# leopard-ai/betty

Hardware: AMD Instinct MI355X
Metric: hypergradient-steps/sec (CG K=20, 10M inner params) (higher is better)
Workload: dtype f32

## Files before the change

betty_amd/_native.py:

```python
from __future__ import annotations

import ctypes
import os
from ctypes import POINTER, c_char_p, c_double, c_float, c_int, c_int32, c_int64, c_size_t, c_void_p

_HERE = os.path.dirname(os.path.abspath(__file__))
LIB_PATH = os.environ.get("BHG_LIB") or os.path.join(_HERE, "csrc", "libbhg.so")
AB_LIB_PATH = os.environ.get("BHG_AB_LIB") or os.path.join(_HERE, "csrc", "libbhg_ab.so")

BHG_CHUNK_ELEMS = 4096
BHG_FLAT_ALIGN = 64
BHG_CG_AUTO, BHG_CG_STREAM, BHG_CG_RESIDENT = 0, 1, 2
BHG_CG_GLOBAL_CHAIN, BHG_CG_GLOBAL_UPDATE, BHG_CG_GLOBAL_DOTS = 0, 1, 2
BHG_CG_FX_BEGIN, BHG_CG_FX_CHAIN, BHG_CG_FX_GRAM, BHG_CG_FX_END = 0, 1, 2, 3


class NativeLibraryError(RuntimeError):
    """libbhg.so is missing or a call into it failed."""


class Chunk(ctypes.Structure):

    _fields_ = [
        ("flat_off", c_int64),
        ("src_off", c_int64),
        ("tensor", c_int32),
        ("len", c_int32),
    ]


BHG_MLP_MAX_LAYERS = 32


class Mlp(ctypes.Structure):

    _fields_ = [
        ("L", c_int32),
        ("B", c_int32),
        ("Bp", c_int32),
        ("dims", c_int32 * (BHG_MLP_MAX_LAYERS + 1)),
        ("W", c_void_p * BHG_MLP_MAX_LAYERS),
        ("h", c_void_p * BHG_MLP_MAX_LAYERS),
        ("mask", c_void_p * BHG_MLP_MAX_LAYERS),
        ("delta", c_void_p * BHG_MLP_MAX_LAYERS),
        ("prob", c_void_p),
        ("sd", c_void_p),
        ("Rh", c_void_p * BHG_MLP_MAX_LAYERS),
        ("Rd", c_void_p * BHG_MLP_MAX_LAYERS),
        ("partial", c_void_p),
        ("partial_floats", c_size_t),
        ("ridge2", c_float),
        ("prepacked", c_int32),
    ]


_PP = POINTER(c_void_p)
_CH = c_void_p

SYMBOLS = {
    "bhg_version": (c_int, []),
    "bhg_last_error": (c_char_p, []),
    "bhg_layout_flat_size": (c_int64, [POINTER(c_int64), c_int]),
    "bhg_layout_num_chunks": (c_int64, [POINTER(c_int64), c_int]),
    "bhg_layout_build": (c_int, [POINTER(c_int64), c_int, POINTER(c_int64), POINTER(Chunk)]),
    "bhg_workspace_bytes": (c_size_t, [c_int]),
    "bhg_flatten": (c_int, [_PP, c_int, _CH, c_int, c_void_p, c_float, c_void_p, c_void_p]),
    "bhg_scatter": (c_int, [c_void_p, _PP, c_int, _CH, c_int, c_float, c_void_p, c_void_p]),
    "bhg_neumann_init": (c_int, [_PP, c_int, _CH, c_int, c_void_p, c_void_p, c_void_p, c_void_p]),
    "bhg_neumann_step": (
        c_int,
        [_PP, c_int, _CH, c_int, c_void_p, c_void_p, c_float, c_float, c_float, c_void_p, c_void_p],
    ),
    "bhg_cg_init": (c_int, [_PP, c_int, _CH, c_int, c_void_p, c_void_p, c_void_p, c_void_p, c_void_p]),
    "bhg_cg_init_masked": (c_int, [_PP, c_int, _CH, c_int, c_void_p, c_void_p, c_void_p, ctypes.c_uint64, c_void_p, c_void_p]),
    "bhg_cg_step": (
        c_int,
        [_PP, c_int, _CH, c_int, c_void_p, c_void_p, c_void_p, c_float, c_int, c_float, c_float, c_int, c_void_p, c_void_p],
    ),
    "bhg_cg_phase": (
        c_int,
        [c_int, _PP, c_int, _CH, c_int, c_void_p, c_void_p, c_void_p, c_float, c_int, c_float, c_float, c_void_p, c_void_p],
    ),
    "bhg_cg_partials_dev": (c_void_p, [c_void_p, c_int, c_int]),
    "bhg_cg_partials_count": (c_int, []),
    "bhg_cg_resident_capacity_chunks": (c_int, []),
    "bhg_cg_resident_ok": (c_int, []),
    "bhg_cg_resident_usable": (c_int, [c_int]),
    "bhg_cg_scalars_dev": (c_void_p, [c_void_p]),
    "bhg_cg_timeout_flag_dev": (c_void_p, [c_void_p]),
    "bhg_scale_flat": (c_int, [c_void_p, c_int64, c_float, c_void_p]),
    "bhg_darts_eps": (c_int, [_PP, c_int, _CH, c_int, c_double, c_void_p, c_void_p, c_void_p, c_void_p]),
    "bhg_axpy_multi": (c_int, [_PP, _PP, c_int, _CH, c_int, c_void_p, c_float, c_void_p, c_void_p]),
    "bhg_fd_perturb": (c_int, [_PP, c_void_p, _PP, c_int, _CH, c_int, c_void_p, c_float, c_void_p, c_void_p]),
    "bhg_cg_step_fd": (
        c_int,
        [_PP, _PP, c_void_p, c_int, _CH, c_int, c_void_p, c_void_p, c_void_p, c_float, c_int, c_float, c_float, c_int, c_void_p, c_void_p],
    ),
    "bhg_neumann_step_fd": (
        c_int,
        [_PP, _PP, c_void_p, c_int, _CH, c_int, c_void_p, c_void_p, c_float, c_float, c_float, c_void_p, c_void_p],
    ),
    "bhg_sama_adam_precondition": (
        c_int,
        [_PP, _PP, _PP, _PP, c_int, _CH, c_int, c_void_p, c_double, c_double, c_double, c_double, c_void_p, c_void_p],
    ),
    "bhg_debug_set": (c_int, [c_char_p, c_int]),
    "bhg_debug_unset": (c_int, [c_char_p]),
    "bhg_debug_reset": (None, []),
    "bhg_debug_key_count": (c_int, []),
    "bhg_debug_key_name": (c_char_p, [c_int]),
    "bhg_is_ab_build": (c_int, []),
    "bhg_timing_enable": (c_int, [c_int]),
    "bhg_timing_read": (c_int, [c_int, POINTER(c_double), POINTER(c_int)]),
    "bhg_logreg_prepare": (c_int, [c_void_p, c_void_p, c_void_p, c_int, c_int, c_void_p]),
    "bhg_logreg_tmp_floats": (c_size_t, [c_int, c_int]),
    "bhg_logreg_hvp": (
        c_int,
        [c_void_p, c_void_p, c_void_p, c_void_p, c_void_p, c_void_p, c_int, c_int, c_void_p],
    ),
    "bhg_logreg_solve_plan": (c_int, [c_int, c_int, c_int, c_int, c_char_p, c_size_t]),
    "bhg_logreg_solve_ws_bytes": (c_size_t, [c_int, c_int]),
    "bhg_logreg_cg_solve": (
        c_int,
        [c_void_p, c_void_p, c_void_p, c_void_p, c_void_p, c_void_p, c_void_p, c_int, c_int, c_int, c_float, c_float, c_int, c_int, c_void_p],
    ),
    "bhg_logreg_neumann_solve": (
        c_int,
        [c_void_p, c_void_p, c_void_p, c_void_p, c_void_p, c_void_p, c_void_p, c_int, c_int, c_int, c_float, c_float, c_int, c_int, c_void_p],
    ),
    "bhg_mlp_partial_floats": (c_size_t, [POINTER(Mlp)]),
    "bhg_mlp_hvp": (c_int, [POINTER(Mlp), _PP, _PP, c_void_p]),
    "bhg_mlp_hvp_mode": (c_int, [POINTER(Mlp), _PP, _PP, c_int, c_void_p]),
    "bhg_mlp_supports_native_prepare": (c_int, [POINTER(Mlp)]),
    "bhg_mlp_forward": (c_int, [POINTER(Mlp), _PP, c_void_p, c_void_p, c_void_p]),
    "bhg_mlp_backward": (c_int, [POINTER(Mlp), c_void_p, c_void_p]),
    "bhg_mlp_mixed_coeff": (c_int, [POINTER(Mlp), _PP, c_void_p, c_void_p, c_void_p]),
    "bhg_mlp_supports_fused_solve": (c_int, [POINTER(Mlp)]),
    "bhg_mlp_fused_ws_bytes": (c_size_t, [POINTER(Mlp)]),
    "bhg_mlp_cg_solve": (
        c_int,
        [POINTER(Mlp), c_void_p, c_void_p, c_void_p, POINTER(c_int64), _CH, c_int, c_int, c_float, c_float, c_void_p,
         c_void_p, c_size_t, c_void_p],
    ),
    "bhg_mlp_cg_state_mask": (ctypes.c_uint64, [POINTER(Mlp), c_int]),
    "bhg_mlp_cg_solve_rhs": (
        c_int,
        [POINTER(Mlp), c_void_p, c_void_p, c_void_p, POINTER(c_int64), _CH, c_int, c_int, c_float, c_float, c_void_p,
         c_void_p, c_size_t, _PP, c_void_p],
    ),
    "bhg_mlp_cg_global_phase": (
        c_int,
        [POINTER(Mlp), c_void_p, c_void_p, c_void_p, POINTER(c_int64), _CH, c_int, c_int, c_int, c_int, c_int, c_void_p, c_float,
         c_float, c_void_p, c_void_p, c_size_t, c_void_p],
    ),
    "bhg_mlp_fx_supported": (c_int, [POINTER(Mlp), c_int]),
    "bhg_mlp_fx_ws_bytes": (c_size_t, [POINTER(Mlp), c_int]),
    "bhg_mlp_fx_const_floats": (c_size_t, [POINTER(Mlp)]),
    "bhg_mlp_fx_slab_floats": (c_size_t, [POINTER(Mlp)]),
    "bhg_mlp_fx_scal_doubles": (c_size_t, [POINTER(Mlp)]),
    "bhg_mlp_cg_fx_phase": (
        c_int,
        [POINTER(Mlp), _PP, c_int, c_int, c_int, c_int, c_int, c_void_p, c_void_p, c_void_p, c_float, c_float, c_void_p, c_size_t,
         c_void_p, c_size_t, c_void_p],
    ),
    "bhg_mlp_neumann_fx_phase": (
        c_int,
        [POINTER(Mlp), _PP, c_int, c_int, c_int, c_int, c_int, c_void_p, c_void_p, c_void_p, c_float, c_float, c_void_p, c_size_t,
         c_void_p, c_size_t, c_void_p],
    ),
    "bhg_mlp_cg_mixed_coeff": (c_int, [POINTER(Mlp), c_void_p, c_void_p, c_float, c_void_p, c_size_t, c_void_p]),
    "bhg_mlp_timeout_flag_dev": (c_void_p, [POINTER(Mlp), c_void_p]),
    "bhg_mlp_stage_batch": (c_int, [POINTER(Mlp), c_void_p, c_void_p, c_void_p, c_void_p]),
    "bhg_mlp_supports_packed_prepare": (c_int, [POINTER(Mlp)]),
    "bhg_mlp_forward_packed": (c_int, [POINTER(Mlp), _PP, c_void_p, c_void_p, c_void_p, c_size_t, c_void_p]),
    "bhg_mlp_backward_packed": (c_int, [POINTER(Mlp), c_void_p, c_void_p, c_size_t, c_void_p]),
    "bhg_mwn_max_hidden": (c_int, []),
    "bhg_mlp_fd_ws_bytes": (c_size_t, [POINTER(c_int), c_int, c_int]),
    "bhg_mlp_fd_forward": (
        c_int,
        [c_void_p, c_void_p, c_int, POINTER(c_int), c_int, _PP, _PP, c_void_p, c_int, c_void_p, c_void_p, c_void_p, c_size_t, c_void_p],
    ),
    "bhg_mwn_fd_vjp": (
        c_int,
        [c_void_p, c_void_p, c_int, c_void_p, c_void_p, c_void_p, c_void_p, c_int, c_void_p, c_int, c_void_p, c_void_p, c_void_p, c_void_p,
         c_void_p],
    ),
    "bhg_quad_fd": (c_int, [_PP, _PP, _PP, c_int, _CH, c_int, c_void_p, c_float, c_int, c_int, c_int, c_void_p]),
    "bhg_mwn_forward": (c_int, [c_void_p, c_int, c_void_p, c_void_p, c_void_p, c_void_p, c_int, c_void_p, c_void_p, c_void_p]),
    "bhg_mwn_backward": (
        c_int,
        [c_void_p, c_void_p, c_int, c_void_p, c_void_p, c_void_p, c_void_p, c_int, c_float, c_void_p, c_void_p, c_void_p, c_void_p, c_void_p],
    ),
    "bhg_mlp_neumann_solve": (
        c_int,
        [POINTER(Mlp), c_void_p, c_void_p, c_void_p, POINTER(c_int64), c_int, c_float, c_float, c_void_p, c_size_t, POINTER(c_int), c_void_p],
    ),
    "bhg_mlp_wsk_launches": (c_int64, []),
    "bhg_mlp_hoist_launches": (c_int64, []),
    "bhg_mlp_proj_iterations": (c_int64, []),
    "bhg_mlp_lin_launches": (c_int64, []),
    "bhg_mlp_neumann_mixed_coeff": (c_int, [POINTER(Mlp), _PP, c_void_p, c_void_p, c_float, c_int, c_int, c_void_p, c_size_t, c_void_p]),
    "bhg_mlp_plan_describe": (c_int, [POINTER(Mlp), c_int, c_int, ctypes.c_char_p, c_size_t]),
    "bhg_copy2d": (c_int, [c_void_p, c_int64, c_void_p, c_int64, c_int64, c_int64, c_void_p]),
    "bhg_bn_ws_bytes": (c_size_t, [c_int]),
    "bhg_bn_backward_vjp": (
        c_int,
        [c_void_p, c_void_p, c_void_p, c_void_p, c_void_p, c_void_p, c_void_p, c_void_p, c_int, c_int, c_int, c_void_p, c_void_p, c_void_p,
         c_void_p, c_size_t, c_void_p],
    ),
}

_libs = {}
_current = [None]


_PY_ENV = {"BHG_LIB", "BHG_AB_LIB", "BHG_HVP_GRAPH", "BHG_ALL_RANKS_ON_GPU0"}
_warned_env = [False]


def _warn_legacy_env() -> None:
    if _warned_env[0]:
        return
    _warned_env[0] = True
    stale = sorted(k for k in os.environ if k.startswith("BHG_") and k not in _PY_ENV)
    if stale:
        import warnings

        warnings.warn("betty_amd: environment variable(s) " + ", ".join(stale) + " are IGNORED — libbhg reads no environment variable. "
                      "Measurement arms are selected with betty_amd._native.use_ab() + debug_set(key, int) (bench.py --debug KEY=INT) "
                      "on the measurement build libbhg_ab.so.", RuntimeWarning, stacklevel=3)


def _bind(path: str) -> ctypes.CDLL:
    lib = _libs.get(path)
    if lib is not None:
        return lib
    _warn_legacy_env()
    if not os.path.exists(path):
        raise NativeLibraryError(
            f"{path} not found: the HIP extension has not been built. Run "
            "`python -c 'import __graft_entry__ as g; g.build()'` or `make -C betty_amd/csrc`. "
            "betty_amd has no CPU fallback."
        )
    lib = ctypes.CDLL(path)
    for name, (restype, argtypes) in SYMBOLS.items():
        try:
            fn = getattr(lib, name)
        except AttributeError as exc:
            raise NativeLibraryError(f"{path} does not export {name}") from exc
        fn.restype = restype
        fn.argtypes = argtypes
    _libs[path] = lib
    return lib


def load() -> ctypes.CDLL:
    return _bind(_current[0] or LIB_PATH)


def current_lib_path() -> str:
    return _current[0] or LIB_PATH


def is_ab() -> bool:
    return bool(load().bhg_is_ab_build())


def use_ab(on: bool = True) -> None:
    if on:
        _bind(AB_LIB_PATH)
        _current[0] = AB_LIB_PATH
    else:
        _current[0] = None


def check(rc: int, what: str) -> None:
    if rc != 0:
        msg = load().bhg_last_error()
        raise NativeLibraryError(f"{what} failed with code {rc}: {msg.decode() if msg else ''}")


def _debug_key(key: str) -> bytes:
    k = key.strip()
    if k.upper().startswith("BHG_"):
        k = k[4:]
    return k.lower().encode()


def debug_set(key: str, value) -> None:
    lib = load()
    if value is not None and not lib.bhg_is_ab_build():
        raise NativeLibraryError(f"bhg_debug_set({key}): the product libbhg.so carries no measurement arm — call "
                                 "betty_amd._native.use_ab() first (libbhg_ab.so; the `bhg_debug` fixture and `bench.py --debug` do)")
    if value is None:
        check(lib.bhg_debug_unset(_debug_key(key)), f"bhg_debug_unset({key})")
    else:
        check(lib.bhg_debug_set(_debug_key(key), int(value)), f"bhg_debug_set({key})")


def debug_reset() -> None:
    load().bhg_debug_reset()


def debug_keys():
    lib = load()
    return [lib.bhg_debug_key_name(i).decode() for i in range(lib.bhg_debug_key_count())]


def ptr_array(ptrs):
    arr = (c_void_p * len(ptrs))(*ptrs)
    return ctypes.cast(arr, _PP), arr


def plan_describe(dims, B: int, algo: str = "cg", keep_solution: bool = False) -> dict:
    lib = load()
    d = Mlp()
    d.L, d.B, d.Bp = len(dims) - 1, int(B), (int(B) + 127) // 128 * 128
    for i, v in enumerate(dims):
        d.dims[i] = int(v)
    buf = ctypes.create_string_buffer(2048)
    check(lib.bhg_mlp_plan_describe(ctypes.byref(d), {"cg": 0, "neumann": 1}[algo], 1 if keep_solution else 0, buf, 2048), "bhg_mlp_plan_describe")
    out, text = {}, buf.value.decode()
    import re

# ... 5 lines not shown
```

betty_amd/csrc/bhg_common.hpp:

```cpp
#pragma once
#include <hip/hip_runtime.h>
#include <stdint.h>
#include <stddef.h>
#include <stdio.h>
#include <string.h>

#include "bhg.h"

namespace bhg {

constexpr int kThreads = 256;
constexpr int kWaves = kThreads / 64;
constexpr int kChunk = BHG_CHUNK_ELEMS;
constexpr int kVecPerThread = kChunk / (kThreads * 4);
constexpr int kMaxBlocks = 1024;
constexpr int kInlineT = 32;
constexpr int kWriterT = 448;

constexpr size_t kWsScal = 0;
constexpr size_t kWsPartP = 128;
constexpr size_t kWsPartR = kWsPartP + 8 * kMaxBlocks;
constexpr size_t kWsBarrier = kWsPartR + 16 * kMaxBlocks;
constexpr size_t kWsTables = kWsBarrier + 256;
inline size_t ws_bytes(int T) {
  size_t b = kWsTables + 4 * sizeof(void*) * (size_t)(T > 0 ? T : 0);
  return (b + 255) & ~(size_t)255;
}

enum { S_RR_OLD = 0, S_PHP = 1, S_ALPHA = 2, S_RR_NEW = 3, S_BETA = 4, S_PP = 5 , S_ALPHA_RING = 10 ,
       S_NPART0 = 8  };

#define BHG_DBG_KEYS(X)                                                                                                      \
  X(mlp_wsk) X(mlp_wsk_maxk) X(mlp_wsk_depth) X(mlp_wsk_lds) X(wsl_depth) X(no_nt_slabs) X(gemm_no_xpose) X(mlp_no_fast)      \
  X(mlp_tn) X(split_target) X(split_cap) X(mlp_no_head) X(gram_ksplit) X(gram_kchunk) X(proj_graw_split) X(mlp_proj)         \
  X(mlp_hoist) X(hoist_wgs) X(proj_step_alone) X(mlp_no_side) X(mlp_no_fuse) X(mlp_no_outer_all) X(neumann_side)             \
  X(hoist_staged_mink) X(proj_alpha_alone) X(proj_small_alone) X(outer_order_by_work) X(outer_no_pre) X(outer_stagger)       \
  X(mlp_no_fused_solve) X(cg_eager_p) X(cg_x_every_iter) X(neumann_p_every_iter) X(head_no_prefetch) X(cg_spin_limit)        \
  X(packed_chain) X(packed_depth) X(packed_gram) X(proj_max_ratio) X(proj_ws_cap_mb) X(alpha_in_hoist) X(graw_v2) X(wskp_ragged) X(pstep_v2) X(pstep_unroll) X(rnew_in_graw) X(graw_cols) X(lin_first) X(lin_prio) X(lin_nub) X(lin_order) X(lin_update_next) X(lin_withhold_beta) X(neumann_vnew) X(cg_rhs_direct) X(packed_prepare) X(lin_deep) X(graw_kloop) X(lin_update_in_head) X(xcd_pairs) X(headu_head_first) X(fx_ksplit)
enum DbgKey : int {
#define BHG_DBG_ENUM(n) DBG_##n,
  BHG_DBG_KEYS(BHG_DBG_ENUM)
#undef BHG_DBG_ENUM
  DBG_COUNT
};
constexpr int kDbgUnset = INT32_MIN;
#ifdef BHG_AB
extern int g_dbg[DBG_COUNT];
inline bool dbg_is_set(DbgKey k) { return g_dbg[k] != kDbgUnset; }
inline int dbg(DbgKey k, int dflt) { return g_dbg[k] == kDbgUnset ? dflt : g_dbg[k]; }
#else
constexpr bool dbg_is_set(DbgKey) { return false; }
constexpr int dbg(DbgKey, int dflt) { return dflt; }
#endif

constexpr int kStampKernels = 4, kStampBlocks = 4096, kStampSlots = 8;
#ifdef BHG_STAMPS
#ifdef __HIPCC__
#define BHG_STAMP(kid, slot)                                                                                            \
  do {                                                                                                                  \
    if (threadIdx.x == 0 && blockIdx.x < ::bhg::kStampBlocks) {                                                         \
      unsigned long long* sp_ = ::bhg::d_stamps;                                                                        \
      if (sp_) sp_[((kid) * ::bhg::kStampBlocks + blockIdx.x) * ::bhg::kStampSlots + (slot)] = wall_clock64();          \
    }                                                                                                                   \
  } while (0)
#endif
#else
#define BHG_STAMP(kid, slot) do { } while (0)
#endif

void set_error(const char* fmt, ...);
#define BHG_HIP_CHECK(expr)                                                        \
  do {                                                                             \
    hipError_t _e = (expr);                                                        \
    if (_e != hipSuccess) {                                                        \
      ::bhg::set_error("%s failed: %s (%s:%d)", #expr, hipGetErrorString(_e), __FILE__, \
                       __LINE__);                                                  \
      return BHG_ERR_HIP;                                                          \
    }                                                                              \
  } while (0)
#define BHG_REQUIRE(cond, msg)                                                     \
  do {                                                                             \
    if (!(cond)) {                                                                 \
      ::bhg::set_error("%s: %s", __func__, msg);                                   \
      return BHG_ERR_ARG;                                                          \
    }                                                                              \
  } while (0)

struct PtrTab {
  const void* const* dev;
  const void* inl[kInlineT];
};

int make_table(PtrTab* out, const void* const* host_ptrs, int T, void* ws, int slot,
               hipStream_t stream);

bool span_begin(int kind, hipEvent_t* a, hipEvent_t* b);

#ifdef __HIPCC__
__device__ __forceinline__ float* tab_ptr(const PtrTab& t, int i) {
  const void* p = t.dev ? t.dev[i] : t.inl[i];
  return (float*)p;
}

__device__ __forceinline__ float4 ld4(const float* __restrict__ base, int e, int len) {
  if (e + 4 <= len) return *reinterpret_cast<const float4*>(base + e);
  float4 r = make_float4(0.f, 0.f, 0.f, 0.f);
  if (e < len) r.x = base[e];
  if (e + 1 < len) r.y = base[e + 1];
  if (e + 2 < len) r.z = base[e + 2];
  return r;
}
__device__ __forceinline__ void st4(float* __restrict__ base, int e, int len, float4 v) {
  if (e + 4 <= len) {
    *reinterpret_cast<float4*>(base + e) = v;
    return;
  }
  if (e < len) base[e] = v.x;
  if (e + 1 < len) base[e + 1] = v.y;
  if (e + 2 < len) base[e + 2] = v.z;
}

__device__ __forceinline__ float mul_rn(float a, float b) { return __fmul_rn(a, b); }
__device__ __forceinline__ float add_rn(float a, float b) { return __fadd_rn(a, b); }
__device__ __forceinline__ float sub_rn(float a, float b) { return __fsub_rn(a, b); }
__device__ __forceinline__ float div_rn(float a, float b) { return __fdiv_rn(a, b); }
__device__ __forceinline__ float4 scale4(float s, float4 a) {
  return make_float4(mul_rn(s, a.x), mul_rn(s, a.y), mul_rn(s, a.z), mul_rn(s, a.w));
}
__device__ __forceinline__ float4 add4(float4 a, float4 b) {
  return make_float4(add_rn(a.x, b.x), add_rn(a.y, b.y), add_rn(a.z, b.z), add_rn(a.w, b.w));
}
__device__ __forceinline__ float4 add_scaled4(float4 a, float s, float4 b) {
  return make_float4(add_rn(a.x, mul_rn(s, b.x)), add_rn(a.y, mul_rn(s, b.y)), add_rn(a.z, mul_rn(s, b.z)),
                     add_rn(a.w, mul_rn(s, b.w)));
}
__device__ __forceinline__ float4 sub_scaled4(float4 a, float s, float4 b) {
  return make_float4(sub_rn(a.x, mul_rn(s, b.x)), sub_rn(a.y, mul_rn(s, b.y)), sub_rn(a.z, mul_rn(s, b.z)),
                     sub_rn(a.w, mul_rn(s, b.w)));
}
__device__ __forceinline__ float4 diff_over4(float4 a, float4 b, float d) {
  return make_float4(div_rn(sub_rn(a.x, b.x), d), div_rn(sub_rn(a.y, b.y), d), div_rn(sub_rn(a.z, b.z), d),
                     div_rn(sub_rn(a.w, b.w), d));
}
__device__ __forceinline__ double dot4(float4 a, float4 b) {
  return (double)a.x * b.x + (double)a.y * b.y + (double)a.z * b.z + (double)a.w * b.w;
}

template <int BYTES>
__device__ __forceinline__ void kernarg_warm() {
  typedef const __attribute__((address_space(4))) unsigned* KP;
  KP kp = (KP)__builtin_amdgcn_kernarg_segment_ptr();
  unsigned acc = 0;
#pragma unroll
  for (int o = 0; o < BYTES; o += 64) acc |= kp[o / 4];
  asm volatile("" ::"s"(acc));
}
template <int U>
__device__ __forceinline__ double sum_strided(const double* __restrict__ p, const int n, const int t, const int stride) {
  double acc = 0.0;
  for (int i0 = t; i0 < n; i0 += U * stride) {
    double v[U];
#pragma unroll
    for (int u = 0; u < U; ++u) {
      const int i = i0 + u * stride;
      v[u] = p[i < n ? i : n - 1];
    }
#pragma unroll
    for (int u = 0; u < U; ++u)
      if (i0 + u * stride < n) acc += v[u];
  }
  return acc;
}

template <int U>
struct StridedRegs { double v[U]; };
template <int U>
__device__ __forceinline__ void strided_load(StridedRegs<U>& r, const double* __restrict__ p, const int n, const int t, const int stride,
                                             const double* __restrict__ dummy) {
  const double* q = (p && n > 0) ? p : dummy;
  const int last = (p && n > 0) ? n - 1 : 0;
#pragma unroll
  for (int u = 0; u < U; ++u) {
    const int i = t + u * stride;
    r.v[u] = q[i < n && i <= last ? i : last];
  }
}
template <int U>
__device__ __forceinline__ double strided_sum(const StridedRegs<U>& r, const int n, const int t, const int stride) {
  double acc = 0.0;
#pragma unroll
  for (int u = 0; u < U; ++u)
// ... 72 lines not shown
```

betty_amd/csrc/bhg_mlp.hip:

```cpp
#include <stdlib.h>
#include <vector>


#include "bhg_common.hpp"

#ifdef BHG_STAMPS
namespace bhg { __device__ unsigned long long* d_stamps = nullptr; }
#endif

namespace bhg {
namespace {
#include "mlp/gemm.inc"

#include "mlp/outer.inc"

#include "mlp/scalars.inc"

#include "mlp/head.inc"

#include "mlp/wsk.inc"

#include "mlp/wskp.inc"

inline int wsk_mode(int chain_mode, int unfused_hint) {
  if (dbg_is_set(DBG_mlp_wsk)) return dbg(DBG_mlp_wsk, 0);
  if (chain_mode == FUSE_CG) return 2;
  if (chain_mode == FUSE_NEUMANN) return 3;
  return unfused_hint;
}
inline bool wsk_wanted(int mode, int pairs, int K) {
  if (mode == 1) return true;
  if (mode != 2 && mode != 3) return false;
  return pairs * K <= dbg(DBG_mlp_wsk_maxk, 1024);
}
inline int wsk_depth() {
  const int d = dbg(DBG_mlp_wsk_depth, 3);
  return d == 2 ? 2 : 3;
}
inline bool wsk_eligible(const WskArgs& a) {
  if (a.pairs < 1 || a.pairs > 2) return false;
  bool ok = a.M % 32 == 0 && a.N % 32 == 0 && a.K % 32 == 0 && a.K >= 32;
  for (int i = 0; i < a.pairs; ++i) ok = ok && (a.pr[i].lda & 3) == 0 && (a.pr[i].ldb & 3) == 0;
  return ok;
}
int64_t g_wsk_launches = 0;
int64_t g_hoist_launches = 0;
int64_t g_proj_iterations = 0;
int64_t g_lin_launches = 0;
template <int LB>
void launch_gemm_wsk(const WskArgs& a_in, hipStream_t st, bool staged = false) {
  WskArgs a = a_in;
  ++g_wsk_launches;
  a.ntm = a.M / 32;
  a.ntn = a.N / 32;
  bool bf = false;
  for (int i = 0; i < a.pairs; ++i) bf = bf || a.pr[i].mix != 0;
  const dim3 grid(a.ntm * a.ntn), block(64 * kWskWaves);
  const int d = wsk_depth();
  const bool force_staged = dbg(DBG_mlp_wsk_lds, 0) != 0;
  if ((staged || force_staged) && !bf) {
    const int lds = (int)(sizeof(float) * kWslWaveFloats * kWskWaves);
    static bool attr_done = false;
    if (!attr_done) {
      (void)hipFuncSetAttribute(reinterpret_cast<const void*>(k_gemm_wsk<LB, false, 2, true>), hipFuncAttributeMaxDynamicSharedMemorySize, lds);
      attr_done = true;
    }
#ifdef BHG_AB
    const int wsl_depth = dbg(DBG_wsl_depth, 2);
    if (wsl_depth == 3) {
      static bool attr3 = false;
      if (!attr3) {
        (void)hipFuncSetAttribute(reinterpret_cast<const void*>(k_gemm_wsk<LB, false, 3, true>), hipFuncAttributeMaxDynamicSharedMemorySize, lds);
        attr3 = true;
      }
      hipLaunchKernelGGL((k_gemm_wsk<LB, false, 3, true>), grid, block, lds, st, a);
      return;
    }
#endif
    hipLaunchKernelGGL((k_gemm_wsk<LB, false, 2, true>), grid, block, lds, st, a);
    return;
  }
#define BHG_WSK(BFV, DV) hipLaunchKernelGGL((k_gemm_wsk<LB, BFV, DV>), grid, block, 0, st, a)
  if (bf) {
    if (d == 2 || LB == LAYOUT_RC) BHG_WSK(true, 2); else BHG_WSK(true, LB == LAYOUT_RC ? 2 : 3);
  } else {
#ifdef BHG_AB
    if (d == 2) BHG_WSK(false, 2); else
#endif
    BHG_WSK(false, 3);
  }
#undef BHG_WSK
}

#ifdef BHG_AB
void launch_wsk_group(const WskGroupArgs& g, int blocks, hipStream_t st) {
  const int lds = (int)(sizeof(float) * kWslWaveFloats * kWskWaves);
  static bool attr_done = false;
  if (!attr_done) {
    (void)hipFuncSetAttribute(reinterpret_cast<const void*>(k_wsk_group<2>), hipFuncAttributeMaxDynamicSharedMemorySize, lds);
#ifdef BHG_AB
    (void)hipFuncSetAttribute(reinterpret_cast<const void*>(k_wsk_group<3>), hipFuncAttributeMaxDynamicSharedMemorySize, lds);
#endif
    attr_done = true;
  }
#ifdef BHG_AB
  const int wsl_depth = dbg(DBG_wsl_depth, 2);
  if (wsl_depth == 3) { hipLaunchKernelGGL(k_wsk_group<3>, dim3(blocks), dim3(64 * kWskWaves), lds, st, g); return; }
#endif
  hipLaunchKernelGGL(k_wsk_group<2>, dim3(blocks), dim3(64 * kWskWaves), lds, st, g);
}
#endif

int chip_cus() {
  static int cus[64];
  int dev = 0;
  if (hipGetDevice(&dev) != hipSuccess || dev < 0 || dev >= 64) { (void)hipGetLastError(); return 256; }
  if (cus[dev] > 0) return cus[dev];
  int n = 0;
  if (hipDeviceGetAttribute(&n, hipDeviceAttributeMultiprocessorCount, dev) != hipSuccess || n <= 0) { (void)hipGetLastError(); n = 256; }
  return cus[dev] = n;
}
inline void wskp_tiling(WskpProb* q, bool ragged) {
  q->nfull = q->RA / 32;
  q->nstrip = 0;
  q->pairs = dbg(DBG_xcd_pairs, 1);
  if (!ragged || q->raw || q->nsplit != 1 || q->RB % 64 != 0) return;
  int nf = q->B / 32, rem = q->B % 32;
  if (rem > 16) { ++nf; rem = 0; }
  if (nf == 0) return;
  q->nfull = nf;
  q->nstrip = rem > 0 ? q->RB / 64 : 0;
}
struct WskpBuilder {
  WskpArgs g{};
  int blk = 0;
  bool add(const WskpProb& q_in) {
    if (g.n >= kWskpMax) return false;
    g.p[g.n++] = q_in;
    return true;
  }
  void tile(bool ragged) {
    blk = 0;
    for (int i = 0; i < g.n; ++i) {
      WskpProb& q = g.p[i];
      wskp_tiling(&q, ragged);
      g.blk0[i] = blk;
      blk += (((q.nfull * (q.RB / 32) + q.nstrip) * q.nsplit) + 7) & ~7;
    }
  }
  void launch(hipStream_t st) {
    if (!g.n) return;
    const int mode = dbg(DBG_wskp_ragged, 1);
    tile(mode == 2);
    if (mode == 1 && blk > chip_cus()) tile(true);
    g.blk0[g.n] = blk;
    const int d = dbg(DBG_packed_depth, 2);
    bool riders = g.n <= 3;
// ... 197 lines not shown
  size_t rh0alt_off;
  size_t gp2alt_off;
  bool proj_ok;
  size_t floats;
  int gf[BHG_MLP_MAX_LAYERS], gb[BHG_MLP_MAX_LAYERS];
};
inline bool graw_batch_ok(int Bp) { return Bp == 128 || (Bp % 128 == 0 && dbg(DBG_graw_kloop, 1) != 0); }
inline bool graw_split() {
  return dbg(DBG_proj_graw_split, 1) != 0;
}
inline int proj_mode() {
  return dbg(DBG_mlp_proj, 1);
}
inline int hoist_mode() {
  return dbg(DBG_mlp_hoist, 1);
}
void hoist_plan(const bhg_mlp* m, HoistPlan* hp) {
  memset(hp, 0, sizeof(*hp));
  const int L = m->L, Bp = m->Bp;
  for (int l = 0; l < BHG_MLP_MAX_LAYERS; ++l) hp->gf[l] = hp->gb[l] = -1;
  if (!use_head(m) || L < 3 || L - 1 > kHoistMax / 2 || Bp % kTM != 0) return;
  for (int l = 0; l <= L - 1; ++l) if (m->dims[l] % 32 != 0) return;
  const int Nh = m->dims[L - 1];
  if ((size_t)Nh * sizeof(float) > 64 * 1024) return;
  for (int l = 1; l + 1 < L; ++l)
    if ((Bp / 32) * (m->dims[l] / 32) != reduce_blocks(Bp * m->dims[l], m->dims[l])) return;
  int n = 0;
  for (int l = 0; l + 1 < L; ++l) { hp->layer[n] = l; hp->bwd[n] = 0; hp->K[n] = m->dims[l]; hp->N[n] = m->dims[l + 1]; hp->gf[l] = n; ++n; }
  for (int l = 1; l + 1 < L; ++l) { hp->layer[n] = l; hp->bwd[n] = 1; hp->K[n] = m->dims[l + 1]; hp->N[n] = m->dims[l]; hp->gb[l] = n; ++n; }
  hp->n = n;
  const int slots = dbg(DBG_hoist_wgs, 768);
  const int ntm = Bp / kTM;
  int tgt = 8;
  for (; tgt < 4096; ++tgt) {
    int wgs = 0;
    for (int i = 0; i < n; ++i) {
      const int ks = hp->K[i] / kTK;
      const int per = ks < tgt ? ks : tgt;
      wgs += (hp->N[i] / 32) * ntm * ((ks + per - 1) / per);
    }
    if (wgs <= slots) break;
  }
  size_t off = 0;
  int blk = 0;
  for (int i = 0; i < n; ++i) {
    const int ks = hp->K[i] / kTK;
    int sp = (ks + tgt - 1) / tgt;
    const int per = (ks + sp - 1) / sp;
    sp = (ks + per - 1) / per;
    hp->splits[i] = sp;
    hp->blk0[i] = blk;
    blk += (hp->N[i] / 32) * ntm * sp;
    hp->slab_off[i] = off; off += (size_t)sp * Bp * hp->N[i];
    hp->g_off[i] = off;    off += (size_t)Bp * hp->N[i];
    hp->gr_off[i] = off;   off += (size_t)Bp * hp->N[i];
    hp->graw_off[i] = off; off += (size_t)2 * Bp * hp->N[i];
  }
  {
    double fh = 0.0, fp = 0.0;
    for (int l = 0; l + 1 < L; ++l) fh += (double)m->dims[l] * m->dims[l + 1] * (l >= 1 ? 2.0 : 1.0);
    fh *= 2.0 * Bp;
    for (int l = 0; l + 1 < L; ++l) {
      fp += (double)m->dims[l + 1] * (l == 0 ? 1.0 : 2.0);
      if (l >= 1) fp += 2.0 * m->dims[l] + (double)m->dims[l] + (double)m->dims[l + 1];
    }
    fp *= 2.0 * Bp * (double)Bp;
    size_t gram = 0;
    for (int l = 0; l + 1 < L; ++l) gram += (size_t)Bp * Bp * (l >= 1 ? (2 + 2 * kGramSplitMax + 6) : 2);
    size_t widest = 0;
    for (int i = 0; i < n; ++i) widest = (size_t)hp->N[i] > widest ? (size_t)hp->N[i] : widest;
    hp->proj_ok = fp * 100.0 <= fh * (double)dbg(DBG_proj_max_ratio, 400) &&
                  gram * sizeof(float) <= (size_t)dbg(DBG_proj_ws_cap_mb, 1024) * 1024 * 1024 &&
                  (size_t)Bp * (widest / 4) <= ((size_t)1 << 20);
  }
  hp->dot_blocks = 0;
  for (int i = 0; i < n; ++i) hp->dot_blocks += dot_blocks_of(Bp * (hp->N[i] / 4));
  hp->raw_blocks = 0;
  for (int i = 0; i < n; ++i) hp->raw_blocks += (hp->N[i] / 32) * ntm * 2;
  for (int l = 0; hp->proj_ok && l + 1 < L; ++l) {
    hp->s_off[l] = off; off += (size_t)Bp * Bp;
    if (l >= 1) {
      hp->d_off[l] = off; off += (size_t)Bp * Bp;
      hp->tslab_off[l] = off; off += (size_t)kGramSplitMax * Bp * Bp;
      hp->eslab_off[l] = off; off += (size_t)kGramSplitMax * Bp * Bp;
    }
  }
  for (int l = 0; hp->proj_ok && l + 1 < L; ++l) {
    hp->sp_off[l] = off; off += (size_t)Bp * Bp;
    if (l >= 1) {
      hp->dp_off[l] = off; off += (size_t)Bp * Bp;
      hp->tslabp_off[l] = off; off += (size_t)2 * Bp * Bp;
      hp->eslabp_off[l] = off; off += (size_t)2 * Bp * Bp;
    }
  }
  hp->lin_ok = hp->proj_ok && L >= 4 && (L == 4 || dbg(DBG_lin_deep, 1) != 0);
  if (hp->lin_ok) {
    for (int i = 0; i < 2; ++i) { hp->z1_off[i] = off; off += (size_t)Bp * m->dims[2]; }
    hp->rh0rp_off = off; off += (size_t)Bp * m->dims[1];
    hp->gp1alt_off = off; off += (size_t)Bp * m->dims[2];
    hp->rb0c_off = off; off += (size_t)((m->dims[1] + 63) & ~63);
  }
  if (hp->proj_ok) { hp->rh0alt_off = off; off += (size_t)Bp * m->dims[1]; }
  if (hp->lin_ok) { hp->gp2alt_off = off; off += (size_t)Bp * m->dims[L - 1]; }
  hp->graw_tiles = 0;
  for (int i = 0; i < n; ++i) hp->graw_tiles += (Bp / 64) * (hp->N[i] / 32);
  hp->blk0[n] = blk;
  hp->floats = off;
  hp->ok = true;
}

int graw_cols(const HoistPlan* hp, int Bp = 128) {
  if (dbg(DBG_graw_cols, 32) != 64 || Bp != 128) return 32;
  for (int i = 0; i < hp->n; ++i)
    if (hp->N[i] % 64) return 32;
  return 64;
}
int graw_tile_count(const HoistPlan* hp, int Bp) {
  const int ct = graw_cols(hp, Bp);
  int t = 0;
  for (int i = 0; i < hp->n; ++i) t += (Bp / 64) * (hp->N[i] / ct);
  return t;
}
int graw_blocks(const HoistPlan* hp, int Bp) {
  int n = 0;
  for (int i = 0; i < hp->n; ++i) {
    const bool two = !(hp->bwd[i] == 0 && hp->layer[i] == 0);
    n += (hp->N[i] / 32) * (Bp / kTM) * ((two && graw_split()) ? 2 : 1);
  }
  return n;
}

bool proj_step_merged() {
  return dbg(DBG_proj_step_alone, 0) == 0;
}

struct FusedWs {
  double* partT1; double* partT2h; double* partT2; double* partPP; double* partRR[2];
  float* rz; double* rzx;
  int t2_off[BHG_MLP_MAX_LAYERS];
  int nRR, nT2;
  float* hoist;
  double* part_dot; double* pscal;
  double* part_raw;
  double* part_graw;
  float* pb0[2];
  float* pb1[2];
  unsigned long long* gran;
  float* Wf[BHG_MLP_MAX_LAYERS];
  float* Wb[BHG_MLP_MAX_LAYERS];
  float* hpk[BHG_MLP_MAX_LAYERS];
  float* dpk[BHG_MLP_MAX_LAYERS];
  float* Rhp[BHG_MLP_MAX_LAYERS];
  float* Rdp[BHG_MLP_MAX_LAYERS];
  size_t bytes;
};
void carve_fused_ws(const bhg_mlp* m, void* base, FusedWs* w) {
  memset(w, 0, sizeof(*w));
  const bool head = use_head(m);
  int nrr = bias_blocks(m);
  for (int l = 0; l < m->L; ++l) nrr += outer_blocks(m, l, head);
  w->nRR = nrr;
  size_t off = 0;
  auto take = [&](size_t bytes) { void* p = base ? static_cast<char*>(base) + off : nullptr; off += (bytes + 255) & ~(size_t)255; return p; };
  w->partT1 = static_cast<double*>(take(sizeof(double) * m->Bp));
  w->partT2h = static_cast<double*>(take(sizeof(double) * m->Bp));
  w->partPP = static_cast<double*>(take(sizeof(double) * kMaxBlocks));
  w->partRR[0] = static_cast<double*>(take(sizeof(double) * 3 * nrr));
  w->partRR[1] = static_cast<double*>(take(sizeof(double) * 3 * nrr));
  int nt2 = 0;
  for (int l = 1; l + 1 < m->L; ++l) { w->t2_off[l] = nt2; nt2 += reduce_blocks(m->Bp * m->dims[l], m->dims[l]); }
  w->nT2 = nt2;
  w->partT2 = static_cast<double*>(take(sizeof(double) * (nt2 > 0 ? nt2 : 1)));
  w->rz = static_cast<float*>(take(sizeof(float) * (size_t)m->Bp * m->dims[m->L]));
  w->rzx = static_cast<double*>(take(sizeof(double) * (size_t)m->Bp * m->dims[m->L]));
  HoistPlan hp;
  hoist_plan(m, &hp);
  w->hoist = static_cast<float*>(take(sizeof(float) * (hp.ok ? hp.floats : 1)));
  w->part_dot = static_cast<double*>(take(sizeof(double) * 2 * (hp.ok ? hp.dot_blocks : 1)));
  w->part_raw = static_cast<double*>(take(sizeof(double) * (hp.ok ? hp.raw_blocks : 1)));
  w->part_graw = static_cast<double*>(take(sizeof(double) * 3 * (hp.ok ? hp.graw_tiles : 1)));
  w->pscal = static_cast<double*>(take(sizeof(double) * 8));
  for (int i = 0; i < 2; ++i) w->pb0[i] = static_cast<float*>(take(sizeof(float) * (size_t)m->dims[1]));
  for (int i = 0; i < 2; ++i) w->pb1[i] = static_cast<float*>(take(sizeof(float) * (size_t)(m->L >= 2 ? m->dims[2] : 1)));
  w->gran = static_cast<unsigned long long*>(take(64 * 64));
  if (hp.ok) {
    const int L = m->L;
    const size_t Bp = (size_t)m->Bp;
    for (int l = 0; l + 1 < L; ++l) {
      w->hpk[l] = static_cast<float*>(take(sizeof(float) * Bp * m->dims[l]));
      if (l + 2 < L) w->Rhp[l] = static_cast<float*>(take(sizeof(float) * Bp * m->dims[l + 1]));
      if (l >= 1) {
        w->Wf[l] = static_cast<float*>(take(sizeof(float) * (size_t)m->dims[l + 1] * m->dims[l]));
        w->Wb[l] = static_cast<float*>(take(sizeof(float) * (size_t)m->dims[l + 1] * m->dims[l]));
        w->dpk[l] = static_cast<float*>(take(sizeof(float) * Bp * m->dims[l + 1]));
        w->Rdp[l] = static_cast<float*>(take(sizeof(float) * Bp * m->dims[l + 1]));
      }
    }
  }
  w->bytes = off;
}

bool graw_single_on(bool packed, int Bp) { return packed && dbg(DBG_packed_gram, 1) != 0 && dbg(DBG_graw_v2, 1) != 0 && graw_batch_ok(Bp); }
bool rnew_keys_on() { return dbg(DBG_proj_small_alone, 0) == 0 && dbg(DBG_alpha_in_hoist, 1) != 0 && dbg(DBG_rnew_in_graw, 1) != 0; }

bool packed_chain_on(const FusedWs& w) { return w.Wf[1] != nullptr && dbg(DBG_packed_chain, 1) != 0; }
int pack_operands(const bhg_mlp* m, const FusedWs& w, hipStream_t st, bool weights_only = false) {
  PackArgs g{};
  int blk = 0;
  auto add = [&](const float* X, float* Xp, int R, int K, int kind) {
    if (g.n >= kPackMax) return false;
    g.p[g.n] = {X, Xp, R, K, kind};
    g.blk0[g.n] = blk;
    blk += pack_blocks(g.p[g.n]);
    ++g.n;
    return true;
  };
  const int L = m->L, Bp = m->Bp;
  bool ok = true;
  for (int l = 0; l + 1 < L && ok; ++l) {
    if (!weights_only || l == 0) ok = ok && add(m->h[l], w.hpk[l], Bp, m->dims[l], 0);
    if (l >= 1) {
      if (!weights_only) ok = ok && add(m->delta[l], w.dpk[l], Bp, m->dims[l + 1], 0);
      ok = ok && add(m->W[l], w.Wf[l], m->dims[l + 1], m->dims[l], 0);
      ok = ok && add(m->W[l], w.Wb[l], m->dims[l], m->dims[l + 1], 1);
    }
  }
  BHG_REQUIRE(ok, "too many layers for one packing launch");
  g.blk0[g.n] = blk;
  hipLaunchKernelGGL(k_pack, dim3(blk), dim3(256), 0, st, g);
  BHG_HIP_CHECK(hipGetLastError());
  return BHG_OK;
}

#include "mlp/chain_plan.inc"

int hoist_products(const bhg_mlp* m, const void* const* dir, const ChainMode& cm, const ChainPlan& pl, hipStream_t st, ChainState* cs) {
  const int L = m->L, Bp = m->Bp, B = m->B;
  const HoistPlan* hp = pl.hp;
  float* hbase = pl.hoist;
  HoistArgs ha{};
  HoistRedArgs ra{};
  for (int i = 0; i < hp->n; ++i) {
    const int l = hp->layer[i];
    HoistProb& q = ha.p[i];
    q.A = hp->bwd[i] ? m->delta[l] : m->h[l];
    q.Bm = pl.cg ? ((cm.first && cm.rhs) ? static_cast<const float*>(cm.rhs[2 * l]) : cm.fa + cm.starts[2 * l]) : static_cast<const float*>(dir[2 * l]);
    q.slabs = hbase + hp->slab_off[i];
    q.K = hp->K[i]; q.N = hp->N[i]; q.splits = hp->splits[i]; q.rc = hp->bwd[i];
    q.lda = hp->K[i]; q.ldb = hp->bwd[i] ? hp->N[i] : hp->K[i];
    ha.blk0[i] = hp->blk0[i];
    HoistRedProb& rq = ra.p[i];
    rq.slabs = q.slabs; rq.G = hbase + hp->g_off[i]; rq.N = hp->N[i]; rq.splits = hp->splits[i];
    if (!hp->bwd[i] && l == 0) {
      rq.bias = static_cast<const float*>(dir[1]); rq.mask = m->mask[0]; rq.out = m->Rh[0];
      rq.outp = pl.packed ? cm.ws->Rhp[0] : nullptr;
    }
  }
  ha.blk0[hp->n] = hp->blk0[hp->n];
  ha.n = hp->n; ha.Bp = Bp; ha.gemm_blocks = hp->blk0[hp->n];
  const bool proj = cm.proj != 0;
  int rblk = 0;
  for (int i = 0; i < hp->n; ++i) { ra.blk0[i] = rblk; rblk += (Bp * (hp->N[i] / 4) + 255) / 256; }
  ra.blk0[hp->n] = rblk;
  if (!proj || cm.first) {
    ha.do_beta = (pl.cg && !cm.first && cm.beta && !proj) ? 1 : 0;
    ha.beta_blocks = ha.do_beta ? cm.beta_blocks : 0;
    if (ha.do_beta) ha.beta = *cm.beta;
    hipLaunchKernelGGL(k_hoist<FUSE_CG>, dim3(ha.gemm_blocks + (ha.do_beta ? cm.beta_blocks : 0)), dim3(256), 0, st, ha);
    ++g_hoist_launches;
    if (proj && pl.cg) for (int i = 0; i < hp->n; ++i) ra.p[i].G2 = hbase + hp->gr_off[i];
    ra.n = hp->n; ra.Bp = Bp; ra.B = B; ra.first = pl.cg ? cm.first : 1; ra.scal = cm.scal;
    hipLaunchKernelGGL(k_hoist_reduce, dim3(rblk), dim3(256), 0, st, ra);
  } else if (pl.vnew) {
    ++g_proj_iterations;
  } else {
    ProjArgs pa{};
    for (int i = 0; i < hp->n; ++i) {
      ProjProb& q = pa.p[i];
      q.Gr = hbase + (pl.cg ? hp->gr_off[i] : hp->g_off[i]); q.Gp = hbase + hp->g_off[i]; q.Graw = hbase + hp->graw_off[i]; q.N = hp->N[i];
      if (!pl.graw_single && graw_split() && !(hp->bwd[i] == 0 && hp->layer[i] == 0)) q.Graw2 = q.Graw + (size_t)Bp * hp->N[i];
      if (pl.rnew) q.Graw = nullptr;
      if (!hp->bwd[i] && hp->layer[i] == 0) {
        q.bias = static_cast<const float*>(dir[1]); q.mask = m->mask[0]; q.out = m->Rh[0];
        q.outp = pl.packed ? cm.ws->Rhp[0] : nullptr;
      }
      pa.blk0[i] = ra.blk0[i];
    }
    pa.blk0[hp->n] = rblk;
    pa.n = hp->n; pa.Bp = Bp; pa.B = B; pa.kpar_prev = cm.kpar ^ 1; pa.shift = cm.shift; pa.scal = pl.cg ? cm.scal : nullptr; pa.alpha = cm.alpha;
    if (pl.cg && cm.proj >= 2 && proj_step_merged()) {
      ProjStepArgs g{};
      g.pa = pa;
      ProjScalArgs& sa = g.sa;
      sa.part_dot = cm.ws->part_dot; sa.dot_blocks = hp->dot_blocks;
      sa.part_raw = cm.ws->part_raw; sa.raw_blocks = graw_blocks(hp, Bp);
      if (pl.graw_single) {
        const int gt = graw_tile_count(hp, Bp);
        sa.part_dot = cm.ws->part_graw; sa.dot_blocks = gt;
        sa.part_raw = cm.ws->part_graw + 2 * (size_t)gt; sa.raw_blocks = gt;
      }
      sa.part = cm.beta->part; sa.part_stride = cm.ws->nRR;
      sa.off0 = pl.part_base_w[L - 1]; sa.n0 = outer_blocks(m, L - 1, pl.head); sa.off1 = pl.part_base_bias; sa.n1 = bias_blocks(m);
      sa.r_small = cm.beta->r; sa.p_small = cm.beta->p; sa.snt = cm.beta->nt;
      int small_total = 0;
      for (int t = 0; t < cm.beta->nt; ++t) { sa.soff[t] = cm.beta->off[t]; sa.slen[t] = cm.beta->len[t]; small_total += cm.beta->len[t]; }
      sa.scal = cm.scal; sa.pscal = cm.ws->pscal; sa.shift = cm.shift; sa.first = cm.second; sa.kpar = cm.kpar ^ 1;
      const int sgrid = small_total > 0 ? (small_total + kThreads - 1) / kThreads : 1;
      g.update_blocks = rblk;
      g.r_b0 = cm.fa + cm.starts[1];
      g.p0_rd = cm.second ? cm.fd + cm.starts[1] : cm.ws->pb0[cm.kpar ^ 1];
      g.p0_wr = cm.ws->pb0[cm.kpar];
      if (pl.graw_single && cm.beta->nt <= 16 && dbg(DBG_pstep_v2, 1) != 0) {
        PstepArgs ps{};
        PstepHdr& h = ps.h;
        const int pu = pl.lin ? 4 : dbg(DBG_pstep_unroll, 4);
        const int U = pu >= 4 ? 4 : (pu >= 2 ? 2 : 1);
        int ublk = 0;
        for (int i = 0; i < hp->n; ++i) { h.blk0[i] = ublk; ublk += (Bp * (hp->N[i] / 4) + 256 * U - 1) / (256 * U); }
        h.blk0[hp->n] = ublk;
        const int rblk = ublk;
        h.n = pa.n; h.Bp = pa.Bp; h.B = pa.B; h.kpar_prev = pa.kpar_prev; h.shift = pa.shift; h.update_blocks = rblk;
        h.scal = sa.scal; h.r_b0 = g.r_b0; h.p0_rd = g.p0_rd; h.p0_wr = g.p0_wr; h.r_small = sa.r_small; h.p_small = sa.p_small;
        h.part_dot = sa.part_dot; h.part_raw = sa.part_raw; h.part = sa.part; h.pscal = sa.pscal;
        h.dot_blocks = sa.dot_blocks; h.raw_blocks = sa.raw_blocks; h.part_stride = sa.part_stride;
        h.off0 = sa.off0; h.n0 = sa.n0; h.off1 = sa.off1; h.n1 = sa.n1; h.first = sa.first; h.kpar = sa.kpar; h.snt = sa.snt;
        for (int i = 0; i < hp->n; ++i) {
          const ProjProb& q = pa.p[i];
          ps.p[i] = {q.Gr, q.Gp, q.Graw, q.bias, q.mask, q.out, q.outp, q.N, q.Graw ? 1 : 0};
          if (pl.lin && i == hp->gf[1]) { ps.p[i].Gp = pl.gp1(cm.kpar ^ 1); ps.p[i].X = pl.gp1(cm.kpar); ps.p[i].xkind = 2; }
          if (pl.lin_head && i == hp->gf[L - 2]) { ps.p[i].Gp = pl.gp2(cm.kpar ^ 1); ps.p[i].X = pl.gp2(cm.kpar); ps.p[i].xkind = 2; }
          if (pl.lin) ps.p[i].outp = nullptr;
        }
        if (pl.lin) {
          h.p1_rd = cm.second ? cm.fd + cm.starts[3] : cm.ws->pb1[cm.kpar ^ 1];
          h.p1_wr = cm.ws->pb1[cm.kpar];
          h.gran = cm.ws->gran;
          h.rb0_copy = hbase + hp->rb0c_off;
          h.prio = dbg(DBG_lin_prio, 0);
          h.withhold = dbg(DBG_lin_withhold_beta, 0);
          int nub = dbg(DBG_lin_nub, 0);
          if (nub > 0) {
            WskpProb tq{};
            tq.RA = Bp; tq.RB = m->dims[2]; tq.B = B; tq.nsplit = 1;
            wskp_tiling(&tq, true);
            const int tiles = ((tq.nfull * (tq.RB / 32) + tq.nstrip + 7) & ~7) + (Bp / 32) * (Bp / 32);
            const int room = chip_cus() - tiles - sgrid;
            if (nub == 1 || nub > room) nub = room;
          }
          h.nub = (nub > 0 && nub < rblk) ? nub : 0;
        }
        for (int t = 0; t < sa.snt; ++t) { ps.t.slen[t] = sa.slen[t]; ps.t.soff[t] = sa.soff[t]; }
        if (pl.lin) { cs->lin_ps = ps; cs->lin_nu = (h.nub > 0 ? h.nub : rblk) + sgrid; cs->lin_U = U; }
#ifdef BHG_AB
        else if (U == 2) hipLaunchKernelGGL(k_pstep<2>, dim3(rblk + sgrid), dim3(256), 0, st, ps);
        else if (U == 1) hipLaunchKernelGGL(k_pstep<1>, dim3(rblk + sgrid), dim3(256), 0, st, ps);
#endif
        else hipLaunchKernelGGL(k_pstep<4>, dim3(rblk + sgrid), dim3(256), 0, st, ps);
      } else {
#ifdef BHG_AB
        hipLaunchKernelGGL(k_proj_step, dim3(rblk + sgrid), dim3(256), 0, st, g);
#else
        BHG_REQUIRE(false, "internal: every plan of the product takes k_pstep (<= 16 small tensors, the packed closing launch)");
#endif
      }
    } else {
      hipLaunchKernelGGL(k_proj_update, dim3(rblk), dim3(256), 0, st, pa);
    }
    ++g_proj_iterations;
  }
  return BHG_OK;
}

int lin_first_product(const bhg_mlp* m, const void* const* dir, const ChainMode& cm, const ChainPlan& pl, hipStream_t st, ChainState* cs) {
  const int L = m->L, Bp = m->Bp, B = m->B, K = m->dims[1], N = m->dims[2];
  const HoistPlan* hp = pl.hp;
  float* hbase = pl.hoist;
  const float* c = static_cast<const float*>(dir[3]);
  const float* Gf = hbase + hp->g_off[hp->gf[1]];
  BHG_REQUIRE(cm.first || cs->lin_nu > 0, "no update blocks for the linear first product");
  WskplArgs la{};
  WskpProb& q = la.a;
  q.Ap = cm.first ? cm.ws->Rhp[0] : hbase + hp->rh0rp_off;
  q.Bq = cm.ws->Wf[1]; q.RA = Bp; q.RB = N; q.K = K; q.B = B; q.nsplit = 1;
  q.mask = m->mask[1]; q.out = m->Rh[1]; q.outp = cm.ws->Rhp[1];
  q.znew = hbase + hp->z1_off[cm.kpar];
  if (cm.first) { q.addend = Gf; q.bias = c; }
  else {
    q.addend = hbase + hp->gr_off[hp->gf[1]]; q.addend2 = pl.gp1(cm.kpar ^ 1);
    q.bias = cm.fa + cm.starts[3]; q.bias2 = cs->lin_ps.h.p1_rd;
    q.zold = hbase + hp->z1_off[cm.kpar ^ 1];
    q.gran = cm.ws->gran;
  }
  const int rider_blocks = pl.gram_in_chain ? (Bp / 32) * (Bp / 32) : 0;
  wskp_tiling(&q, false);
  int na = (q.nfull * (q.RB / 32) + q.nstrip + 7) & ~7;
  if (dbg(DBG_wskp_ragged, 1) == 2 || (dbg(DBG_wskp_ragged, 1) == 1 && na + rider_blocks > chip_cus()) ||
      (!cm.first && cs->lin_ps.h.nub > 0)) {
    wskp_tiling(&q, true);
    na = (q.nfull * (q.RB / 32) + q.nstrip + 7) & ~7;
  }
  la.na = na;
  if (pl.gram_in_chain) {
    float* tnew = hbase + hp->tslab_off[1] + (size_t)cm.kpar * Bp * Bp;
    float* tnewp = pl.graw2 ? hbase + hp->tslabp_off[1] + (size_t)cm.kpar * Bp * Bp : nullptr;
    la.r0 = {cm.ws->hpk[1], q.Ap, tnew, tnewp, K, 0};
    la.r0_old = cm.first ? nullptr : hbase + hp->tslab_off[1] + (size_t)(cm.kpar ^ 1) * Bp * Bp;
  }
  la.nu = cm.first ? 0 : cs->lin_nu;
  const bool upd_next = !cm.first && L == 4 && dbg(DBG_lin_update_next, 1) != 0 && cs->lin_ps.h.nub == 0;
  if (upd_next) {
    la.ns = cs->lin_nu - cs->lin_ps.h.update_blocks;
    la.nt = na + rider_blocks;
  } else if (!cm.first && L > 4 && cs->lin_ps.h.nub == 0) {
    la.ns = cs->lin_nu - cs->lin_ps.h.update_blocks;
    la.nt = na + rider_blocks;
    la.upd_first = 1;
  } else
  if (!cm.first && dbg(DBG_lin_order, 0) != 0) {
    la.ns = cs->lin_nu - (cs->lin_ps.h.nub > 0 ? cs->lin_ps.h.nub : cs->lin_ps.h.update_blocks);
    la.nt = na + rider_blocks;
  }
  la.ps = cs->lin_ps;
  BHG_REQUIRE(cm.first || la.ns > 0 || cs->lin_ps.h.update_blocks <= 2 * chip_cus(),
              "update blocks ahead of the publisher would not all be resident: use the default order");
  const int grid = (upd_next ? la.ns : la.nu) + na + rider_blocks;
  cs->lin_update_pending = upd_next;
  BHG_REQUIRE(cm.first || cs->lin_U == 4, "the update blocks inside k_wskpl are built for four float4 per thread");
#ifdef BHG_AB
  if (la.ps.h.nub > 0) hipLaunchKernelGGL((k_wskpl<2, 4, true>), dim3(grid), dim3(64 * kWskpWaves), 0, st, la); else
#endif
  hipLaunchKernelGGL((k_wskpl<2, 4, false>), dim3(grid), dim3(64 * kWskpWaves), 0, st, la);
  ++g_lin_launches;
  if (cm.first)
    BHG_HIP_CHECK(hipMemcpyAsync(hbase + hp->rb0c_off, cm.fa + cm.starts[1], sizeof(float) * (size_t)m->dims[1],
                                 hipMemcpyDeviceToDevice, st));
  return BHG_OK;
}

int hoist_forward(const bhg_mlp* m, const void* const* dir, const ChainMode& cm, const ChainPlan& pl, hipStream_t st, int staged_mink,
                  ChainState* cs) {
  const int L = m->L, Bp = m->Bp, B = m->B;
  const HoistPlan* hp = pl.hp;
  float* hbase = pl.hoist;
  for (int l = 1; l + 1 < L; ++l) {
    const int K = m->dims[l], N = m->dims[l + 1];
    const float* c = static_cast<const float*>(dir[2 * l + 1]);
    const float* Gf = hbase + hp->g_off[hp->gf[l]];
    if (pl.packed) {
    if (pl.lin && l == 1) {
      if (int rc = lin_first_product(m, dir, cm, pl, st, cs)) return rc;
    } else {
      WskpBuilder wb;
      WskpProb q{};
      q.Ap = cm.ws->Rhp[l - 1]; q.Bq = cm.ws->Wf[l]; q.RA = Bp; q.RB = N; q.K = K; q.B = B; q.nsplit = 1;
      if (l == L - 2) {
        const int riders = (pl.gram_in_chain && l == 1) ? (Bp / 32) * (Bp / 32) : 0;
        const int tiles_l = (Bp / 32) * (N / 32);
        int sp = (chip_cus() - riders) / tiles_l;
        const int cap = pick_splits((N + pl.tn - 1) / pl.tn, K, 1);
        if (sp > cap) sp = cap;
        if (sp > K / 64) sp = K / 64;
        if (sp < 1) sp = 1;
        q.nsplit = sp; q.raw = 1; q.out = m->partial;
        cs->head_fuse = {m->partial, sp, Bp * N, c, m->mask[l], m->Rh[l], (pl.lin_head && !cm.first) ? hbase + hp->gr_off[hp->gf[l]] : Gf};
        cs->fuse_head = true;
      } else {
        q.bias = c; q.mask = m->mask[l]; q.addend = Gf; q.out = m->Rh[l]; q.outp = cm.ws->Rhp[l];
      }
      wb.add(q);
      if (pl.gram_in_chain && l == 1) {
        WskpProb t{};
        t.Ap = cm.ws->hpk[l]; t.Bq = cm.ws->Rhp[l - 1]; t.RA = Bp; t.RB = Bp; t.K = K; t.B = B;
        t.nsplit = 1; t.raw = 1; t.out = hbase + hp->tslab_off[l]; t.outp = pl.graw2 ? hbase + hp->tslabp_off[l] : nullptr;
        wb.add(t);
      }
      if (cs->lin_update_pending && wb.g.n == 1 && !pl.lin_head) {
        launch_wskpu(wb.g.p[0], cs->lin_ps, cs->lin_ps.h.update_blocks, st);
        cs->lin_update_pending = false;
      } else wb.launch(st);
    }
      if (pl.gram_in_chain && cm.first && l == 1) {
        WskpBuilder sb;
        for (int j = 0; j + 1 < L; ++j) {
          WskpProb u{};
          u.Ap = cm.ws->hpk[j]; u.Bq = cm.ws->hpk[j]; u.RA = Bp; u.RB = Bp; u.K = m->dims[j]; u.B = B; u.raw = 1;
          u.nsplit = 1;
          u.out = hbase + hp->s_off[j]; u.outp = hbase + hp->sp_off[j];
          if (!sb.add(u)) { sb.launch(st); sb.add(u); }
          if (j >= 1) {
            u.Ap = cm.ws->dpk[j]; u.Bq = cm.ws->dpk[j]; u.K = m->dims[j + 1]; u.out = hbase + hp->d_off[j]; u.outp = hbase + hp->dp_off[j];
            if (!sb.add(u)) { sb.launch(st); sb.add(u); }
          }
        }
        sb.launch(st);
        cs->sd_in_chain = true;
      }
      continue;
    }
    if (l == L - 2) {
      GemmArgs a{};
      a.pr[0] = {m->Rh[l - 1], m->W[l], K, K};
      a.pairs = 1; a.M = Bp; a.N = N; a.K = K;
      a.splits = pick_splits((N + pl.tn - 1) / pl.tn, K, 1);
      a.out = m->partial; a.ldo = N; a.out_rows = Bp;
      launch_gemm<LAYOUT_KC, LAYOUT_KC>(a, pl.tn, st);
      cs->head_fuse = {m->partial, a.splits, Bp * N, c, m->mask[l], m->Rh[l], Gf};
      cs->fuse_head = true;
    } else {
      WskArgs w{};
      w.pr[0] = {m->Rh[l - 1], m->W[l], K, K}; w.pairs = 1; w.M = Bp; w.N = N; w.K = K; w.B = B;
      w.bias = c; w.mask = m->mask[l]; w.out = m->Rh[l]; w.addend = Gf;
      launch_gemm_wsk<LAYOUT_KC>(w, st, K >= staged_mink);
    }
  }
  BHG_REQUIRE(!cs->lin_update_pending || pl.lin_head, "the update blocks found no launch to ride in");
  return BHG_OK;
}

int hoist_head(const bhg_mlp* m, const void* const* dir, const ChainMode& cm, const ChainPlan& pl, hipStream_t st, ChainState* cs) {
  const int L = m->L, Bp = m->Bp, B = m->B;
  if (cs->lin_update_pending) {
    const int l = L - 1, K = m->dims[l], N = m->dims[l + 1];
    BHG_REQUIRE(cs->fuse_head && pl.cg && pl.packed && N <= 12 && K <= 512, "k_headu was planned for a head it cannot run");
    HeaduArgs ha{};
    ha.Rh = (const float*)m->Rh[l - 1]; ha.h = m->h[l]; ha.W = m->W[l]; ha.V = static_cast<const float*>(dir[2 * l]);
    ha.cb = static_cast<const float*>(dir[2 * l + 1]); ha.prob = m->prob; ha.sd = m->sd; ha.rd = m->Rd[l];
    ha.K = K; ha.C = N; ha.B = B; ha.mode = HEAD_JVP;
    ha.delta_top = (const float*)m->delta[l]; ha.mask_prev = (const float*)m->mask[l - 1]; ha.rd_prev = m->Rd[l - 1];
    ha.fz = cs->head_fuse;
    ha.partT1 = cm.ws->partT1; ha.partT2h = cm.ws->partT2h; ha.rz_out = cm.ws->rz; ha.rzx_acc = cm.rzx_acc; ha.rzx_first = cm.first;
    ha.rows = Bp; ha.rd_prev_p = cm.ws->Rdp[l - 1];
    ha.addend2 = pl.gp2(cm.kpar ^ 1); ha.gran = cm.ws->gran;
    ha.nu = cs->lin_ps.h.update_blocks; ha.ps = cs->lin_ps; ha.head_first = dbg(DBG_headu_head_first, 1);
    hipLaunchKernelGGL(k_headu<4>, dim3(ha.nu + Bp), dim3(256), (size_t)K * sizeof(float), st, ha);
    cs->lin_update_pending = false;
  } else {
    const int l = L - 1, K = m->dims[l], N = m->dims[l + 1];
    launch_head_forward(st, Bp, (const float*)m->Rh[l - 1], m->h[l], m->W[l], static_cast<const float*>(dir[2 * l]),
                        static_cast<const float*>(dir[2 * l + 1]), m->prob, m->sd, m->Rd[l], K, N, B, HEAD_JVP, nullptr, nullptr,
                        (const float*)m->delta[l], (const float*)m->mask[l - 1], m->Rd[l - 1], &cs->head_fuse,
                        pl.cg ? cm.ws->partT1 : nullptr, pl.cg ? cm.ws->partT2h : nullptr, pl.cg ? cm.ws->rz : nullptr, cm.rzx_acc, cm.first,
                        pl.packed ? cm.ws->Rdp[l - 1] : nullptr);
  }
  return BHG_OK;
}

void hoist_backward(const bhg_mlp* m, const ChainMode& cm, const ChainPlan& pl, hipStream_t st, int staged_mink) {
  const int L = m->L, Bp = m->Bp, B = m->B;
  const HoistPlan* hp = pl.hp;
  float* hbase = pl.hoist;
  for (int l = L - 2; l >= 1; --l) {
    const int K = m->dims[l + 1], N = m->dims[l];
    if (pl.packed) {
      WskpBuilder wb;
      WskpProb q{};
      q.Ap = cm.ws->Rdp[l]; q.Bq = cm.ws->Wb[l]; q.RA = Bp; q.RB = N; q.K = K; q.B = B; q.nsplit = 1;
      q.mask = m->mask[l - 1]; q.addend = hbase + hp->g_off[hp->gb[l]]; q.out = m->Rd[l - 1];
      q.outp = l >= 2 ? cm.ws->Rdp[l - 1] : nullptr;
      if (pl.cg) { q.rh = m->Rh[l - 1]; q.partT2 = cm.ws->partT2 + cm.ws->t2_off[l]; }
      wb.add(q);
      if (pl.gram_in_chain) {
        WskpProb t{};
        t.Ap = cm.ws->dpk[l]; t.Bq = cm.ws->Rdp[l]; t.RA = Bp; t.RB = Bp; t.K = K; t.B = B;
        t.nsplit = 1; t.raw = 1; t.out = hbase + hp->eslab_off[l]; t.outp = pl.graw2 ? hbase + hp->eslabp_off[l] : nullptr;
        wb.add(t);
        if (l + 1 <= L - 2) {
          t.Ap = cm.ws->hpk[l + 1]; t.Bq = cm.ws->Rhp[l];
          t.out = hbase + hp->tslab_off[l + 1]; t.outp = pl.graw2 ? hbase + hp->tslabp_off[l + 1] : nullptr;
          wb.add(t);
        }
      }
      wb.launch(st);
      continue;
    }
    WskArgs w{};
    w.pr[0] = {m->Rd[l], m->W[l], K, N}; w.pairs = 1; w.M = Bp; w.N = N; w.K = K; w.B = B;
    w.mask = m->mask[l - 1]; w.out = m->Rd[l - 1]; w.addend = hbase + hp->g_off[hp->gb[l]];
    if (pl.cg) { w.rh = m->Rh[l - 1]; w.partT2 = cm.ws->partT2 + cm.ws->t2_off[l]; }
    launch_gemm_wsk<LAYOUT_RC>(w, st, K >= staged_mink);
  }
}

int chain_hoisted(const bhg_mlp* m, const void* const* dir, const ChainMode& cm, const ChainPlan& pl, hipStream_t st, ChainState* cs) {
  if (int rc = hoist_products(m, dir, cm, pl, st, cs)) return rc;
  const int staged_mink = dbg(DBG_hoist_staged_mink, 256);
  if (int rc = hoist_forward(m, dir, cm, pl, st, staged_mink, cs)) return rc;
  if (int rc = hoist_head(m, dir, cm, pl, st, cs)) return rc;
  if (!cm.stop_after_head) hoist_backward(m, cm, pl, st, staged_mink);
  return BHG_OK;
}

void chain_forward(const bhg_mlp* m, const void* const* dir, const ChainMode& cm, const ChainPlan& pl, hipStream_t st, ChainState* cs) {
  const int L = m->L, Bp = m->Bp, B = m->B;
  for (int l = 0; l < L; ++l) {
    const int K = m->dims[l], N = m->dims[l + 1];
    const float* V = static_cast<const float*>(dir[2 * l]);
    const float* c = static_cast<const float*>(dir[2 * l + 1]);
    if (pl.head && l == L - 1) {
      launch_head_forward(st, Bp, l > 0 ? (const float*)m->Rh[l - 1] : nullptr, m->h[l], m->W[l], V, c, m->prob, m->sd,
                          m->Rd[l], K, N, B, HEAD_JVP, nullptr, nullptr, l > 0 ? (const float*)m->delta[l] : nullptr,
                          l > 0 ? (const float*)m->mask[l - 1] : nullptr, l > 0 ? m->Rd[l - 1] : nullptr,
                          cs->fuse_head ? &cs->head_fuse : nullptr, pl.cg ? cm.ws->partT1 : nullptr, pl.cg ? cm.ws->partT2h : nullptr,
                          pl.cg ? cm.ws->rz : nullptr, cm.rzx_acc, cm.first);
      continue;
    }
    GemmArgs a{};
    a.pr[0] = {m->h[l], V, K, K};
    if (cm.lazy) a.pr[0] = {m->h[l], cm.fa + cm.starts[2 * l], K, K, cm.fd + cm.starts[2 * l], 1};
    a.scal = cm.scal;
    a.pairs = 1;
    if (l > 0) { a.pr[1] = {m->Rh[l - 1], m->W[l], K, K}; a.pairs = 2; }
    a.M = Bp; a.N = N; a.K = K;
    const bool to_head = pl.head && l == L - 2 && !pl.no_fuse && (N & 3) == 0 && (size_t)N * sizeof(float) <= 64 * 1024;
    if (wsk_wanted(pl.wsk, a.pairs, K) && !to_head && l + 1 < L) {
      WskArgs w{};
      w.pr[0] = a.pr[0]; w.pr[1] = a.pr[1]; w.pairs = a.pairs; w.M = Bp; w.N = N; w.K = K; w.B = B;
      w.bias = c; w.mask = m->mask[l]; w.out = m->Rh[l]; w.scal = cm.scal;
      if (wsk_eligible(w)) { launch_gemm_wsk<LAYOUT_KC>(w, st); continue; }
    }
    a.splits = pick_splits((N + pl.tn - 1) / pl.tn, K, a.pairs);
    a.out = m->partial; a.ldo = N; a.out_rows = Bp;
    launch_gemm<LAYOUT_KC, LAYOUT_KC>(a, pl.tn, st);
    const int slab = Bp * N;
    if (to_head) {
      cs->head_fuse = {m->partial, a.splits, slab, c, m->mask[l], m->Rh[l]};
      cs->fuse_head = true;
    } else if (l + 1 < L) {
      launch_reduce_mask(st, m->partial, a.splits, slab, c, m->mask[l], m->Rh[l], Bp, N, B);
    } else {
      hipLaunchKernelGGL(k_reduce_softmax_jvp, dim3((Bp + 15) / 16), dim3(256), 0, st, (const float*)m->partial,
                         a.splits, slab, c, m->prob, m->sd, m->Rd[l], Bp, N, B);
    }
  }
}

void outer_args(const bhg_mlp* m, const void* const* dir, const ChainMode& cm, const ChainPlan& pl, int l, GemmArgs* ga, size_t* lds,
                bool* fast) {
  const int B = m->B, Mo = m->dims[l + 1], No = m->dims[l];
  const float* V = static_cast<const float*>(dir[2 * l]);
  GemmArgs a{};
  a.pr[0] = {m->Rd[l], m->h[l], Mo, No};
  a.pairs = 1;
  if (l > 0) { a.pr[1] = {m->delta[l], m->Rh[l - 1], Mo, No}; a.pairs = 2; }
  a.M = Mo; a.N = No; a.K = B;
  a.splits = 1;
  a.out = cm.mode == FUSE_NONE ? static_cast<float*>(cm.out[2 * l]) : nullptr; a.ldo = No; a.out_rows = 0;
  a.addend = pl.rho2 != 0.f ? V : nullptr; a.addend_scale = pl.rho2;
  a.kstages = (B + kOH - 1) / kOH < 2 ? 2 : (B + kOH - 1) / kOH;
  const int Kh = (((B + a.kstages - 1) / a.kstages) + 1) & ~1;
  *lds = (size_t)Kh * (kTM + kTN) * sizeof(float);
  const size_t lds_c = (size_t)kTM * kCPad * sizeof(float);
  if (*lds < lds_c) *lds = lds_c;
  bool f = Mo % kTM == 0 && No % kTN == 0 && (a.ldo & 3) == 0;
  for (int i = 0; i < a.pairs; ++i) f = f && (a.pr[i].lda & 3) == 0 && (a.pr[i].ldb & 3) == 0;
  if (cm.mode != FUSE_NONE) f = f && (cm.starts[2 * l] & 3) == 0;
  const bool no_fast = dbg(DBG_mlp_no_fast, 0) != 0;
  *fast = f && !no_fast;
  *ga = a;
}
HeadOuterArgs head_outer_args(const bhg_mlp* m, const void* const* dir, const ChainMode& cm, const ChainPlan& pl, int l) {
  HeadOuterArgs ha{};
  ha.rd = m->Rd[l]; ha.h = m->h[l]; ha.delta = m->delta[l]; ha.Rh = l > 0 ? m->Rh[l - 1] : nullptr;
  ha.V = static_cast<const float*>(dir[2 * l]); ha.rho2 = pl.rho2;
  ha.out = cm.mode == FUSE_NONE ? static_cast<float*>(cm.out[2 * l]) : nullptr;
  ha.N = m->dims[l]; ha.C = m->dims[l + 1]; ha.B = m->B;
  return ha;
}
void launch_outer(const bhg_mlp* m, const void* const* dir, const ChainMode& cm, const ChainPlan& pl, int l, hipStream_t s) {
  const FuseArgs fz = fuse_at(cm, pl, 2 * l, pl.part_base_w[l]);
  if (pl.head && l == pl.L - 1) {
    const HeadOuterArgs ha = head_outer_args(m, dir, cm, pl, l);
    const dim3 grid((ha.N + 63) / 64, ha.C);
#define BHG_HEAD_OUTER(RH, MODE) hipLaunchKernelGGL((k_head_outer<RH, MODE>), grid, dim3(256), 0, s, ha, fz)
    if (l > 0) {
// ... 237 lines not shown
  for (int i = 0; i < hp->n && !pl.graw2; ++i) {
    const int l = hp->layer[i];
    HoistProb& q = ga.p[i];
    if (!hp->bwd[i]) {
      q.A = hbase + hp->s_off[l]; q.Bm = m->Rd[l];
      if (l >= 1) { q.A2 = hbase + hp->tslab_off[l]; q.B2m = m->delta[l]; q.a2_slabs = pl.gram_slabs(m->dims[l]); }
    } else {
      q.A = hbase + hp->eslab_off[l]; q.Bm = m->h[l]; q.a_slabs = pl.gram_slabs(m->dims[l + 1]);
      q.A2 = hbase + hp->d_off[l]; q.B2m = m->Rh[l - 1];
    }
    q.slabs = hbase + hp->graw_off[i];
    q.a_slab_stride = Bp * Bp;
    if (full) q.X = hp->bwd[i] ? (const float*)m->Rh[l - 1] : (const float*)m->Rd[l];
    q.K = Bp; q.N = hp->N[i]; q.splits = (q.A2 && graw_split()) ? 2 : 1; q.rc = 1; q.lda = Bp; q.ldb = hp->N[i];
    ga.blk0[i] = gblk; gblk += (hp->N[i] / 32) * ntm * q.splits;
  }
  ga.blk0[hp->n] = gblk;
  ga.n = hp->n; ga.Bp = Bp; ga.gemm_blocks = gblk; ga.do_beta = 0;
  if (full && !pl.graw2) {
    int dblk = 0, nd = 0;
    for (int i = 0; i < hp->n; ++i) {
      const int l = hp->layer[i];
      ga.dp[nd] = {hbase + hp->gr_off[i], hbase + hp->g_off[i], hp->bwd[i] ? (const float*)m->Rh[l - 1] : (const float*)m->Rd[l], hp->N[i]};
      ga.dblk0[nd++] = dblk; dblk += dot_blocks_of(Bp * (hp->N[i] / 4));
    }
    ga.dblk0[nd] = dblk;
    ga.nd = nd; ga.dot_blocks = dblk; ga.B = B; ga.part_dot = cm.ws->part_dot; ga.part_raw = cm.ws->part_raw;
    BHG_REQUIRE(gblk == graw_blocks(hp, Bp), "tile count of the G(raw) launch and of its raw.raw partials disagree");
    BHG_REQUIRE(dblk == hp->dot_blocks, "dot block count of the plan and of the launch disagree");
  }
  if (small_in_graw) {
    ga.so = so;
    ga.small_blocks = small_blocks;
    if (alpha_in_hoist) { ga.do_alpha = 1; ga.alpha = od.aa; }
  }
  if (pl.graw2) {
  } else if (pl.cg) hipLaunchKernelGGL(k_hoist<FUSE_CG>, dim3(gblk + ga.dot_blocks + ga.small_blocks), dim3(256), 0, st, ga);
  else hipLaunchKernelGGL(k_hoist<FUSE_NEUMANN>, dim3(gblk + ga.dot_blocks + ga.small_blocks), dim3(256), 0, st, ga);
#endif
  return BHG_OK;
}

int close_outputs(const bhg_mlp* m, const void* const* dir, const ChainMode& cm, const ChainPlan& pl, const ChainOutputs& od, hipStream_t st,
                  bool small_in_graw) {
  const int L = m->L;
  const HoistPlan* hp = pl.hp;
  const bool proj_full = hp && ((pl.cg && cm.proj >= 2) || (!pl.cg && cm.proj));
  const int n_mfma = proj_full ? 0 : (pl.head ? L - 1 : L);
  OuterAllArgs oa{};
  bool all_fast = !pl.no_outer_all && n_mfma <= kOuterAllMax && pl.head;
  size_t lds_max = 0;
  int order[BHG_MLP_MAX_LAYERS];
  const bool work_first = dbg(DBG_outer_order_by_work, 0) != 0;
  auto weight = [&](int l) { return !work_first ? (double)outer_blocks(m, l, pl.head) : (l > 0 ? 2.0 : 1.0) * 1e9 + outer_blocks(m, l, pl.head); };
  for (int i = 0; i < n_mfma; ++i) order[i] = i;
  for (int i = 1; i < n_mfma; ++i)
    for (int j = i; j > 0 && weight(order[j]) > weight(order[j - 1]); --j) { int t = order[j]; order[j] = order[j - 1]; order[j - 1] = t; }
  int blk = 0;
  for (int i = 0; i < n_mfma && all_fast; ++i) {
    const int l = order[i];
    size_t lds; bool fast;
    outer_args(m, dir, cm, pl, l, &oa.g[i], &lds, &fast);
    all_fast = all_fast && fast;
    if (lds > lds_max) lds_max = lds;
    oa.f[i] = fuse_at(cm, pl, 2 * l, pl.part_base_w[l]);
    oa.gx[i] = (oa.g[i].N + kTN - 1) / kTN;
    oa.blk0[i] = blk;
    blk += outer_blocks(m, l, pl.head);
  }
  if (small_in_graw) {
  } else if (all_fast) {
    oa.n = n_mfma;
    oa.blk0[n_mfma] = blk;
    oa.head = head_outer_args(m, dir, cm, pl, L - 1);
    oa.hf = fuse_at(cm, pl, 2 * (L - 1), pl.part_base_w[L - 1]);
    oa.head_gx = (oa.head.N + 63) / 64;
    oa.head_blocks = oa.head_gx * oa.head.C;
    oa.head_has_rh = L > 1;
    oa.bf = od.bias_fz;
    const int total = blk + oa.head_blocks + od.bias_blk;
    if (lds_max < (size_t)kTM * kCPad * sizeof(float)) lds_max = (size_t)kTM * kCPad * sizeof(float);
    const bool no_pre = dbg(DBG_outer_no_pre, 0) != 0;
    (void)no_pre;
    const int stagger = dbg(DBG_outer_stagger, 1);
    oa.stagger = stagger;
#ifdef BHG_AB
    if (no_pre) {
      if (pl.cg) hipLaunchKernelGGL((k_outer_all<FUSE_CG, false>), dim3(total), dim3(256), lds_max, st, oa, od.ba);
      else hipLaunchKernelGGL((k_outer_all<FUSE_NEUMANN, false>), dim3(total), dim3(256), lds_max, st, oa, od.ba);
    } else
#endif
    {
      if (pl.cg) hipLaunchKernelGGL((k_outer_all<FUSE_CG, true>), dim3(total), dim3(256), lds_max, st, oa, od.ba);
      else hipLaunchKernelGGL((k_outer_all<FUSE_NEUMANN, true>), dim3(total), dim3(256), lds_max, st, oa, od.ba);
    }
  } else {
    for (int l = L - 1; l >= 0; --l) launch_outer(m, dir, cm, pl, l, st);
    launch_bias(cm, od, st);
  }
#ifdef BHG_AB
  if (proj_full && pl.cg && !proj_step_merged()) {
    BHG_REQUIRE(all_fast || small_in_graw, "the fully projected CG solver needs the single-launch output path");
    ProjScalArgs sa{};
    sa.part_dot = cm.ws->part_dot; sa.dot_blocks = hp->dot_blocks;
    sa.part_raw = cm.ws->part_raw; sa.raw_blocks = graw_blocks(hp, m->Bp);
    if (pl.graw_single) {
      const int gt = graw_tile_count(hp, m->Bp);
      sa.part_dot = cm.ws->part_graw; sa.dot_blocks = gt;
      sa.part_raw = cm.ws->part_graw + 2 * (size_t)gt; sa.raw_blocks = gt;
    }
    sa.part = cm.partRR_new; sa.part_stride = cm.ws->nRR;
    sa.off0 = pl.part_base_w[L - 1]; sa.n0 = outer_blocks(m, L - 1, pl.head); sa.off1 = pl.part_base_bias; sa.n1 = od.bias_blk;
    sa.r_small = cm.beta->r; sa.p_small = cm.beta->p; sa.snt = cm.beta->nt;
    for (int t = 0; t < cm.beta->nt; ++t) { sa.soff[t] = cm.beta->off[t]; sa.slen[t] = cm.beta->len[t]; }
    sa.scal = cm.scal; sa.pscal = cm.ws->pscal; sa.shift = cm.shift; sa.first = cm.first; sa.kpar = cm.kpar;
    int small_total = 0;
    for (int t = 0; t < cm.beta->nt; ++t) small_total += cm.beta->len[t];
    const int sgrid = small_total > 0 ? (small_total + kThreads - 1) / kThreads : 1;
    hipLaunchKernelGGL(k_proj_scalars, dim3(sgrid), dim3(kThreads), 0, st, sa);
  }
#endif
  return BHG_OK;
}

int chain_close(const bhg_mlp* m, const void* const* dir, const ChainMode& cm, const ChainPlan& pl, const ChainOutputs& od, hipStream_t st,
                const ChainState& cs) {
  const bool alpha_alone = dbg(DBG_proj_alpha_alone, 0) != 0 || pl.gram_in_chain;
  const bool small_alone = dbg(DBG_proj_small_alone, 0) != 0;
  const bool small_in_graw = pl.proj_iter && (cm.proj >= 2 || !pl.cg) && !small_alone;
  const bool alpha_in_hoist = pl.cg && pl.proj_iter && cm.proj >= 2 && small_in_graw && pl.gram_in_chain && cm.gphase == 0 &&
                              dbg(DBG_alpha_in_hoist, 1) != 0;
  const bool alpha_in_gram = pl.cg && pl.proj_iter && !alpha_alone;
  if (pl.cg && !alpha_in_gram && !alpha_in_hoist) hipLaunchKernelGGL(k_cg_alpha, dim3(1), dim3(kThreads), 0, st, od.aa);
  if (pl.cg && cm.skip_outputs) return BHG_OK;
  if (pl.proj_iter)
    if (int rc = close_graw(m, dir, cm, pl, od, st, cs, small_in_graw, alpha_in_gram, alpha_in_hoist)) return rc;
  return close_outputs(m, dir, cm, pl, od, st, small_in_graw);
}

int run_chain(const bhg_mlp* m, const void* const* dir, const ChainMode& cm, hipStream_t st) {
  ChainPlan pl;
  if (int rc = plan_chain(m, cm, &pl)) return rc;
  ChainState cs;
  if (pl.do_chain && pl.hp) {
    if (int rc = chain_hoisted(m, dir, cm, pl, st, &cs)) return rc;
    if (cm.stop_after_head) {
      BHG_HIP_CHECK(hipGetLastError());
      return BHG_OK;
    }
  }
  if (pl.do_chain && !pl.hp) chain_forward(m, dir, cm, pl, st, &cs);
  ChainOutputs od;
  describe_outputs(m, dir, cm, pl, &od);
  if (pl.do_chain && !pl.hp)
    if (int rc = chain_backward(m, dir, cm, pl, st)) return rc;

  if (pl.cg && cm.gphase == 1) {
    hipLaunchKernelGGL(k_php_local, dim3(1), dim3(kThreads), 0, st, od.aa, cm.php);
    BHG_HIP_CHECK(hipGetLastError());
    return BHG_OK;
  }
  if (pl.single) {
    if (int rc = chain_close(m, dir, cm, pl, od, st, cs)) return rc;
    BHG_HIP_CHECK(hipGetLastError());
    return BHG_OK;
  }

  const bool fork = m->L > 1 && !pl.no_side;
  if (fork) {
    BHG_HIP_CHECK(hipEventRecord(pl.ss->ev_rd[0], st));
    BHG_HIP_CHECK(hipStreamWaitEvent(pl.ss->side, pl.ss->ev_rd[0], 0));
    launch_bias(cm, od, pl.ss->side);
  } else {
    launch_bias(cm, od, st);
  }
  launch_outer(m, dir, cm, pl, 0, st);
  if (fork) {
    BHG_HIP_CHECK(hipEventRecord(pl.ss->ev_join, pl.ss->side));
    BHG_HIP_CHECK(hipStreamWaitEvent(st, pl.ss->ev_join, 0));
  }
  BHG_HIP_CHECK(hipGetLastError());
  return BHG_OK;
}

int check_mlp(const bhg_mlp* m) {
  BHG_REQUIRE(m, "NULL descriptor");
  BHG_REQUIRE(m->L >= 1 && m->L <= BHG_MLP_MAX_LAYERS, "unsupported layer count");
  BHG_REQUIRE(m->Bp > 0 && m->Bp % kTM == 0 && m->B >= 1 && m->B <= m->Bp, "Bp must be a multiple of 128 rows >= B");
  return BHG_OK;
}

#include "mlp/fx.inc"

}
}

using namespace bhg;

extern "C" {

size_t bhg_mlp_partial_floats(const bhg_mlp* m) {
  if (!m || m->L < 1 || m->L > BHG_MLP_MAX_LAYERS) return 0;
  size_t mx = 0;
  for (int l = 0; l < m->L; ++l) {
    const int Nf = m->dims[l + 1], Kf = m->dims[l];
    const int sf = pick_splits((Nf + skinny_tile_n() - 1) / skinny_tile_n(), Kf, 2);
    mx = mx > (size_t)sf * m->Bp * Nf ? mx : (size_t)sf * m->Bp * Nf;
    int sb = pick_splits((Kf + skinny_tile_n() - 1) / skinny_tile_n(), Nf, 2);
    if (sb < 2) sb = 2;
    mx = mx > (size_t)sb * m->Bp * Kf ? mx : (size_t)sb * m->Bp * Kf;
  }
  return mx;
}

int bhg_mlp_hvp(const bhg_mlp* m, const void* const* dir, void* const* out, void* stream) {
  return bhg_mlp_hvp_mode(m, dir, out, 0, stream);
}

int bhg_mlp_hvp_mode(const bhg_mlp* m, const void* const* dir, void* const* out, int gemm_mode, void* stream) {
  if (int rc = check_mlp(m)) return rc;
  BHG_REQUIRE(gemm_mode >= 0 && gemm_mode <= 3, "gemm_mode is 0 .. 3");
  BHG_REQUIRE(dir && out, "NULL argument");
  BHG_REQUIRE(m->partial && m->partial_floats >= bhg_mlp_partial_floats(m), "split-K scratch too small");
  hipStream_t st = static_cast<hipStream_t>(stream);
  hipEvent_t t_a, t_b;
  const bool timed = span_begin(BHG_TIMING_MLP_HVP, &t_a, &t_b);
  if (timed) BHG_HIP_CHECK(hipEventRecord(t_a, st));
  ChainMode cm{};
  cm.mode = FUSE_NONE;
  cm.out = out;
  cm.gemm_mode = gemm_mode;
  if (int rc = run_chain(m, dir, cm, st)) return rc;
  if (timed) BHG_HIP_CHECK(hipEventRecord(t_b, st));
  return BHG_OK;
}

int64_t bhg_mlp_wsk_launches(void) { return bhg::g_wsk_launches; }
int64_t bhg_mlp_hoist_launches(void) { return bhg::g_hoist_launches; }
int64_t bhg_mlp_proj_iterations(void) { return bhg::g_proj_iterations; }
int64_t bhg_mlp_lin_launches(void) { return bhg::g_lin_launches; }

int bhg_mlp_neumann_mixed_coeff(const bhg_mlp* m, const void* const* v_last, const int64_t* labels, float* coeff, float alpha,
                                int K, int projected, void* fws, size_t fws_bytes, void* stream) {
  BHG_REQUIRE(fws && fws_bytes >= bhg_mlp_fused_ws_bytes(m), "fused workspace too small");
  if (!projected)
    if (int rc = bhg_mlp_mixed_coeff(m, v_last, labels, coeff, stream)) return rc;
  FusedWs w;
  carve_fused_ws(m, fws, &w);
  hipLaunchKernelGGL(k_coeff_from_rzx, dim3((m->Bp + kThreads - 1) / kThreads), dim3(kThreads), 0, static_cast<hipStream_t>(stream),
                     K > 0 ? (const double*)w.rzx : (const double*)nullptr, m->prob, labels, coeff, m->Bp, m->dims[m->L], m->B, -alpha,
                     projected ? 0.f : -alpha);
  BHG_HIP_CHECK(hipGetLastError());
  return BHG_OK;
}

int bhg_mlp_supports_fused_solve(const bhg_mlp* m) {
  const bool off = dbg(DBG_mlp_no_fused_solve, 0) != 0;
  return !off && m && m->L >= 1 && m->L <= BHG_MLP_MAX_LAYERS && m->Bp > 0 && m->Bp % kTM == 0 && use_head(m);
}

void* bhg_mlp_timeout_flag_dev(const bhg_mlp* m, void* fws) {
  if (!m || !fws || m->L < 1 || m->L > BHG_MLP_MAX_LAYERS || m->Bp <= 0) return nullptr;
  FusedWs w;
  carve_fused_ws(m, fws, &w);
  return w.gran + 1;
}

size_t bhg_mlp_fused_ws_bytes(const bhg_mlp* m) {
  if (!m || m->L < 1 || m->L > BHG_MLP_MAX_LAYERS || m->Bp <= 0) return 0;
  FusedWs w;
  carve_fused_ws(m, nullptr, &w);
  return w.bytes;
}

static int solve_common_checks(const bhg_mlp* m, const int64_t* starts, const void* fws, size_t fws_bytes) {
  if (int rc = check_mlp(m)) return rc;
  BHG_REQUIRE(bhg_mlp_supports_fused_solve(m), "fused solve needs a narrow classifier head (<= 256 classes, feature width % 4 == 0)");
  BHG_REQUIRE(starts && fws, "NULL argument");
  BHG_REQUIRE(m->partial && m->partial_floats >= bhg_mlp_partial_floats(m), "split-K scratch too small");
  BHG_REQUIRE(fws_bytes >= bhg_mlp_fused_ws_bytes(m), "fused workspace too small");
  for (int l = 0; l < m->L; ++l) BHG_REQUIRE((starts[2 * l] & 3) == 0, "weight slices of the flat vectors must be 16-byte aligned");
  return BHG_OK;
}

struct CgCtx {
  const bhg_mlp* m; float* x; float* r; float* p; const int64_t* starts; const bhg_chunk* chunks_dev; int n_chunks, K;
  float cg_alpha, shift;
  FusedWs w; double* scal; const double* partR0; int n_init, pgrid, bgrid;
  bool lazy, hoist, lin, lin_head; int proj_level;
  const void* const* rhs;
  BetaArgs ba; HoistPlan hplan;
  const void* dir[2 * BHG_MLP_MAX_LAYERS];
};
static void cg_ctx_init(CgCtx* c, const bhg_mlp* m, float* x, float* r, float* p, const int64_t* starts, const bhg_chunk* chunks_dev,
                        int n_chunks, int K, float cg_alpha, float hvp_shift, void* ws, void* fws, bool global) {
  c->m = m; c->x = x; c->r = r; c->p = p; c->starts = starts; c->chunks_dev = chunks_dev; c->n_chunks = n_chunks; c->K = K;
  c->cg_alpha = cg_alpha; c->shift = hvp_shift; c->rhs = nullptr;
  carve_fused_ws(m, fws, &c->w);
  char* wsb = static_cast<char*>(ws);
  c->scal = reinterpret_cast<double*>(wsb + kWsScal);
  c->partR0 = reinterpret_cast<const double*>(wsb + kWsPartR);
  c->n_init = n_chunks < kMaxBlocks ? n_chunks : kMaxBlocks;
  for (int i = 0; i < 2 * m->L; ++i) c->dir[i] = p + starts[i];
  c->pgrid = n_chunks < kMaxBlocks ? n_chunks : kMaxBlocks;
  const bool eager = dbg(DBG_cg_eager_p, 0) != 0;
  c->lazy = global || !eager;
  BetaArgs& ba = c->ba;
  ba = BetaArgs{};
  int small_total = 0;
  {
    const bool head = use_head(m);
    ba.stride = c->w.nRR; ba.n = c->w.nRR; ba.scal = c->scal; ba.r = r; ba.p = p;
    for (int l = 0; l < m->L; ++l) {
      ba.off[ba.nt] = starts[2 * l + 1]; ba.len[ba.nt] = m->dims[l + 1]; small_total += ba.len[ba.nt]; ++ba.nt;
    }
    if (head) {
      ba.off[ba.nt] = starts[2 * (m->L - 1)]; ba.len[ba.nt] = m->dims[m->L] * m->dims[m->L - 1]; small_total += ba.len[ba.nt]; ++ba.nt;
    }
  }
  c->bgrid = small_total > 0 ? (small_total + kThreads - 1) / kThreads : 1;
  c->hplan.ok = false;
  if (c->lazy && hoist_mode() != 0) hoist_plan(m, &c->hplan);
  c->hoist = c->lazy && c->hplan.ok;
  c->proj_level = (!c->hoist || !c->hplan.proj_ok || proj_mode() == 0 || global) ? 0 : ((proj_mode() == 9 || x) ? 1 : 2);
  c->lin = c->proj_level == 2 && c->hplan.lin_ok && graw_single_on(packed_chain_on(c->w), m->Bp) && rnew_keys_on() &&
           c->ba.nt <= 16 && proj_step_merged() && dbg(DBG_pstep_v2, 1) != 0 && dbg(DBG_lin_first, 1) != 0;
  c->lin_head = c->lin && m->L == 4 && dbg(DBG_lin_update_next, 1) != 0 && dbg(DBG_lin_update_in_head, 1) != 0 && dbg(DBG_lin_nub, 0) == 0 &&
                m->dims[m->L] <= 12 && m->dims[m->L - 1] <= 512 && dbg(DBG_head_no_prefetch, 0) == 0;
}
static int cg_iteration(CgCtx* c, int k, int gphase, double* php, double inv_world, hipStream_t st) {
  const bhg_mlp* m = c->m;
  FusedWs& w = c->w;
  const int K = c->K;
  const bool lazy = c->lazy, hoist = c->hoist;
  hipEvent_t ta, tb, tc, td;
  const bool timed = gphase == 0 && span_begin(BHG_TIMING_MLP_HVP, &ta, &tb);
  const bool timed_it = gphase == 0 && span_begin(BHG_TIMING_MLP_CG_ITER, &tc, &td);
  if (timed_it) BHG_HIP_CHECK(hipEventRecord(tc, st));
  if (lazy && k > 0 && gphase != 2) {
    c->ba.part = w.partRR[k & 1];
    if (!hoist || c->proj_level == 1) hipLaunchKernelGGL(k_cg_beta, dim3(c->bgrid), dim3(kThreads), 0, st, c->ba);
  }
  if (timed) BHG_HIP_CHECK(hipEventRecord(ta, st));
  ChainMode cm{};
  cm.mode = FUSE_CG;
  cm.fa = c->r; cm.fb = c->x; cm.fd = c->p; cm.starts = c->starts;
  cm.shift = c->shift; cm.cg_alpha = c->cg_alpha;
  cm.apply_out = k == K - 1; cm.out_scale = -c->cg_alpha;
  cm.ws = &w; cm.scal = c->scal;
  cm.partRR_old = c->partR0;
  cm.nRR_old = k == 0 ? c->n_init : 0;
  cm.partPP = k == 0 ? c->partR0 : w.partPP;
  cm.nPP = k == 0 ? c->n_init : (lazy ? 0 : c->pgrid);
  cm.partRR_new = w.partRR[(k + 1) & 1];
  cm.lazy = lazy;
  const bool x_every = dbg(DBG_cg_x_every_iter, 0) != 0;
  cm.x_mode = (lazy && !x_every) ? ((k & 1) ? 2 : (k + 1 < K ? 1 : 0)) : 0;
  if (!c->x) cm.x_mode = 1;
  cm.skip_outputs = (!c->x && k == K - 1) ? 1 : 0;
  cm.first = k == 0;
  cm.kpar = k & 1;
  cm.hoist = hoist ? &c->hplan : nullptr;
  cm.beta = &c->ba; cm.beta_blocks = c->bgrid;
  cm.proj = c->proj_level;
  cm.gphase = gphase; cm.php = php; cm.inv_world = inv_world;
  cm.second = k == 1;
  if (c->proj_level == 2 && proj_step_merged())
    c->dir[1] = k == 0 ? static_cast<const void*>(c->p + c->starts[1]) : static_cast<const void*>(w.pb0[k & 1]);
  if (c->lin) c->dir[3] = k == 0 ? static_cast<const void*>(c->p + c->starts[3]) : static_cast<const void*>(w.pb1[k & 1]);
  cm.lin = c->lin ? 1 : 0;
  cm.lin_head = c->lin_head ? 1 : 0;
  cm.rhs = c->rhs;
  if (int rc = run_chain(m, c->dir, cm, st)) return rc;
  if (timed) BHG_HIP_CHECK(hipEventRecord(tb, st));
#ifdef BHG_AB
  if (!lazy && k + 1 < K)
    hipLaunchKernelGGL(k_cg_pdir, dim3(c->pgrid), dim3(kThreads), 0, st, c->chunks_dev, c->n_chunks, (const float*)c->r, c->p,
                       (const double*)w.partRR[(k + 1) & 1], w.nRR, w.partPP, c->scal);
#endif
  if (timed_it) BHG_HIP_CHECK(hipEventRecord(td, st));
  return BHG_OK;
}

int bhg_mlp_cg_solve(const bhg_mlp* m, float* x, float* r, float* p, const int64_t* starts,
                     const bhg_chunk* chunks_dev, int n_chunks, int K, float cg_alpha, float hvp_shift, void* ws,
                     void* fws, size_t fws_bytes, void* stream) {
  return bhg_mlp_cg_solve_rhs(m, x, r, p, starts, chunks_dev, n_chunks, K, cg_alpha, hvp_shift, ws, fws, fws_bytes, nullptr, stream);
}

unsigned long long bhg_mlp_cg_state_mask(const bhg_mlp* m, int has_x) {
  if (!m || m->L < 1 || m->L > BHG_MLP_MAX_LAYERS || 2 * m->L > 64 || has_x || !bhg_mlp_supports_fused_solve(m)) return ~0ull;
  HoistPlan hp;
  hp.ok = false;
  if (dbg(DBG_cg_eager_p, 0) == 0 && hoist_mode() != 0) hoist_plan(m, &hp);
  const bool level2 = hp.ok && hp.proj_ok && proj_mode() != 0 && proj_mode() != 9;
  if (!level2 || dbg(DBG_cg_rhs_direct, 1) == 0) return ~0ull;
  unsigned long long mask = 0ull;
  for (int l = 0; l < m->L; ++l) mask |= 1ull << (2 * l + 1);
  mask |= 1ull << (2 * (m->L - 1));
  return mask;
}

int bhg_mlp_cg_solve_rhs(const bhg_mlp* m, float* x, float* r, float* p, const int64_t* starts,
                         const bhg_chunk* chunks_dev, int n_chunks, int K, float cg_alpha, float hvp_shift, void* ws,
                         void* fws, size_t fws_bytes, const void* const* rhs, void* stream) {
  if (int rc = solve_common_checks(m, starts, fws, fws_bytes)) return rc;
  BHG_REQUIRE(r && p && ws && chunks_dev, "NULL argument");
  BHG_REQUIRE(K >= 0 && n_chunks > 0, "bad size");
  if (K == 0) return BHG_OK;
  hipStream_t st = static_cast<hipStream_t>(stream);
  CgCtx c;
  cg_ctx_init(&c, m, x, r, p, starts, chunks_dev, n_chunks, K, cg_alpha, hvp_shift, ws, fws, false);
  BHG_REQUIRE(!rhs || c.proj_level == 2, "rhs names the right-hand side for the FULLY PROJECTED solver only (see bhg_mlp_cg_state_mask)");
  if (rhs)
    for (int l = 0; l + 1 < m->L; ++l) BHG_REQUIRE(rhs[2 * l] && ((uintptr_t)rhs[2 * l] & 15) == 0, "rhs tensors must be 16-byte aligned device pointers");
  c.rhs = rhs;
  if (c.hoist && packed_chain_on(c.w) && !m->prepacked)
    if (int rc = pack_operands(m, c.w, st)) return rc;
  for (int k = 0; k < K; ++k)
    if (int rc = cg_iteration(&c, k, 0, nullptr, 1.0, st)) return rc;
  BHG_HIP_CHECK(hipGetLastError());
  return BHG_OK;
}

int bhg_mlp_cg_global_phase(const bhg_mlp* m, float* x, float* r, float* p, const int64_t* starts, const bhg_chunk* chunks_dev,
                            int n_chunks, int k, int K, int phase, int world, double* php, float cg_alpha, float hvp_shift,
                            void* ws, void* fws, size_t fws_bytes, void* stream) {
  if (int rc = solve_common_checks(m, starts, fws, fws_bytes)) return rc;
  BHG_REQUIRE(r && p && ws && chunks_dev && php, "NULL argument");
  BHG_REQUIRE(K > 0 && k >= 0 && k < K && n_chunks > 0 && world >= 1, "bad size");
  BHG_REQUIRE(phase == BHG_CG_GLOBAL_CHAIN || phase == BHG_CG_GLOBAL_UPDATE || phase == BHG_CG_GLOBAL_DOTS, "unknown phase");
  hipStream_t st = static_cast<hipStream_t>(stream);
  CgCtx c;
  cg_ctx_init(&c, m, x, r, p, starts, chunks_dev, n_chunks, K, cg_alpha, hvp_shift, ws, fws, true);
  if (phase == BHG_CG_GLOBAL_DOTS) {
    BHG_REQUIRE(k + 1 < K, "the last iteration has no direction update");
    int grid = n_chunks < c.w.nRR ? n_chunks : c.w.nRR;
    if (grid > kMaxBlocks) grid = kMaxBlocks;
    hipLaunchKernelGGL(k_cg_global_dots, dim3(grid), dim3(kThreads), 0, st, chunks_dev, n_chunks, (const float*)r, (const float*)p,
                       c.w.partRR[(k + 1) & 1], c.w.nRR, c.w.nRR);
    BHG_HIP_CHECK(hipGetLastError());
    return BHG_OK;
  }
  if (k == 0 && phase == BHG_CG_GLOBAL_CHAIN && c.hoist && packed_chain_on(c.w) && !m->prepacked)
    if (int rc = pack_operands(m, c.w, st)) return rc;
  if (int rc = cg_iteration(&c, k, phase == BHG_CG_GLOBAL_CHAIN ? 1 : 2, php, 1.0 / (double)world, st)) return rc;
  BHG_HIP_CHECK(hipGetLastError());
  return BHG_OK;
}

int bhg_mlp_fx_supported(const bhg_mlp* m, int world) {
  if (!m || m->L < 1 || m->L > BHG_MLP_MAX_LAYERS || m->Bp <= 0 || m->Bp % kTM != 0 || !bhg_mlp_supports_fused_solve(m)) return 0;
  FxPlan fp;
  fx_plan(m, world, &fp);
  return fp.ok && dbg(DBG_packed_chain, 1) != 0 ? 1 : 0;
}
size_t bhg_mlp_fx_ws_bytes(const bhg_mlp* m, int world) {
  if (!bhg_mlp_fx_supported(m, world)) return 0;
  FxPlan fp; fx_plan(m, world, &fp);
  FxWs x; fx_carve(m, fp, nullptr, &x);
  return x.bytes;
}
size_t bhg_mlp_fx_const_floats(const bhg_mlp* m) {
  if (!bhg_mlp_fx_supported(m, 1)) return 0;
  FxPlan fp; fx_plan(m, 1, &fp);
  return fp.const_floats;
}
size_t bhg_mlp_fx_slab_floats(const bhg_mlp* m) {
  if (!bhg_mlp_fx_supported(m, 1)) return 0;
  FxPlan fp; fx_plan(m, 1, &fp);
  return fp.slab_floats;
}
size_t bhg_mlp_fx_scal_doubles(const bhg_mlp* m) {
  if (!bhg_mlp_fx_supported(m, 1)) return 0;
  FxPlan fp; fx_plan(m, 1, &fp);
  return fp.scal_doubles;
}
static int fx_phase(int algo, const bhg_mlp* m, const void* const* rhs, int k, int K, int phase, int world, int rank, float* const_all,
                    float* slab_all, double* scal_all, float alpha, float hvp_shift, void* fws, size_t fws_bytes, void* xws, size_t xws_bytes,
                    void* stream) {
  if (int rc = check_mlp(m)) return rc;
  const bool neumann = algo == 1;
  BHG_REQUIRE(world >= 1 && rank >= 0 && rank < world, "bad world size / rank");
  BHG_REQUIRE(bhg_mlp_fx_supported(m, world), "this network does not take the factor-exchange form (bhg_mlp_fx_supported)");
  BHG_REQUIRE(phase == BHG_CG_FX_BEGIN || phase == BHG_CG_FX_CHAIN || phase == BHG_CG_FX_GRAM || phase == BHG_CG_FX_END, "unknown phase");
  BHG_REQUIRE(K > 0 && k >= 0 && (k < K || (neumann && k == K && (phase == BHG_CG_FX_CHAIN || phase == BHG_CG_FX_END))), "bad iteration index");
  BHG_REQUIRE(const_all && slab_all && scal_all && fws && xws, "NULL argument");
  BHG_REQUIRE(m->partial && m->partial_floats >= bhg_mlp_partial_floats(m), "split-K scratch too small");
  BHG_REQUIRE(fws_bytes >= bhg_mlp_fused_ws_bytes(m), "fused workspace too small");
  BHG_REQUIRE(xws_bytes >= bhg_mlp_fx_ws_bytes(m, world), "factor-exchange workspace too small");
  hipStream_t st = static_cast<hipStream_t>(stream);
  FxPlan fp;
  fx_plan(m, world, &fp);
  FusedWs w;
  carve_fused_ws(m, fws, &w);
  FxWs x;
  fx_carve(m, fp, xws, &x);
  const bhg_mlp ml = fx_local(m, fp, slab_all, rank);
  double* scal_mine = scal_all + (size_t)rank * fp.scal_doubles;
  if (phase == BHG_CG_FX_BEGIN) {
    BHG_REQUIRE(k == 0, "BEGIN belongs to iteration 0");
    return fx_begin(m, fp, const_all, rank, st);
  }
  if (phase == BHG_CG_FX_CHAIN) {
    if (k == 0) {
      BHG_REQUIRE(rhs, "iteration 0 reads the right-hand side");
      for (int l = 0; l + 1 < m->L; ++l) BHG_REQUIRE(rhs[2 * l] && ((uintptr_t)rhs[2 * l] & 15) == 0, "rhs tensors must be 16-byte aligned device pointers");
      for (int i = 0; i < 2 * m->L; ++i) BHG_REQUIRE(rhs[i], "rhs holds 2 L device pointers");
      if (int rc = fx_first(m, &ml, fp, w, x, rhs, const_all, rank, st, neumann)) return rc;
    } else {
      if (int rc = fx_step(&ml, fp, w, x, scal_all, k - 1, false, alpha, hvp_shift, st, neumann)) return rc;
    }
    return fx_chain(&ml, fp, w, x, k & 1, st, neumann && k == K);
  }
  if (phase == BHG_CG_FX_GRAM) {
    BHG_REQUIRE(k < K, "GRAM belongs to iterations 0 .. K-1");
    return fx_gram(&ml, fp, w, x, slab_all, const_all, scal_mine, k & 1, hvp_shift, st);
  }
  BHG_REQUIRE(k == (neumann ? K : K - 1), "END belongs to the last iteration");
  return fx_step(&ml, fp, w, x, scal_all, k, true, alpha, hvp_shift, st, neumann);
}
int bhg_mlp_cg_fx_phase(const bhg_mlp* m, const void* const* rhs, int k, int K, int phase, int world, int rank, float* const_all,
                        float* slab_all, double* scal_all, float cg_alpha, float hvp_shift, void* fws, size_t fws_bytes, void* xws,
                        size_t xws_bytes, void* stream) {
  return fx_phase(0, m, rhs, k, K, phase, world, rank, const_all, slab_all, scal_all, cg_alpha, hvp_shift, fws, fws_bytes, xws, xws_bytes, stream);
}
int bhg_mlp_neumann_fx_phase(const bhg_mlp* m, const void* const* rhs, int k, int K, int phase, int world, int rank, float* const_all,
                             float* slab_all, double* scal_all, float alpha, float hvp_shift, void* fws, size_t fws_bytes, void* xws,
                             size_t xws_bytes, void* stream) {
  return fx_phase(1, m, rhs, k, K, phase, world, rank, const_all, slab_all, scal_all, alpha, hvp_shift, fws, fws_bytes, xws, xws_bytes, stream);
}

int bhg_mlp_neumann_solve(const bhg_mlp* m, float* v0, float* v1, float* p, const int64_t* starts, int K, float alpha,
                          float hvp_shift, void* fws, size_t fws_bytes, int* projected_out, void* stream) {
  if (int rc = solve_common_checks(m, starts, fws, fws_bytes)) return rc;
  BHG_REQUIRE(v0 && v1, "NULL argument");
  BHG_REQUIRE(K >= 0, "bad size");
  BHG_REQUIRE(p || use_head(m), "the accumulator-free Neumann solver needs the narrow-head kernels");
  hipStream_t st = static_cast<hipStream_t>(stream);
  FusedWs w;
  carve_fused_ws(m, fws, &w);
  HoistPlan hplan;
  hplan.ok = false;
  const bool want_proj = !p && K > 0 && proj_mode() != 0 && hoist_mode() != 0;
  if (hoist_mode() == 2 || want_proj) hoist_plan(m, &hplan);
  const bool proj = want_proj && hplan.ok && hplan.proj_ok && use_head(m);
  if (projected_out) *projected_out = proj ? 1 : 0;
  if (hplan.ok && K > 0 && packed_chain_on(w) && !m->prepacked)
    if (int rc = pack_operands(m, w, st)) return rc;
  for (int k = 0; k < K; ++k) {
    float* vin = (k & 1) ? v1 : v0;
    float* vout = (k & 1) ? v0 : v1;
    const void* dir[2 * BHG_MLP_MAX_LAYERS];
    for (int i = 0; i < 2 * m->L; ++i) dir[i] = vin + starts[i];
    hipEvent_t ta, tb;
    const bool timed = span_begin(BHG_TIMING_MLP_HVP, &ta, &tb);
    if (timed) BHG_HIP_CHECK(hipEventRecord(ta, st));
    ChainMode cm{};
    cm.mode = FUSE_NEUMANN;
    cm.fa = vout; cm.fb = p; cm.fd = vin; cm.starts = starts;
    cm.alpha = alpha; cm.shift = hvp_shift;
    cm.apply_out = k == K - 1; cm.out_scale = -alpha;
    const bool p_every = dbg(DBG_neumann_p_every_iter, 0) != 0;
    cm.x_mode = p_every ? 0 : ((k & 1) ? 2 : (k + 1 < K ? 1 : 0));
    cm.first = k == 0;
    if (!p) { cm.x_mode = 1; cm.rzx_acc = w.rzx; }
    cm.ws = &w;
    cm.hoist = hplan.ok ? &hplan : nullptr;
    cm.proj = proj ? 1 : 0;
    cm.nk = k;
    if (int rc = run_chain(m, dir, cm, st)) return rc;
// ... 146 lines not shown
    launch_reduce_mask(st, m->partial, a.splits, Bp * N, nullptr, m->mask[l - 1], const_cast<float*>(m->delta[l - 1]), Bp,
                       N, B);
  }
  BHG_HIP_CHECK(hipGetLastError());
  return BHG_OK;
}

int bhg_mlp_supports_packed_prepare(const bhg_mlp* m) {
  if (!bhg_mlp_supports_native_prepare(m) || !bhg_mlp_supports_fused_solve(m) || dbg(DBG_packed_prepare, 1) == 0) return 0;
  HoistPlan hp;
  hoist_plan(m, &hp);
  return hp.ok && dbg(DBG_packed_chain, 1) != 0 ? 1 : 0;
}

int bhg_mlp_forward_packed(const bhg_mlp* m, const void* const* bias, const int64_t* labels, float* ce, void* fws, size_t fws_bytes,
                           void* stream) {
  if (int rc = check_head_problem(m)) return rc;
  BHG_REQUIRE(narrow_head(m), "the packed once-per-step passes need a narrow classifier head (<= 256 classes, feature width % 4 == 0)");
  BHG_REQUIRE(bias && labels && ce && fws, "NULL argument");
  BHG_REQUIRE(bhg_mlp_supports_packed_prepare(m), "this network does not take the packed form (bhg_mlp_supports_packed_prepare)");
  BHG_REQUIRE(fws_bytes >= bhg_mlp_fused_ws_bytes(m), "fused workspace too small");
  hipStream_t st = static_cast<hipStream_t>(stream);
  const int L = m->L, Bp = m->Bp, B = m->B;
  FusedWs w;
  carve_fused_ws(m, fws, &w);
  if (int rc = pack_operands(m, w, st, true)) return rc;
  {
    const int K = m->dims[0], N = m->dims[1];
    GemmArgs a{};
    a.pr[0] = {m->h[0], m->W[0], K, K};
    a.pairs = 1;
    a.M = Bp; a.N = N; a.K = K;
    const int tn = skinny_tile_n();
    a.splits = pick_splits((N + tn - 1) / tn, K, 1);
    a.out = m->partial; a.ldo = N; a.out_rows = Bp;
    launch_gemm<LAYOUT_KC, LAYOUT_KC>(a, tn, st);
    launch_reduce_mask(st, m->partial, a.splits, Bp * N, static_cast<const float*>(bias[0]), nullptr, const_cast<float*>(m->h[1]), Bp, N, B,
                       const_cast<float*>(m->mask[0]), w.hpk[1]);
  }
  for (int l = 1; l + 1 < L; ++l) {
    WskpfArgs f{};
    WskpProb& q = f.a;
    q.Ap = w.hpk[l]; q.Bq = w.Wf[l]; q.RA = Bp; q.RB = m->dims[l + 1]; q.K = m->dims[l]; q.B = B; q.nsplit = 1;
    q.bias = static_cast<const float*>(bias[l]);
    q.out = const_cast<float*>(m->h[l + 1]);
    q.outp = l + 2 < L ? w.hpk[l + 1] : nullptr;
    f.relu_mask = const_cast<float*>(m->mask[l]);
    wskp_tiling(&q, false);
    const int blk = q.nfull * (q.RB / 32) + q.nstrip;
    hipLaunchKernelGGL(k_wskpf<2>, dim3(blk), dim3(64 * kWskpWaves), 0, st, f);
  }
  launch_head_forward(st, Bp, nullptr, m->h[L - 1], m->W[L - 1] , m->W[L - 1], static_cast<const float*>(bias[L - 1]),
                      nullptr, nullptr, const_cast<float*>(m->prob), m->dims[L - 1], m->dims[L], B, HEAD_LOGITS, labels, ce, nullptr,
                      nullptr, nullptr);
  BHG_HIP_CHECK(hipGetLastError());
  return BHG_OK;
}

int bhg_mlp_backward_packed(const bhg_mlp* m, const int64_t* labels, void* fws, size_t fws_bytes, void* stream) {
  if (int rc = check_head_problem(m)) return rc;
  BHG_REQUIRE(narrow_head(m), "the packed once-per-step passes need a narrow classifier head (<= 256 classes, feature width % 4 == 0)");
  BHG_REQUIRE(labels && fws, "NULL argument");
  BHG_REQUIRE(bhg_mlp_supports_packed_prepare(m), "this network does not take the packed form (bhg_mlp_supports_packed_prepare)");
  BHG_REQUIRE(fws_bytes >= bhg_mlp_fused_ws_bytes(m), "fused workspace too small");
  hipStream_t st = static_cast<hipStream_t>(stream);
  const int L = m->L, Bp = m->Bp, B = m->B;
  const int C = m->dims[L];
  FusedWs w;
  carve_fused_ws(m, fws, &w);
  hipLaunchKernelGGL(k_delta_top, dim3((Bp * C + 255) / 256), dim3(256), 0, st, m->prob, m->sd, labels,
                     const_cast<float*>(m->delta[L - 1]), Bp, C, B);
  {
    const int l = L - 1, K = m->dims[l + 1], N = m->dims[l];
    const int blocks = (Bp * (N / 4) + 255) / 256;
    hipLaunchKernelGGL(k_head_backward, dim3(blocks), dim3(256), 0, st, (const float*)nullptr, m->delta[l], m->W[l],
                       (const float*)nullptr, m->mask[l - 1], const_cast<float*>(m->delta[l - 1]), N, K, B, Bp, w.dpk[l - 1]);
  }
  for (int l = L - 2; l >= 1; --l) {
    WskpBuilder wb;
    WskpProb q{};
    q.Ap = w.dpk[l]; q.Bq = w.Wb[l]; q.RA = Bp; q.RB = m->dims[l]; q.K = m->dims[l + 1]; q.B = B; q.nsplit = 1;
    q.mask = m->mask[l - 1]; q.out = const_cast<float*>(m->delta[l - 1]);
    q.outp = l >= 2 ? w.dpk[l - 1] : nullptr;
    wb.add(q);
    wb.launch(st);
  }
  BHG_HIP_CHECK(hipGetLastError());
  return BHG_OK;
}

__global__ __launch_bounds__(256) void k_stage_batch(const float* __restrict__ x, const int64_t* __restrict__ y, float* __restrict__ h0,
                                                     int64_t* __restrict__ labels, int64_t n4, int B) {
  for (int64_t i = (int64_t)blockIdx.x * 256 + threadIdx.x; i < n4; i += (int64_t)gridDim.x * 256)
    reinterpret_cast<float4*>(h0)[i] = reinterpret_cast<const float4*>(x)[i];
  if (blockIdx.x == 0)
    for (int b = threadIdx.x; b < B; b += 256) labels[b] = y[b];
}
int bhg_mlp_stage_batch(const bhg_mlp* m, const float* x, const int64_t* y, int64_t* labels, void* stream) {
  if (int rc = check_mlp(m)) return rc;
  BHG_REQUIRE(x && y && labels && m->h[0], "NULL argument");
  BHG_REQUIRE((m->dims[0] & 3) == 0 && ((uintptr_t)x & 15) == 0, "the input batch must be 16-byte aligned with a width that is a multiple of 4");
  const int64_t n4 = (int64_t)m->B * m->dims[0] / 4;
  int blocks = (int)((n4 + 255) / 256);
  if (blocks > 2048) blocks = 2048;
  if (blocks < 1) blocks = 1;
  hipLaunchKernelGGL(k_stage_batch, dim3(blocks), dim3(256), 0, static_cast<hipStream_t>(stream), x, y, const_cast<float*>(m->h[0]), labels, n4, m->B);
  BHG_HIP_CHECK(hipGetLastError());
  return BHG_OK;
}

int bhg_mlp_mixed_coeff(const bhg_mlp* m, const void* const* dir, const int64_t* labels, float* coeff, void* stream) {
  if (int rc = check_head_problem(m)) return rc;
  BHG_REQUIRE(dir && labels && coeff, "NULL argument");
  hipStream_t st = static_cast<hipStream_t>(stream);
  const int L = m->L, Bp = m->Bp, B = m->B;
  for (int l = 0; l < L; ++l) {
    const int K = m->dims[l], N = m->dims[l + 1];
    const float* V = static_cast<const float*>(dir[2 * l]);
    const float* c = static_cast<const float*>(dir[2 * l + 1]);
    if (l == L - 1 && narrow_head(m)) {
      launch_head_forward(st, Bp, l > 0 ? (const float*)m->Rh[l - 1] : nullptr, m->h[l], m->W[l], V, c, m->prob, nullptr,
                          nullptr, K, N, B, HEAD_COEFF, labels, coeff, nullptr, nullptr, nullptr);
      break;
    }
    GemmArgs a{};
    a.pr[0] = {m->h[l], V, K, K};
    a.pairs = 1;
    if (l > 0) { a.pr[1] = {m->Rh[l - 1], m->W[l], K, K}; a.pairs = 2; }
    a.M = Bp; a.N = N; a.K = K;
    const int tn = skinny_tile_n();
    a.splits = pick_splits((N + tn - 1) / tn, K, a.pairs);
    a.out = m->partial; a.ldo = N; a.out_rows = Bp;
    launch_gemm<LAYOUT_KC, LAYOUT_KC>(a, tn, st);
    if (l == L - 1) {
      launch_reduce_mask(st, m->partial, a.splits, Bp * N, c, nullptr, m->Rd[l], Bp, N, B);
      hipLaunchKernelGGL(k_coeff_rows, dim3(Bp), dim3(kThreads), 0, st, m->prob, (const float*)m->Rd[l], labels, coeff, N, B);
      break;
    }
    launch_reduce_mask(st, m->partial, a.splits, Bp * N, c, m->mask[l], m->Rh[l], Bp, N, B);
  }
  BHG_HIP_CHECK(hipGetLastError());
  return BHG_OK;
}

int bhg_mlp_plan_describe(const bhg_mlp* m, int algo, int keep_solution, char* buf, size_t buf_bytes) {
  if (int rc = check_mlp(m)) return rc;
  BHG_REQUIRE(buf && buf_bytes >= 64, "output buffer too small");
  BHG_REQUIRE(algo == 0 || algo == 1, "algo: 0 = cg, 1 = neumann");
  const int L = m->L;
  const bool fused = bhg_mlp_supports_fused_solve(m) != 0;
  HoistPlan hp;
  hoist_plan(m, &hp);
  const char* form = "unfused";
  int hoist = 0, proj_level = 0, lin = 0, lin_head = 0, upd_first = 0;
  const char* closing = "k_outer_all";
  if (fused) {
    int64_t numel[2 * BHG_MLP_MAX_LAYERS], starts[2 * BHG_MLP_MAX_LAYERS];
    for (int l = 0; l < L; ++l) { numel[2 * l] = (int64_t)m->dims[l] * m->dims[l + 1]; numel[2 * l + 1] = m->dims[l + 1]; }
    const int64_t nch = bhg_layout_num_chunks(numel, 2 * L);
    std::vector<bhg_chunk> chunks((size_t)(nch > 0 ? nch : 1));
    if (int rc = bhg_layout_build(numel, 2 * L, starts, chunks.data())) return rc;
    float* const fake = reinterpret_cast<float*>((uintptr_t)1 << 30);
    if (algo == 0) {
      static CgCtx c;
      cg_ctx_init(&c, m, keep_solution ? fake : nullptr, fake, fake, starts, nullptr, (int)nch, 2, 1.f, 0.f, fake, fake, false);
      hoist = c.hoist ? 1 : 0; proj_level = c.proj_level; lin = c.lin ? 1 : 0; lin_head = c.lin_head ? 1 : 0;
      upd_first = (c.lin && L > 4) ? 1 : 0;
      form = !c.lazy ? "classic-eager" : (!c.hoist ? "classic" : (c.proj_level == 0 ? "hoisted" : (c.proj_level == 1 ? "projected-keep-state" :
             (c.lin ? (c.lin_head ? "six-launch (k_wskpl .. k_headu .. k_graw)" : "six-launch-class (k_wskpl first, recurrences beside the chain)") :
              "fully-projected (k_pstep launch)"))));
      if (c.proj_level >= 1) closing = graw_batch_ok(m->Bp) ? (m->Bp == 128 ? "k_graw" : "k_grawk") : "k_hoist+k_proj_update";
    } else {
      const bool want_proj = !keep_solution && proj_mode() != 0 && hoist_mode() != 0;
      const bool proj = want_proj && hp.ok && hp.proj_ok && use_head(m);
      hoist = (hp.ok && (hoist_mode() == 2 || want_proj)) ? 1 : 0;
      proj_level = proj ? 1 : 0;
      form = proj ? "projected-neumann (update inside k_graw)" : (hoist ? "hoisted" : "classic");
      if (proj) closing = graw_batch_ok(m->Bp) ? (m->Bp == 128 ? "k_graw" : "k_grawk") : "k_hoist+k_proj_update";
    }
  }
  size_t gram = 0;
  if (hp.ok && hp.proj_ok)
    for (int l = 0; l + 1 < L; ++l) gram += (size_t)m->Bp * m->Bp * (l >= 1 ? (2 + 2 * kGramSplitMax + 6) : 2);
  const int n = snprintf(buf, buf_bytes,
                         "algo=%s keep_solution=%d fused=%d form=\"%s\" hoist=%d proj_level=%d lin=%d lin_head=%d upd_first=%d closing=%s "
                         "plan_ok=%d proj_ok=%d lin_ok=%d hoist_products=%d hoist_wgs=%d gram_floats=%zu fused_ws_bytes=%zu narrow_head=%d packed_prepare=%d "
                         "global_form=%s fx_slab_bytes=%zu fx_ws_bytes_world8=%zu",
                         algo == 0 ? "cg" : "neumann", keep_solution ? 1 : 0, fused ? 1 : 0, form, hoist, proj_level, lin, lin_head, upd_first, closing,
                         hp.ok ? 1 : 0, hp.proj_ok ? 1 : 0, hp.lin_ok ? 1 : 0, hp.n, hp.ok ? hp.blk0[hp.n] : 0, gram,
                         fused ? bhg_mlp_fused_ws_bytes(m) : (size_t)0, narrow_head(m) ? 1 : 0, bhg_mlp_supports_packed_prepare(m),
                         (algo == 0 && !keep_solution && bhg_mlp_fx_supported(m, 1)) ? "factor-exchange" : (fused ? "one-pass" : "sharded"),
                         sizeof(float) * bhg_mlp_fx_slab_floats(m), bhg_mlp_fx_ws_bytes(m, 8));
  BHG_REQUIRE(n > 0 && (size_t)n < buf_bytes, "output buffer too small");
  return BHG_OK;
}

#ifdef BHG_STAMPS
static unsigned long long* g_stamps_dev = nullptr;
int bhg_debug_stamps_enable(int on) {
  const size_t bytes = sizeof(unsigned long long) * bhg::kStampKernels * bhg::kStampBlocks * bhg::kStampSlots;
  if (on && !g_stamps_dev) {
    BHG_HIP_CHECK(hipMalloc(&g_stamps_dev, bytes));
  }
  if (g_stamps_dev) BHG_HIP_CHECK(hipMemset(g_stamps_dev, 0, bytes));
  unsigned long long* p = on ? g_stamps_dev : nullptr;
  BHG_HIP_CHECK(hipMemcpyToSymbol(HIP_SYMBOL(bhg::d_stamps), &p, sizeof(p)));
  return BHG_OK;
}
int bhg_debug_stamps_read(unsigned long long* host, size_t count) {
  BHG_REQUIRE(g_stamps_dev && host, "stamps are not enabled");
  const size_t total = (size_t)bhg::kStampKernels * bhg::kStampBlocks * bhg::kStampSlots;
  BHG_HIP_CHECK(hipDeviceSynchronize());
  BHG_HIP_CHECK(hipMemcpy(host, g_stamps_dev, sizeof(unsigned long long) * (count < total ? count : total), hipMemcpyDeviceToHost));
  return BHG_OK;
}
#endif

}

#ifndef BHG_LAYOUT_PAD
#define BHG_LAYOUT_PAD 8
#endif
namespace bhg {
namespace {
#define BHG_STR2(x) #x
#define BHG_STR(x) BHG_STR2(x)
__global__ __attribute__((aligned(16384))) void k_layout_anchor() {
#if BHG_LAYOUT_PAD > 0
  asm volatile(".rept " BHG_STR(BHG_LAYOUT_PAD) " * 64 - 8\n s_nop 0\n .endr");
#endif
}
}
}
```

betty_amd/csrc/mlp/chain_plan.inc:

```

struct ChainMode {
  int mode;
  void* const* out;
  float* fa; float* fb; float* fd;
  const int64_t* starts;
  float alpha, shift, out_scale;
  int apply_out;
  FusedWs* ws;
  const double* partRR_old; int nRR_old;
  const double* partPP; int nPP;
  double* partRR_new;
  double* scal;
  float cg_alpha;
  int kpar;
  int x_mode;
  int first;
  int lazy;
  double* rzx_acc;
  int skip_outputs;
  int gemm_mode;
  const HoistPlan* hoist;
  const BetaArgs* beta; int beta_blocks;
  int proj;
  int stop_after_head;
  int gphase; double* php; double inv_world;
  int second;
  int lin;
  int nk;
  const void* const* rhs;
  int lin_head;
};

struct ChainPlan {
  int L;
  float rho2;
  bool cg;
  bool no_fuse, no_outer_all;
  bool single;
  bool no_side;
  bool head;
  SideState* ss;
  int tn, wsk;
  FuseArgs fbase;
  int part_base_w[BHG_MLP_MAX_LAYERS], part_base_bias;
  const HoistPlan* hp;
  float* hoist;
  float* rh0;
  bool do_chain;
  bool proj_iter;
  bool packed, gram_in_chain;
  bool graw_single, graw2;
  bool rnew;
  bool vnew;
  bool lin, lin_head;

  float* rh0_slot(int k) const { return (k & 1) ? hoist + hp->rh0alt_off : rh0; }
  float* gp1(int par) const { return hoist + (par ? hp->gp1alt_off : hp->g_off[hp->gf[1]]); }
  float* gp2(int par) const { return hoist + (par ? hp->gp2alt_off : hp->g_off[hp->gf[L - 2]]); }
  int gram_slabs(int K) const { return gram_in_chain ? 1 : gram_ksplit(K); }
};

struct ChainState {
  HeadFuse head_fuse{};
  bool fuse_head = false;
  PstepArgs lin_ps{};
  int lin_nu = 0, lin_U = 4;
  bool lin_update_pending = false;
  bool sd_in_chain = false;
};

int plan_chain(const bhg_mlp* m, const ChainMode& cm, ChainPlan* p) {
  const int L = m->L;
  *p = ChainPlan{};
  p->L = L;
  p->rho2 = cm.mode == FUSE_NONE ? m->ridge2 : 0.f;
  const bool cg = p->cg = cm.mode == FUSE_CG;
  const bool no_side_env = dbg(DBG_mlp_no_side, 0) != 0;
  p->no_fuse = dbg(DBG_mlp_no_fuse, 0) != 0;
  p->no_outer_all = dbg(DBG_mlp_no_outer_all, 0) != 0;
  const bool neumann_side = dbg(DBG_neumann_side, 0) != 0;
  p->single = cg || (cm.mode == FUSE_NEUMANN && !neumann_side && !p->no_outer_all);
  p->no_side = no_side_env || p->single;
  p->head = use_head(m);
  BHG_REQUIRE(!cg || p->head, "the fused CG solver needs the narrow-head kernels");
  if (int rc = side_state(&p->ss)) return rc;
  p->tn = skinny_tile_n();
  p->wsk = wsk_mode(cm.mode, cm.gemm_mode);

  FuseArgs& fbase = p->fbase;
  fbase.scal = cm.scal; fbase.part = cm.partRR_new; fbase.alpha = cm.alpha; fbase.shift = cm.shift;
  fbase.out_scale = cm.out_scale; fbase.apply_out = cm.apply_out;
  fbase.part_stride = cg ? cm.ws->nRR : 0;
  fbase.kpar = cm.kpar;
  int base = 0;
  for (int l = 0; l < L; ++l) { p->part_base_w[l] = base; base += outer_blocks(m, l, p->head); }
  p->part_base_bias = base;

  const HoistPlan* hp = p->hp = ((cg && cm.lazy) || (cm.mode == FUSE_NEUMANN && p->single)) ? cm.hoist : nullptr;
  p->hoist = hp ? cm.ws->hoist : nullptr;
  p->rh0 = m->Rh[0];
  p->do_chain = cm.gphase != 2;
  p->proj_iter = hp && cm.proj && (cg ? (!cm.apply_out && !cm.skip_outputs) : true);
  p->packed = hp && packed_chain_on(*cm.ws);
  p->gram_in_chain = p->packed && p->proj_iter && !cm.stop_after_head && dbg(DBG_packed_gram, 1) != 0;
  p->graw_single = graw_single_on(p->packed, m->Bp);
  p->graw2 = p->gram_in_chain && p->graw_single;
  p->rnew = p->graw_single && cg && cm.proj >= 2 && cm.gphase == 0 && rnew_keys_on();
  p->vnew = cm.mode == FUSE_NEUMANN && hp && cm.proj && p->graw_single && L >= 3 && dbg(DBG_neumann_vnew, 1) != 0;
  p->lin = cm.lin != 0;
  BHG_REQUIRE(!p->lin || (p->rnew && hp && hp->lin_ok && cm.beta && cm.beta->nt <= 16 && proj_step_merged() && L >= 4),
              "the linear first product was planned for a solve that cannot run it");
  p->lin_head = p->lin && cm.lin_head != 0;
  return BHG_OK;
}

FuseArgs fuse_at(const ChainMode& cm, const ChainPlan& pl, int tensor, int part_base) {
  FuseArgs f = pl.fbase;
  if (cm.mode != FUSE_NONE) {
    const int64_t o = cm.starts[tensor];
    f.a = cm.fa + o; f.b = cm.fb ? cm.fb + o : nullptr; f.d = cm.fd + o;
    f.lazy = cm.lazy && (tensor & 1) == 0 && !(pl.head && tensor == 2 * (pl.L - 1));
    f.x_mode = (f.lazy || cm.mode == FUSE_NEUMANN) ? cm.x_mode : 0;
    if (!cm.fb) f.x_mode = 1;
  }
  f.part_base = part_base;
  return f;
}
```

betty_amd/csrc/mlp/head_body.inc:

```
#if !BHG_HEAD_LAZY
  kernarg_warm<256>();
#endif
  extern __shared__ __attribute__((aligned(16))) float srow[];
  __shared__ float t1s[kSmallC];
  __shared__ double red_t[kWaves];
  __shared__ float rz[kSmallC], rdl[kSmallC], dtl[kSmallC], pz[kSmallC];
  const int b = BHG_HEAD_B;
  const int t = threadIdx.x;
  const int lane = t & 63, wave = t >> 6;
  if (b >= B) {
    if (mode != HEAD_COEFF && t < C) rd[(int64_t)b * C + t] = 0.f;
    if (mode != HEAD_JVP && t == 0) aux[b] = 0.f;
    if (mode == HEAD_JVP && rd_prev)
      for (int k = 4 * t; k < K; k += 1024) {
        *reinterpret_cast<float4*>(rd_prev + (int64_t)b * K + k) = make_float4(0.f, 0.f, 0.f, 0.f);
        if (rd_prev_p) *reinterpret_cast<float4*>(rd_prev_p + ((int64_t)(k >> 4) * BHG_HEAD_ROWS + b) * 16 + (k & 15)) = make_float4(0.f, 0.f, 0.f, 0.f);
      }
    if (FUSED)
      for (int k = 4 * t; k < K; k += 1024) *reinterpret_cast<float4*>(fz.rh_out + (int64_t)b * K + k) = make_float4(0.f, 0.f, 0.f, 0.f);
    return;
  }
  const float* hb = h + (int64_t)b * K;
  float acc[JMAX], cbv[JMAX];
  const float* vrow[JMAX];
  const float* wrow[JMAX];
#pragma unroll
  for (int j = 0; j < JMAX; ++j) {
    const int cc = min(wave + 4 * j, C - 1);
    acc[j] = 0.f;
    vrow[j] = V + (int64_t)cc * K;
    wrow[j] = W + (int64_t)cc * K;
    cbv[j] = cb[cc];
  }
  float4 pf_h[2], pf_v[2][JMAX], pf_w[2][JMAX];
  float pf_p = 0.f, pf_sd = 0.f, pf_dt = 0.f;
  if (PF) {
#pragma unroll
    for (int tr = 0; tr < 2; ++tr) {
      const int k = 4 * lane + 256 * tr;
      const int kc = k < K ? k : 0;
      pf_h[tr] = ld16(hb + kc);
#pragma unroll
      for (int j = 0; j < JMAX; ++j) {
        pf_v[tr][j] = ld16(vrow[j] + kc);
        pf_w[tr][j] = ld16(wrow[j] + kc);
      }
    }
    const int tc = t < C ? t : C - 1;
    pf_p = prob[(int64_t)b * C + tc];
    pf_sd = sd[b];
    pf_dt = delta_top[(int64_t)b * C + tc];
  }
  if (FUSED) {
    for (int k = 4 * t; k < K; k += 1024) {
      const float* p0 = fz.part + (int64_t)b * K + k;
      const float4 bv = ld16(fz.bias + k);
      const float4 mv = ld16(fz.mask + (int64_t)b * K + k);
      float4 v = make_float4(0.f, 0.f, 0.f, 0.f);
      constexpr int NB = PF ? 16 : 8;
      for (int s0 = 0; s0 < fz.splits; s0 += NB) {
        float4 tt[NB];
#pragma unroll
        for (int u = 0; u < NB; ++u) tt[u] = ld16(p0 + (int64_t)(s0 + u < fz.splits ? s0 + u : fz.splits - 1) * fz.slab);
#pragma unroll
        for (int u = 0; u < NB; ++u)
          if (s0 + u < fz.splits) { v.x += tt[u].x; v.y += tt[u].y; v.z += tt[u].z; v.w += tt[u].w; }
      }
      if (fz.addend) {
        float4 ad = ld16(fz.addend + (int64_t)b * K + k);
#if BHG_HEAD_LAZY
        if (lazy_addend2) {
          const float4 a2 = ld16(lazy_addend2 + (int64_t)b * K + k);
          ad.x = add_rn(ad.x, mul_rn(lazy_beta, a2.x)); ad.y = add_rn(ad.y, mul_rn(lazy_beta, a2.y));
          ad.z = add_rn(ad.z, mul_rn(lazy_beta, a2.z)); ad.w = add_rn(ad.w, mul_rn(lazy_beta, a2.w));
        }
#endif
        v.x += ad.x; v.y += ad.y; v.z += ad.z; v.w += ad.w;
      }
      v.x = (v.x + bv.x) * mv.x; v.y = (v.y + bv.y) * mv.y; v.z = (v.z + bv.z) * mv.z; v.w = (v.w + bv.w) * mv.w;
      *reinterpret_cast<float4*>(srow + k) = v;
      *reinterpret_cast<float4*>(fz.rh_out + (int64_t)b * K + k) = v;
    }
    __syncthreads();
  }
  const float* rhb = HAS_RH ? (FUSED ? srow : Rh + (int64_t)b * K) : nullptr;
  float4 pf_mk, pf_W[12], pf_V[12];
  if (PF) {
    const int kd = 4 * t < K ? 4 * t : 0;
    pf_mk = ld16(mask_prev + (int64_t)b * K + kd);
#pragma unroll
    for (int c = 0; c < 12; ++c) {
      const int cc = min(c, C - 1);
      pf_W[c] = ld16(W + (int64_t)cc * K + kd);
      pf_V[c] = ld16(V + (int64_t)cc * K + kd);
    }
#pragma unroll
    for (int tr = 0; tr < 2; ++tr) {
      const int k = 4 * lane + 256 * tr;
      if (k < K) {
        const float4 hv = pf_h[tr];
        float4 rv = make_float4(0.f, 0.f, 0.f, 0.f);
        if (HAS_RH) rv = *reinterpret_cast<const float4*>(rhb + k);
#pragma unroll
        for (int j = 0; j < JMAX; ++j) {
          float a = acc[j];
          const float4 vv = pf_v[tr][j], ww = pf_w[tr][j];
          a = fmaf(hv.x, vv.x, a); a = fmaf(hv.y, vv.y, a); a = fmaf(hv.z, vv.z, a); a = fmaf(hv.w, vv.w, a);
          if (HAS_RH) {
            a = fmaf(rv.x, ww.x, a); a = fmaf(rv.y, ww.y, a); a = fmaf(rv.z, ww.z, a); a = fmaf(rv.w, ww.w, a);
          }
          acc[j] = a;
        }
      }
    }
  }
  for (int k = 4 * lane; k < (PF ? 0 : K); k += 256) {
    const float4 hv = *reinterpret_cast<const float4*>(hb + k);
    float4 rv = make_float4(0.f, 0.f, 0.f, 0.f);
    if (HAS_RH) rv = *reinterpret_cast<const float4*>(rhb + k);
    float4 vv[JMAX], ww[JMAX];
#pragma unroll
    for (int j = 0; j < JMAX; ++j) {
      vv[j] = *reinterpret_cast<const float4*>(vrow[j] + k);
      if (HAS_RH) ww[j] = *reinterpret_cast<const float4*>(wrow[j] + k);
    }
#pragma unroll
    for (int j = 0; j < JMAX; ++j) {
      float a = acc[j];
      a = fmaf(hv.x, vv[j].x, a); a = fmaf(hv.y, vv[j].y, a); a = fmaf(hv.z, vv[j].z, a); a = fmaf(hv.w, vv[j].w, a);
      if (HAS_RH) {
        a = fmaf(rv.x, ww[j].x, a); a = fmaf(rv.y, ww[j].y, a); a = fmaf(rv.z, ww[j].z, a); a = fmaf(rv.w, ww[j].w, a);
      }
      acc[j] = a;
    }
  }
#pragma unroll
  for (int j = 0; j < JMAX; ++j) {
    const int c = wave + 4 * j;
    const float a = wave_sum_f32(acc[j]);
    if (lane == 0 && c < C) rz[c] = a + cbv[j];
  }
  for (int cbase = 4 * JMAX; cbase < C; cbase += 4 * JMAX) {
    float acc2[JMAX], cb2[JMAX];
    const float* v2[JMAX];
    const float* w2[JMAX];
#pragma unroll
    for (int j = 0; j < JMAX; ++j) {
      const int cc = min(cbase + wave + 4 * j, C - 1);
      acc2[j] = 0.f;
      v2[j] = V + (int64_t)cc * K;
      w2[j] = W + (int64_t)cc * K;
      cb2[j] = cb[cc];
    }
    for (int k = 4 * lane; k < K; k += 256) {
      const float4 hv = *reinterpret_cast<const float4*>(hb + k);
      float4 rv = make_float4(0.f, 0.f, 0.f, 0.f);
      if (HAS_RH) rv = *reinterpret_cast<const float4*>(rhb + k);
      float4 vv[JMAX], ww[JMAX];
#pragma unroll
      for (int j = 0; j < JMAX; ++j) {
        vv[j] = *reinterpret_cast<const float4*>(v2[j] + k);
        if (HAS_RH) ww[j] = *reinterpret_cast<const float4*>(w2[j] + k);
      }
#pragma unroll
      for (int j = 0; j < JMAX; ++j) {
        float a = acc2[j];
        a = fmaf(hv.x, vv[j].x, a); a = fmaf(hv.y, vv[j].y, a); a = fmaf(hv.z, vv[j].z, a); a = fmaf(hv.w, vv[j].w, a);
        if (HAS_RH) {
          a = fmaf(rv.x, ww[j].x, a); a = fmaf(rv.y, ww[j].y, a); a = fmaf(rv.z, ww[j].z, a); a = fmaf(rv.w, ww[j].w, a);
        }
        acc2[j] = a;
      }
    }
#pragma unroll
    for (int j = 0; j < JMAX; ++j) {
      const int c = cbase + wave + 4 * j;
      const float a = wave_sum_f32(acc2[j]);
      if (lane == 0 && c < C) rz[c] = a + cb2[j];
    }
  }
  __syncthreads();
  if (mode == HEAD_JVP) {
    float p = 0.f, sdv = 0.f, dt = 0.f;
    if (rz_out && t < C) rz_out[(int64_t)b * C + t] = rz[t];
    if (rzx_acc && t < C) rzx_acc[(int64_t)b * C + t] = (rzx_first ? 0.0 : rzx_acc[(int64_t)b * C + t]) + (double)rz[t];
    if (t < C) {
      if (PF) { p = pf_p; sdv = pf_sd; dt = pf_dt; }
      else {
        p = prob[(int64_t)b * C + t];
        sdv = sd[b];
        if (rd_prev) dt = delta_top[(int64_t)b * C + t];
      }
      pz[t] = p * rz[t];
    }
    __syncthreads();
    if (t < C) {
      float dot = 0.f;
      for (int c = 0; c < C; ++c) dot += pz[c];
      const float v = sdv * (p * rz[t] - p * dot);
      rd[(int64_t)b * C + t] = v;
      rdl[t] = v;
      dtl[t] = dt;
      t1s[t] = rz[t] * v;
    }
    if (rd_prev || partT1) __syncthreads();
    if (partT1 && t == 0) {
      double s1 = 0.0;
      for (int c = 0; c < C; ++c) s1 += (double)t1s[c];
      partT1[b] = s1;
    }
    double dacc = 0.0;
    if (PF) {
      const int k = 4 * t;
      if (k < K) {
        float4 acc2 = make_float4(0.f, 0.f, 0.f, 0.f);
        float4 accd = make_float4(0.f, 0.f, 0.f, 0.f);
#pragma unroll
        for (int c = 0; c < 12; ++c) {
          if (c < C) {
            const float r = rdl[c], d = dtl[c];
            const float4 v = pf_V[c], w = pf_W[c];
            acc2.x += d * v.x + r * w.x; acc2.y += d * v.y + r * w.y;
            acc2.z += d * v.z + r * w.z; acc2.w += d * v.w + r * w.w;
            accd.x += d * v.x; accd.y += d * v.y; accd.z += d * v.z; accd.w += d * v.w;
          }
        }
        acc2.x *= pf_mk.x; acc2.y *= pf_mk.y; acc2.z *= pf_mk.z; acc2.w *= pf_mk.w;
        *reinterpret_cast<float4*>(rd_prev + (int64_t)b * K + k) = acc2;
        if (rd_prev_p) *reinterpret_cast<float4*>(rd_prev_p + ((int64_t)(k >> 4) * BHG_HEAD_ROWS + b) * 16 + (k & 15)) = acc2;
        if (HAS_RH && partT2h) {
          const float4 rh4 = *reinterpret_cast<const float4*>(rhb + k);
          dacc += (double)accd.x * rh4.x + (double)accd.y * rh4.y + (double)accd.z * rh4.z + (double)accd.w * rh4.w;
        }
      }
    } else if (rd_prev) {
      for (int k = 4 * t; k < K; k += 1024) {
        const float4 mk = *reinterpret_cast<const float4*>(mask_prev + (int64_t)b * K + k);
// ... 72 lines not shown
```

include/bhg.h:

```cpp
#ifndef BHG_H_
#define BHG_H_

#include <stddef.h>
#include <stdint.h>

#ifdef __cplusplus
extern "C" {
#endif

#define BHG_VERSION 1
#define BHG_CHUNK_ELEMS 4096
#define BHG_FLAT_ALIGN 64

#define BHG_OK 0
#define BHG_ERR_ARG (-1)
#define BHG_ERR_HIP (-2)
#define BHG_ERR_WS (-3)
#define BHG_ERR_CAPACITY (-4)

typedef struct bhg_chunk {
  int64_t flat_off;
  int64_t src_off;
  int32_t tensor;
  int32_t len;
// ... 12 lines not shown
int bhg_scatter(const float* flat, void* const* dst, int T, const bhg_chunk* chunks_dev,
                int n_chunks, float scale, void* ws, void* stream);

int bhg_neumann_init(const void* const* vec, int T, const bhg_chunk* chunks_dev, int n_chunks,
                     float* v, float* p, void* ws, void* stream);
int bhg_neumann_step(const void* const* hvp, int T, const bhg_chunk* chunks_dev, int n_chunks,
                     float* v, float* p, float alpha, float out_scale, float hvp_shift, void* ws,
                     void* stream);

#define BHG_CG_AUTO 0
#define BHG_CG_STREAM 1
#define BHG_CG_RESIDENT 2
int bhg_cg_init(const void* const* vec, int T, const bhg_chunk* chunks_dev, int n_chunks,
                float* x, float* r, float* p, void* ws, void* stream);
int bhg_cg_init_masked(const void* const* vec, int T, const bhg_chunk* chunks_dev, int n_chunks,
                       float* x, float* r, float* p, unsigned long long keep_mask, void* ws, void* stream);
int bhg_cg_step(const void* const* hvp, int T, const bhg_chunk* chunks_dev, int n_chunks,
                float* x, float* r, float* p, float cg_alpha, int iter, float out_scale,
                float hvp_shift , int variant,
                void* ws, void* stream);
int bhg_cg_resident_capacity_chunks(void);
int bhg_cg_resident_ok(void);
int bhg_cg_resident_usable(int n_chunks);
const double* bhg_cg_scalars_dev(const void* ws);
const unsigned* bhg_cg_timeout_flag_dev(const void* ws);

int bhg_cg_phase(int phase, const void* const* hvp, int T, const bhg_chunk* chunks_dev, int n_chunks, float* x,
                 float* r, float* p, float cg_alpha, int iter, float out_scale, float hvp_shift, void* ws, void* stream);
double* bhg_cg_partials_dev(void* ws, int which, int iter);
int bhg_cg_partials_count(void);

int bhg_scale_flat(float* flat, int64_t n, float scale, void* stream);

int bhg_darts_eps(const void* const* vec, int T, const bhg_chunk* chunks_dev, int n_chunks,
                  double R, double* out_dev, float* eps_f32_dev, void* ws, void* stream);
int bhg_axpy_multi(void* const* dst, const void* const* src, int T, const bhg_chunk* chunks_dev,
                   int n_chunks, const float* coef_dev, float mul, void* ws, void* stream);

int bhg_fd_perturb(void* const* w, const float* w0_flat, const void* const* dir, int T, const bhg_chunk* chunks_dev,
                   int n_chunks, const float* eps_dev, float sign, void* ws, void* stream);
int bhg_cg_step_fd(const void* const* grad_plus, const void* const* grad_minus, const float* two_eps_dev, int T,
                   const bhg_chunk* chunks_dev, int n_chunks, float* x, float* r, float* p, float cg_alpha, int iter,
                   float out_scale, float hvp_shift, int variant, void* ws, void* stream);
int bhg_neumann_step_fd(const void* const* grad_plus, const void* const* grad_minus, const float* two_eps_dev, int T,
                        const bhg_chunk* chunks_dev, int n_chunks, float* v, float* p, float alpha, float out_scale,
                        float hvp_shift, void* ws, void* stream);

int bhg_sama_adam_precondition(const void* const* vec, const void* const* last_grad,
                               const void* const* exp_avg, const void* const* exp_avg_sq, int T,
                               const bhg_chunk* chunks_dev, int n_chunks, float* out_flat,
                               double beta1, double beta2, double eps, double lr, void* ws, void* stream);

int bhg_debug_set(const char* key, int value);
int bhg_debug_unset(const char* key);
void bhg_debug_reset(void);
int bhg_debug_key_count(void);
const char* bhg_debug_key_name(int i);
int bhg_is_ab_build(void);

#define BHG_TIMING_CG_STEP 0
#define BHG_TIMING_NEUMANN_STEP 1
#define BHG_TIMING_MLP_HVP 2
#define BHG_TIMING_MLP_CG_ITER 3
int bhg_timing_enable(int on);
int bhg_timing_read(int kind, double* total_ms, int* launches);

int bhg_logreg_prepare(const float* X, const float* w, float* s, int n, int d, void* stream);
size_t bhg_logreg_tmp_floats(int n, int d);
int bhg_logreg_hvp(const float* X, const float* s, const float* lam, const float* p, float* out,
                   float* tmp, int n, int d, void* stream);

int bhg_logreg_solve_plan(int n, int d, int form, int strips, char* buf, size_t buf_bytes);
size_t bhg_logreg_solve_ws_bytes(int n, int d);
int bhg_logreg_cg_solve(const float* X, const float* w, const float* lam, const float* rhs, float* out, float* coeff, void* ws,
                        int n, int d, int K, float cg_alpha, float out_scale, int form, int strips, void* stream);
int bhg_logreg_neumann_solve(const float* X, const float* w, const float* lam, const float* rhs, float* out, float* coeff, void* ws,
                             int n, int d, int K, float alpha, float out_scale, int form, int strips, void* stream);

#define BHG_MLP_MAX_LAYERS 32
typedef struct bhg_mlp {
  int32_t L, B, Bp;
  int32_t dims[BHG_MLP_MAX_LAYERS + 1];
  const float* W[BHG_MLP_MAX_LAYERS];
  const float* h[BHG_MLP_MAX_LAYERS];
  const float* mask[BHG_MLP_MAX_LAYERS];
  const float* delta[BHG_MLP_MAX_LAYERS];
  const float* prob;
  const float* sd;
  float* Rh[BHG_MLP_MAX_LAYERS];
  float* Rd[BHG_MLP_MAX_LAYERS];
  float* partial;
  size_t partial_floats;
  float ridge2;
  int32_t prepacked;
} bhg_mlp;
size_t bhg_mlp_partial_floats(const bhg_mlp* m);
int bhg_mlp_hvp(const bhg_mlp* m, const void* const* dir, void* const* out, void* stream);
int bhg_mlp_hvp_mode(const bhg_mlp* m, const void* const* dir, void* const* out, int gemm_mode, void* stream);

int bhg_mlp_supports_native_prepare(const bhg_mlp* m);
int bhg_mlp_forward(const bhg_mlp* m, const void* const* bias, const int64_t* labels, float* ce, void* stream);
int bhg_mlp_backward(const bhg_mlp* m, const int64_t* labels, void* stream);
int bhg_mlp_mixed_coeff(const bhg_mlp* m, const void* const* dir, const int64_t* labels, float* coeff, void* stream);

int bhg_mlp_supports_fused_solve(const bhg_mlp* m);
size_t bhg_mlp_fused_ws_bytes(const bhg_mlp* m);
int bhg_mlp_cg_solve(const bhg_mlp* m, float* x, float* r, float* p, const int64_t* starts,
                     const bhg_chunk* chunks_dev, int n_chunks, int K, float cg_alpha, float hvp_shift, void* ws,
                     void* fws, size_t fws_bytes, void* stream);
int bhg_mlp_neumann_solve(const bhg_mlp* m, float* v0, float* v1, float* p, const int64_t* starts, int K,
                          float alpha, float hvp_shift, void* fws, size_t fws_bytes, int* projected_out, void* stream);
#define BHG_CG_GLOBAL_CHAIN 0
#define BHG_CG_GLOBAL_UPDATE 1
#define BHG_CG_GLOBAL_DOTS 2
int bhg_mlp_cg_global_phase(const bhg_mlp* m, float* x, float* r, float* p, const int64_t* starts, const bhg_chunk* chunks_dev,
                            int n_chunks, int k, int K, int phase, int world, double* php, float cg_alpha, float hvp_shift,
                            void* ws, void* fws, size_t fws_bytes, void* stream);
#define BHG_CG_FX_BEGIN 0
#define BHG_CG_FX_CHAIN 1
#define BHG_CG_FX_GRAM 2
#define BHG_CG_FX_END 3
int bhg_mlp_fx_supported(const bhg_mlp* m, int world);
size_t bhg_mlp_fx_ws_bytes(const bhg_mlp* m, int world);
size_t bhg_mlp_fx_const_floats(const bhg_mlp* m);
size_t bhg_mlp_fx_slab_floats(const bhg_mlp* m);
size_t bhg_mlp_fx_scal_doubles(const bhg_mlp* m);
int bhg_mlp_cg_fx_phase(const bhg_mlp* m, const void* const* rhs, int k, int K, int phase, int world, int rank, float* const_all,
                        float* slab_all, double* scal_all, float cg_alpha, float hvp_shift, void* fws, size_t fws_bytes, void* xws,
                        size_t xws_bytes, void* stream);
int bhg_mlp_neumann_fx_phase(const bhg_mlp* m, const void* const* rhs, int k, int K, int phase, int world, int rank, float* const_all,
                             float* slab_all, double* scal_all, float alpha, float hvp_shift, void* fws, size_t fws_bytes, void* xws,
                             size_t xws_bytes, void* stream);
unsigned long long bhg_mlp_cg_state_mask(const bhg_mlp* m, int has_x);
int bhg_mlp_cg_solve_rhs(const bhg_mlp* m, float* x, float* r, float* p, const int64_t* starts, const bhg_chunk* chunks_dev,
                         int n_chunks, int K, float cg_alpha, float hvp_shift, void* ws, void* fws, size_t fws_bytes,
                         const void* const* rhs, void* stream);
int bhg_mlp_cg_mixed_coeff(const bhg_mlp* m, const int64_t* labels, float* coeff, float cg_alpha, void* fws,
                           size_t fws_bytes, void* stream);
int64_t bhg_mlp_wsk_launches(void);
int64_t bhg_mlp_hoist_launches(void);
int64_t bhg_mlp_proj_iterations(void);
int64_t bhg_mlp_lin_launches(void);
int bhg_mlp_neumann_mixed_coeff(const bhg_mlp* m, const void* const* v_last, const int64_t* labels, float* coeff,
                                float alpha, int K, int projected, void* fws, size_t fws_bytes, void* stream);

int bhg_mlp_stage_batch(const bhg_mlp* m, const float* x, const int64_t* y, int64_t* labels, void* stream);
int bhg_mlp_supports_packed_prepare(const bhg_mlp* m);
int bhg_mlp_forward_packed(const bhg_mlp* m, const void* const* bias, const int64_t* labels, float* ce, void* fws, size_t fws_bytes,
                           void* stream);
int bhg_mlp_backward_packed(const bhg_mlp* m, const int64_t* labels, void* fws, size_t fws_bytes, void* stream);

void* bhg_mlp_timeout_flag_dev(const bhg_mlp* m, void* fws);

int bhg_mwn_max_hidden(void);
int bhg_mwn_forward(const float* ce, int B, const float* w1, const float* b1, const float* w2, const float* b2, int H, float* s,
                    float* sd, void* stream);
int bhg_mwn_backward(const float* ce, const float* coeff, int B, const float* w1, const float* b1, const float* w2, const float* b2,
                     int H, float scale, float* gw1, float* gb1, float* gw2, float* gb2, void* stream);

int bhg_mlp_plan_describe(const bhg_mlp* m, int algo, int keep_solution, char* buf, size_t buf_bytes);

int bhg_copy2d(float* dst, int64_t ldd, const float* src, int64_t lds, int64_t rows, int64_t cols, void* stream);

size_t bhg_bn_ws_bytes(int C);
int bhg_bn_backward_vjp(const float* x, const float* gy, const float* a, const float* gamma, const float* mean, const float* invstd,
                        const float* b, const float* c, int N, int C, int HW, float* dx, float* dgy, float* dgamma, void* ws,
                        size_t ws_bytes, void* stream);

size_t bhg_mlp_fd_ws_bytes(const int* dims, int L, int B);
int bhg_mlp_fd_forward(const float* x, const int64_t* labels, int B, const int* dims, int L, void* const* params, const void* const* dir,
                       const float* eps_dev, int restore, float* ce_plus, float* ce_minus, void* ws, size_t ws_bytes, void* stream);
int bhg_mwn_fd_vjp(const float* ce_plus, const float* ce_minus, int B, const float* w1, const float* b1, const float* w2, const float* b2,
                   int H, const float* two_eps_dev, int accumulate, float* gw1, float* gb1, float* gw2, float* gb2, void* stream);

int bhg_quad_fd(void* const* w, const void* const* dir, void* const* out, int T, const bhg_chunk* chunks_dev, int n_chunks,
                const float* eps_dev, float scale, int mode, int restore, int accumulate, void* stream);

#ifdef __cplusplus
}
#endif
#endif
```

Before: 767.9.

## Precompute head Jacobian J once per solve and fuse it into a new k_headj kernel

Before the CG iterations, a product J = (W3 masked) × W2 is built once per solve from weights that stay fixed. A new k_headj kernel then computes the head's contribution directly as Rh1·J and fuses the layer-3 tile GEMM, its reduction and the update blocks into one launch. This replaces the split-K partial GEMM and the separate reduction in the head path. The cost is extra workspace, a packing pass and a GEMM at setup, and a new, large and complex code path that only applies to L=4 nets with a narrow head.

```diff
diff --git a/betty_amd/_native.py b/betty_amd/_native.py
--- a/betty_amd/_native.py
+++ b/betty_amd/_native.py
@@ -170,6 +170,7 @@
     ),
     "bhg_mlp_cg_mixed_coeff": (c_int, [POINTER(Mlp), c_void_p, c_void_p, c_float, c_void_p, c_size_t, c_void_p]),
     "bhg_mlp_timeout_flag_dev": (c_void_p, [POINTER(Mlp), c_void_p]),
+    "bhg_mlp_head_j_dev": (c_void_p, [POINTER(Mlp), c_void_p, POINTER(c_int), POINTER(c_int)]),
     "bhg_mlp_stage_batch": (c_int, [POINTER(Mlp), c_void_p, c_void_p, c_void_p, c_void_p]),
     "bhg_mlp_supports_packed_prepare": (c_int, [POINTER(Mlp)]),
     "bhg_mlp_forward_packed": (c_int, [POINTER(Mlp), _PP, c_void_p, c_void_p, c_void_p, c_size_t, c_void_p]),
diff --git a/betty_amd/csrc/bhg_common.hpp b/betty_amd/csrc/bhg_common.hpp
--- a/betty_amd/csrc/bhg_common.hpp
+++ b/betty_amd/csrc/bhg_common.hpp
@@ -36,7 +36,7 @@
   X(mlp_hoist) X(hoist_wgs) X(proj_step_alone) X(mlp_no_side) X(mlp_no_fuse) X(mlp_no_outer_all) X(neumann_side)             \
   X(hoist_staged_mink) X(proj_alpha_alone) X(proj_small_alone) X(outer_order_by_work) X(outer_no_pre) X(outer_stagger)       \
   X(mlp_no_fused_solve) X(cg_eager_p) X(cg_x_every_iter) X(neumann_p_every_iter) X(head_no_prefetch) X(cg_spin_limit)        \
-  X(packed_chain) X(packed_depth) X(packed_gram) X(proj_max_ratio) X(proj_ws_cap_mb) X(alpha_in_hoist) X(graw_v2) X(wskp_ragged) X(pstep_v2) X(pstep_unroll) X(rnew_in_graw) X(graw_cols) X(lin_first) X(lin_prio) X(lin_nub) X(lin_order) X(lin_update_next) X(lin_withhold_beta) X(neumann_vnew) X(cg_rhs_direct) X(packed_prepare) X(lin_deep) X(graw_kloop) X(lin_update_in_head) X(xcd_pairs) X(headu_head_first) X(fx_ksplit)
+  X(packed_chain) X(packed_depth) X(packed_gram) X(proj_max_ratio) X(proj_ws_cap_mb) X(alpha_in_hoist) X(graw_v2) X(wskp_ragged) X(pstep_v2) X(pstep_unroll) X(rnew_in_graw) X(graw_cols) X(lin_first) X(lin_prio) X(lin_nub) X(lin_order) X(lin_update_next) X(lin_withhold_beta) X(neumann_vnew) X(cg_rhs_direct) X(packed_prepare) X(lin_deep) X(graw_kloop) X(lin_update_in_head) X(xcd_pairs) X(headu_head_first) X(fx_ksplit) X(head_j) X(head_j_tile)
 enum DbgKey : int {
 #define BHG_DBG_ENUM(n) DBG_##n,
   BHG_DBG_KEYS(BHG_DBG_ENUM)
diff --git a/betty_amd/csrc/bhg_mlp.hip b/betty_amd/csrc/bhg_mlp.hip
--- a/betty_amd/csrc/bhg_mlp.hip
+++ b/betty_amd/csrc/bhg_mlp.hip
@@ -3,6 +3,7 @@
 
 
 #include "bhg_common.hpp"
+#include "bhg_mlp_headj.hpp"
 
 #ifdef BHG_STAMPS
 namespace bhg { __device__ unsigned long long* d_stamps = nullptr; }
@@ -506,8 +507,13 @@
   float* dpk[BHG_MLP_MAX_LAYERS];
   float* Rhp[BHG_MLP_MAX_LAYERS];
   float* Rdp[BHG_MLP_MAX_LAYERS];
+  float* hj_J; float* hj_Ap; int nT2j;
   size_t bytes;
 };
+inline bool headj_shape_ok(const bhg_mlp* m, const HoistPlan& hp) {
+  return hp.ok && hp.lin_ok && m->L == 4 && m->dims[m->L] <= 12 && m->dims[m->L - 1] <= 512 && m->Bp == 128;
+}
+inline int headj_rows(int rows_valid, int C) { return (rows_valid * C + 31) & ~31; }
 void carve_fused_ws(const bhg_mlp* m, void* base, FusedWs* w) {
   memset(w, 0, sizeof(*w));
   const bool head = use_head(m);
@@ -524,11 +530,13 @@
   int nt2 = 0;
   for (int l = 1; l + 1 < m->L; ++l) { w->t2_off[l] = nt2; nt2 += reduce_blocks(m->Bp * m->dims[l], m->dims[l]); }
   w->nT2 = nt2;
-  w->partT2 = static_cast<double*>(take(sizeof(double) * (nt2 > 0 ? nt2 : 1)));
+  HoistPlan hp;
+  hoist_plan(m, &hp);
+  const bool hj = headj_shape_ok(m, hp);
+  w->nT2j = hj ? headj_tiles(m->Bp, m->dims[m->L - 1], 1) : 0;
+  w->partT2 = static_cast<double*>(take(sizeof(double) * (nt2 + w->nT2j > 0 ? nt2 + w->nT2j : 1)));
   w->rz = static_cast<float*>(take(sizeof(float) * (size_t)m->Bp * m->dims[m->L]));
   w->rzx = static_cast<double*>(take(sizeof(double) * (size_t)m->Bp * m->dims[m->L]));
-  HoistPlan hp;
-  hoist_plan(m, &hp);
   w->hoist = static_cast<float*>(take(sizeof(float) * (hp.ok ? hp.floats : 1)));
   w->part_dot = static_cast<double*>(take(sizeof(double) * 2 * (hp.ok ? hp.dot_blocks : 1)));
   w->part_raw = static_cast<double*>(take(sizeof(double) * (hp.ok ? hp.raw_blocks : 1)));
@@ -551,6 +559,11 @@
       }
     }
   }
+  if (hj) {
+    const size_t rj = (size_t)headj_rows(m->Bp, m->dims[m->L]);
+    w->hj_J = static_cast<float*>(take(sizeof(float) * rj * m->dims[m->L - 2]));
+    w->hj_Ap = static_cast<float*>(take(sizeof(float) * rj * m->dims[m->L - 1]));
+  }
   w->bytes = off;
 }
 
@@ -582,6 +595,20 @@
   BHG_REQUIRE(ok, "too many layers for one packing launch");
   g.blk0[g.n] = blk;
   hipLaunchKernelGGL(k_pack, dim3(blk), dim3(256), 0, st, g);
+  BHG_HIP_CHECK(hipGetLastError());
+  return BHG_OK;
+}
+
+int build_head_j(const bhg_mlp* m, const FusedWs& w, hipStream_t st) {
+  const int L = m->L, C = m->dims[L], K = m->dims[L - 1], N = m->dims[L - 2], RA = headj_rows(m->B, C);
+  BHG_REQUIRE(w.nT2j > 0 && w.hj_J && w.hj_Ap && w.Wb[L - 2], "the head_j form was planned for a net it cannot take");
+  if (int rc = launch_headj_pack(m->W[L - 1], m->mask[L - 2], w.hj_Ap, m->B, C, K, RA, st)) return rc;
+  WskpBuilder wb;
+  WskpProb q{};
+  q.Ap = w.hj_Ap; q.Bq = w.Wb[L - 2]; q.RA = RA; q.RB = N; q.K = K; q.B = m->B * C; q.nsplit = 1;
+  q.out = w.hj_J;
+  wb.add(q);
+  wb.launch(st);
   BHG_HIP_CHECK(hipGetLastError());
   return BHG_OK;
 }
@@ -815,6 +842,12 @@
         if (sp > cap) sp = cap;
         if (sp > K / 64) sp = K / 64;
         if (sp < 1) sp = 1;
+        if (pl.head_j && cs->lin_update_pending) {
+          cs->head_fuse = {nullptr, 0, Bp * N, c, m->mask[l], m->Rh[l], hbase + hp->gr_off[hp->gf[l]]};
+          cs->fuse_head = true;
+          cs->head_j = true;
+          continue;
+        }
         q.nsplit = sp; q.raw = 1; q.out = m->partial;
         cs->head_fuse = {m->partial, sp, Bp * N, c, m->mask[l], m->Rh[l], (pl.lin_head && !cm.first) ? hbase + hp->gr_off[hp->gf[l]] : Gf};
         cs->fuse_head = true;
@@ -873,7 +906,27 @@
 
 int hoist_head(const bhg_mlp* m, const void* const* dir, const ChainMode& cm, const ChainPlan& pl, hipStream_t st, ChainState* cs) {
   const int L = m->L, Bp = m->Bp, B = m->B;
-  if (cs->lin_update_pending) {
+  if (cs->lin_update_pending && cs->head_j) {
+    const int l = L - 1, K = m->dims[l], N = m->dims[l + 1];
+    BHG_REQUIRE(cs->fuse_head && pl.cg && pl.packed && cm.ws->nT2j > 0 && !cm.rzx_acc, "k_headj was planned for a head it cannot run");
+    HeadjLaunch a{};
+    a.h = m->h[l]; a.W = m->W[l]; a.V = static_cast<const float*>(dir[2 * l]); a.cb = static_cast<const float*>(dir[2 * l + 1]);
+    a.prob = m->prob; a.sd = m->sd; a.rd = m->Rd[l];
+    a.K = K; a.C = N; a.B = B; a.rows = Bp;
+    a.delta_top = (const float*)m->delta[l]; a.mask_prev = (const float*)m->mask[l - 1]; a.rd_prev = m->Rd[l - 1]; a.rd_prev_p = cm.ws->Rdp[l - 1];
+    a.partT1 = cm.ws->partT1; a.rz_out = cm.ws->rz;
+    a.bias2 = cs->head_fuse.bias; a.mask2 = cs->head_fuse.mask; a.addend = cs->head_fuse.addend;
+    a.addend2 = pl.gp2(cm.kpar ^ 1); a.gran = cm.ws->gran;
+    a.J = cm.ws->hj_J; a.Rh1 = m->Rh[l - 2]; a.K1 = m->dims[l - 1];
+    a.Rh1p = cm.ws->Rhp[l - 2]; a.W2p = cm.ws->Wf[l - 1]; a.rh_out = m->Rh[l - 1];
+    a.tile_shape = dbg(DBG_head_j_tile, kHeadjTile);
+    const int nt = headj_tiles(Bp, K, a.tile_shape);
+    if (nt <= B) { a.partT2 = cm.ws->partT2h; a.t2n = B; cs->head_j_nt = 0; }
+    else { a.partT2 = cm.ws->partT2 + cm.ws->nT2; a.t2n = nt; cs->head_j_nt = nt; }
+    a.ps = &cs->lin_ps; a.ps_bytes = sizeof(cs->lin_ps); a.nu = cs->lin_ps.h.update_blocks;
+    if (int rc = launch_headj(a, st)) return rc;
+    cs->lin_update_pending = false;
+  } else if (cs->lin_update_pending) {
     const int l = L - 1, K = m->dims[l], N = m->dims[l + 1];
     BHG_REQUIRE(cs->fuse_head && pl.cg && pl.packed && N <= 12 && K <= 512, "k_headu was planned for a head it cannot run");
     HeaduArgs ha{};
@@ -1417,6 +1470,10 @@
   if (pl.do_chain && !pl.hp) chain_forward(m, dir, cm, pl, st, &cs);
   ChainOutputs od;
   describe_outputs(m, dir, cm, pl, &od);
+  if (cs.head_j && cs.head_j_nt > 0) {
+    od.aa.partT2h = nullptr;
+    od.aa.nT2 = cm.ws->nT2 + cs.head_j_nt;
+  }
   if (pl.do_chain && !pl.hp)
     if (int rc = chain_backward(m, dir, cm, pl, st)) return rc;
 
@@ -1531,6 +1588,16 @@
   return w.gran + 1;
 }
 
+const float* bhg_mlp_head_j_dev(const bhg_mlp* m, void* fws, int* rows, int* cols) {
+  if (!m || m->L < 1 || m->L > BHG_MLP_MAX_LAYERS || m->Bp <= 0 || !fws) return nullptr;
+  FusedWs w;
+  carve_fused_ws(m, fws, &w);
+  if (w.nT2j == 0) return nullptr;
+  if (rows) *rows = headj_rows(m->B, m->dims[m->L]);
+  if (cols) *cols = m->dims[m->L - 2];
+  return w.hj_J;
+}
+
 size_t bhg_mlp_fused_ws_bytes(const bhg_mlp* m) {
   if (!m || m->L < 1 || m->L > BHG_MLP_MAX_LAYERS || m->Bp <= 0) return 0;
   FusedWs w;
@@ -1552,7 +1619,7 @@
   const bhg_mlp* m; float* x; float* r; float* p; const int64_t* starts; const bhg_chunk* chunks_dev; int n_chunks, K;
   float cg_alpha, shift;
   FusedWs w; double* scal; const double* partR0; int n_init, pgrid, bgrid;
-  bool lazy, hoist, lin, lin_head; int proj_level;
+  bool lazy, hoist, lin, lin_head, head_j; int proj_level;
   const void* const* rhs;
   BetaArgs ba; HoistPlan hplan;
   const void* dir[2 * BHG_MLP_MAX_LAYERS];
@@ -1592,6 +1659,7 @@
            c->ba.nt <= 16 && proj_step_merged() && dbg(DBG_pstep_v2, 1) != 0 && dbg(DBG_lin_first, 1) != 0;
   c->lin_head = c->lin && m->L == 4 && dbg(DBG_lin_update_next, 1) != 0 && dbg(DBG_lin_update_in_head, 1) != 0 && dbg(DBG_lin_nub, 0) == 0 &&
                 m->dims[m->L] <= 12 && m->dims[m->L - 1] <= 512 && dbg(DBG_head_no_prefetch, 0) == 0;
+  c->head_j = c->lin_head && c->w.nT2j > 0 && dbg(DBG_head_j, 1) != 0;
 }
 static int cg_iteration(CgCtx* c, int k, int gphase, double* php, double inv_world, hipStream_t st) {
   const bhg_mlp* m = c->m;
@@ -1635,6 +1703,7 @@
   if (c->lin) c->dir[3] = k == 0 ? static_cast<const void*>(c->p + c->starts[3]) : static_cast<const void*>(w.pb1[k & 1]);
   cm.lin = c->lin ? 1 : 0;
   cm.lin_head = c->lin_head ? 1 : 0;
+  cm.head_j = c->head_j ? 1 : 0;
   cm.rhs = c->rhs;
   if (int rc = run_chain(m, c->dir, cm, st)) return rc;
   if (timed) BHG_HIP_CHECK(hipEventRecord(tb, st));
@@ -1682,6 +1751,8 @@
   c.rhs = rhs;
   if (c.hoist && packed_chain_on(c.w) && !m->prepacked)
     if (int rc = pack_operands(m, c.w, st)) return rc;
+  if (c.head_j && K >= 2)
+    if (int rc = build_head_j(m, c.w, st)) return rc;
   for (int k = 0; k < K; ++k)
     if (int rc = cg_iteration(&c, k, 0, nullptr, 1.0, st)) return rc;
   BHG_HIP_CHECK(hipGetLastError());
@@ -2134,7 +2205,7 @@
   HoistPlan hp;
   hoist_plan(m, &hp);
   const char* form = "unfused";
-  int hoist = 0, proj_level = 0, lin = 0, lin_head = 0, upd_first = 0;
+  int hoist = 0, proj_level = 0, lin = 0, lin_head = 0, upd_first = 0, head_j = 0;
   const char* closing = "k_outer_all";
   if (fused) {
     int64_t numel[2 * BHG_MLP_MAX_LAYERS], starts[2 * BHG_MLP_MAX_LAYERS];
@@ -2146,7 +2217,7 @@
     if (algo == 0) {
       static CgCtx c;
       cg_ctx_init(&c, m, keep_solution ? fake : nullptr, fake, fake, starts, nullptr, (int)nch, 2, 1.f, 0.f, fake, fake, false);
-      hoist = c.hoist ? 1 : 0; proj_level = c.proj_level; lin = c.lin ? 1 : 0; lin_head = c.lin_head ? 1 : 0;
+      hoist = c.hoist ? 1 : 0; proj_level = c.proj_level; lin = c.lin ? 1 : 0; lin_head = c.lin_head ? 1 : 0; head_j = c.head_j ? 1 : 0;
       upd_first = (c.lin && L > 4) ? 1 : 0;
       form = !c.lazy ? "classic-eager" : (!c.hoist ? "classic" : (c.proj_level == 0 ? "hoisted" : (c.proj_level == 1 ? "projected-keep-state" :
              (c.lin ? (c.lin_head ? "six-launch (k_wskpl .. k_headu .. k_graw)" : "six-launch-class (k_wskpl first, recurrences beside the chain)") :
@@ -2167,12 +2238,12 @@
   const int n = snprintf(buf, buf_bytes,
                          "algo=%s keep_solution=%d fused=%d form=\"%s\" hoist=%d proj_level=%d lin=%d lin_head=%d upd_first=%d closing=%s "
                          "plan_ok=%d proj_ok=%d lin_ok=%d hoist_products=%d hoist_wgs=%d gram_floats=%zu fused_ws_bytes=%zu narrow_head=%d packed_prepare=%d "
-                         "global_form=%s fx_slab_bytes=%zu fx_ws_bytes_world8=%zu",
+                         "global_form=%s fx_slab_bytes=%zu fx_ws_bytes_world8=%zu head_j=%d",
                          algo == 0 ? "cg" : "neumann", keep_solution ? 1 : 0, fused ? 1 : 0, form, hoist, proj_level, lin, lin_head, upd_first, closing,
                          hp.ok ? 1 : 0, hp.proj_ok ? 1 : 0, hp.lin_ok ? 1 : 0, hp.n, hp.ok ? hp.blk0[hp.n] : 0, gram,
                          fused ? bhg_mlp_fused_ws_bytes(m) : (size_t)0, narrow_head(m) ? 1 : 0, bhg_mlp_supports_packed_prepare(m),
                          (algo == 0 && !keep_solution && bhg_mlp_fx_supported(m, 1)) ? "factor-exchange" : (fused ? "one-pass" : "sharded"),
-                         sizeof(float) * bhg_mlp_fx_slab_floats(m), bhg_mlp_fx_ws_bytes(m, 8));
+                         sizeof(float) * bhg_mlp_fx_slab_floats(m), bhg_mlp_fx_ws_bytes(m, 8), head_j);
   BHG_REQUIRE(n > 0 && (size_t)n < buf_bytes, "output buffer too small");
   return BHG_OK;
 }
diff --git a/betty_amd/csrc/bhg_mlp_headj.hip b/betty_amd/csrc/bhg_mlp_headj.hip
--- /dev/null
+++ b/betty_amd/csrc/bhg_mlp_headj.hip
@@ -0,0 +1,224 @@
+#include <stdlib.h>
+
+#include "bhg_mlp_headj.hpp"
+
+#ifdef BHG_STAMPS
+#undef BHG_STAMP
+#define BHG_STAMP(kid, slot) do { } while (0)
+#endif
+
+namespace bhg {
+namespace {
+#include "mlp/gemm.inc"
+#include "mlp/outer.inc"
+#include "mlp/scalars.inc"
+#include "mlp/head.inc"
+#include "mlp/wsk.inc"
+#include "mlp/wskp.inc"
+#include "mlp/recurrence.inc"
+#include "mlp/proj.inc"
+#include "mlp/pstep.inc"
+
+struct HeadjArgs {
+  const float* h; const float* W; const float* V; const float* cb; const float* prob; const float* sd; float* rd;
+  int K, C, B, rows;
+  const float* delta_top; const float* mask_prev; float* rd_prev; float* rd_prev_p;
+  HeadFuse fz;
+  double* partT1; float* rz_out;
+  const float* addend2;
+  const unsigned long long* gran;
+  const float* J; const float* Rh1; int K1;
+  const float* Rh1p; const float* W2p; double* partT2;
+  int nt, nu;
+  int t2n;
+  alignas(64) PstepArgs ps;
+};
+static_assert(offsetof(HeadjArgs, ps) % 64 == 0 && sizeof(HeadjArgs) <= 3900, "kernel arguments of k_headj");
+
+constexpr int kHjC = 12;
+
+template <int RBLK, int CBLK>
+__device__ __forceinline__ void headj_tile(const HeadjArgs& g, const int t, float* __restrict__ sPf, float* __restrict__ sD,
+                                           float* __restrict__ sV, double* __restrict__ red) {
+  constexpr int TR = 16 * RBLK, TC = 16 * CBLK, TCP = TC + 1;
+  static_assert(kWskpWaves * TR * TCP <= kWskpLds && TR <= 32 && TC <= 32 && (TR * TC) % (64 * kWskpWaves) == 0, "four partial tiles");
+  const int RA = g.rows, RB = g.K, KT = g.K1, B = g.B, C = g.C;
+  const int ntm = RA / TR, ntn = RB / TC;
+  int tm = t % ntm, tn = t / ntm;
+  if ((ntn & 7) == 0) { const int j = t >> 3; tm = j % ntm; tn = (j / ntm) * 8 + (t & 7); }
+  const int m0 = TR * tm, n0 = TC * tn;
+  const int lane = threadIdx.x & 63;
+  const int wave = __builtin_amdgcn_readfirstlane(threadIdx.x >> 6);
+  const int li = lane & 15, lk = lane >> 4;
+  const int nct = KT / 32;
+  const int c0 = (int)(((int64_t)wave * nct) / kWskpWaves), c1 = (int)(((int64_t)(wave + 1) * nct) / kWskpWaves);
+  const int nch_w = c1 - c0;
+  f32x4 acc[RBLK][CBLK];
+#pragma unroll
+  for (int a = 0; a < RBLK; ++a)
+#pragma unroll
+    for (int b = 0; b < CBLK; ++b)
+#pragma unroll
+      for (int r = 0; r < 4; ++r) acc[a][b][r] = 0.f;
+  constexpr int kOutPer = TR * TC / (64 * kWskpWaves);
+  float e_mask[kOutPer], e_bias[kOutPer], e_add[kOutPer], e_add2[kOutPer];
+#pragma unroll
+  for (int u = 0; u < kOutPer; ++u) {
+    const int e = threadIdx.x + 64 * kWskpWaves * u;
+    const int64_t idx = (int64_t)(m0 + e / TC) * RB + n0 + (e % TC);
+    e_mask[u] = g.fz.mask[idx];
+    e_bias[u] = g.fz.bias[n0 + (e % TC)];
+    e_add[u] = g.fz.addend[idx];
+    e_add2[u] = (g.addend2 ? g.addend2 : g.fz.addend)[idx];
+  }
+  for (int e = threadIdx.x; e < TR * C; e += 64 * kWskpWaves) {
+    const int r = e / C, c = e - r * C;
+    sD[r * kHjC + c] = m0 + r < B ? g.delta_top[(int64_t)(m0 + r) * C + c] : 0.f;
+  }
+  for (int e = threadIdx.x; e < C * TC; e += 64 * kWskpWaves) {
+    const int c = e / TC, j = e % TC;
+    sV[c * TC + j] = g.V[(int64_t)c * RB + n0 + j];
+  }
+  if (nch_w > 0) {
+    const int64_t sA = (int64_t)16 * RA, sB = (int64_t)16 * RB;
+    const float* gA = g.Rh1p + (int64_t)(2 * c0) * sA + (m0 + li) * 16 + 4 * lk;
+    const float* gB = g.W2p + (int64_t)(2 * c0) * sB + (n0 + li) * 16 + 4 * lk;
+    wskp_loop<2, RBLK, CBLK>(gA, gB, sA, sB, nch_w, acc);
+  }
+  float* sW = sPf + wave * (TR * TCP);
+#pragma unroll
+  for (int rb = 0; rb < RBLK; ++rb)
+#pragma unroll
+    for (int cbk = 0; cbk < CBLK; ++cbk)
+#pragma unroll
+      for (int r = 0; r < 4; ++r) sW[(16 * rb + 4 * lk + r) * TCP + 16 * cbk + li] = acc[rb][cbk][r];
+  __syncthreads();
+  const float beta = g.addend2 ? poll_beta(g.gran) : 0.f;
+  double t2 = 0.0;
+#pragma unroll
+  for (int u = 0; u < kOutPer; ++u) {
+    const int e = threadIdx.x + 64 * kWskpWaves * u;
+    const int row = e / TC, col = e % TC;
+    const int m = m0 + row;
+    const int64_t idx = (int64_t)m * RB + n0 + col;
+    float v = 0.f;
+#pragma unroll
+    for (int w = 0; w < kWskpWaves; ++w) v += sPf[w * (TR * TCP) + row * TCP + col];
+    float ad = e_add[u];
+    if (g.addend2) ad = add_rn(ad, mul_rn(beta, e_add2[u]));
+    v += ad;
+    v = (v + e_bias[u]) * e_mask[u];
+    v = m < B ? v : 0.f;
+    g.fz.rh_out[idx] = v;
+    float dv = 0.f;
+    for (int c = 0; c < C; ++c) dv += sD[row * kHjC + c] * sV[c * TC + col];
+    if (m < B) t2 += (double)dv * (double)v;
+  }
+  t2 = wave_sum(t2);
+  if (lane == 0) red[wave] = t2;
+  __syncthreads();
+  if (threadIdx.x == 0) {
+    double s = 0.0;
+#pragma unroll
+    for (int w = 0; w < kWskpWaves; ++w) s += red[w];
+    g.partT2[t] = 2.0 * s;
+    for (int z = t + g.nt; z < g.t2n; z += g.nt) g.partT2[z] = 0.0;
+  }
+}
+
+template <int U, int TS>
+__global__ __launch_bounds__(256) void k_headj(HeadjArgs g) {
+  static_assert(64 * kWskpWaves == 256, "the tiles run in the head launch's workgroups");
+  const int bx = (int)blockIdx.x;
+  if (bx >= g.rows + g.nt) { pstep_body<U, (int)offsetof(HeadjArgs, ps), false>(bx - g.rows - g.nt); return; }
+  if (bx >= g.rows) {
+    __shared__ float sPf[kWskpLds];
+    __shared__ float sD[32 * kHjC], sV[kHjC * 32];
+    __shared__ double red[kWskpWaves];
+    if constexpr (TS == 0) headj_tile<2, 2>(g, bx - g.rows, sPf, sD, sV, red);
+    else headj_tile<2, 1>(g, bx - g.rows, sPf, sD, sV, red);
+    return;
+  }
+  const float* __restrict__ Rh = nullptr; const float* __restrict__ h = g.h; const float* __restrict__ W = g.W;
+  const float* __restrict__ V = g.V; const float* __restrict__ cb = g.cb; const float* __restrict__ prob = g.prob;
+  const float* __restrict__ sd = g.sd; float* __restrict__ rd = g.rd;
+  const int K = g.K, C = g.C, B = g.B;
+  constexpr int mode = HEAD_JVP;
+  const int64_t* __restrict__ labels = nullptr; float* __restrict__ aux = nullptr; const float* __restrict__ delta_top = g.delta_top;
+  const float* __restrict__ mask_prev = g.mask_prev; float* __restrict__ rd_prev = g.rd_prev;
+  const HeadFuse fz = g.fz;
+  double* __restrict__ partT1 = g.partT1; double* __restrict__ partT2h = nullptr; float* __restrict__ rz_out = g.rz_out;
+  double* __restrict__ rzx_acc = nullptr; const int rzx_first = 0; float* __restrict__ rd_prev_p = g.rd_prev_p;
+  const float* __restrict__ lazy_addend2 = g.addend2;
+  const float lazy_beta = g.addend2 ? poll_beta(g.gran) : 0.f;
+  const float* __restrict__ hj_J = g.J; const float* __restrict__ hj_Rh1 = g.Rh1; const int hj_K1 = g.K1;
+  constexpr bool HAS_RH = true, FUSED = true, PF = true;
+  constexpr int JMAX = 3;
+  (void)Rh; (void)labels; (void)aux; (void)rzx_acc; (void)rzx_first;
+#define BHG_HEAD_B (bx)
+#define BHG_HEAD_ROWS (g.rows)
+#define BHG_HEAD_LAZY 1
+#define BHG_HEAD_J 1
+#include "mlp/head_body.inc"
+#undef BHG_HEAD_B
+#undef BHG_HEAD_ROWS
+#undef BHG_HEAD_LAZY
+#undef BHG_HEAD_J
+}
+
+__global__ __launch_bounds__(256) void k_headj_pack(const float* __restrict__ W3, const float* __restrict__ mask2, float* __restrict__ Ap,
+                                                    const int B, const int C, const int K, const int RA) {
+  const int64_t idx = (int64_t)blockIdx.x * 256 + threadIdx.x;
+  const int64_t total = (int64_t)RA * K / 4;
+  if (idx >= total) return;
+  const int c4 = (int)(idx & 3);
+  const int64_t rr = idx >> 2;
+  const int r = (int)(rr % RA), kb = (int)(rr / RA);
+  const int k = 16 * kb + 4 * c4;
+  f32x4 v = {0.f, 0.f, 0.f, 0.f};
+  if (r < B * C) {
+    const int b = r / C, c = r - b * C;
+    const f32x4 w = *reinterpret_cast<const f32x4*>(W3 + (int64_t)c * K + k);
+    const f32x4 mk = *reinterpret_cast<const f32x4*>(mask2 + (int64_t)b * K + k);
+#pragma unroll
+    for (int j = 0; j < 4; ++j) v[j] = w[j] * mk[j];
+  }
+  *reinterpret_cast<f32x4*>(Ap + idx * 4) = v;
+}
+}
+
+int headj_tiles(int rows, int K, int shape) { return (rows / 32) * (K / (shape == 0 ? 32 : 16)); }
+
+int launch_headj(const HeadjLaunch& a, hipStream_t st) {
+  BHG_REQUIRE(a.C >= 1 && a.C <= kHjC && a.K >= 32 && a.K <= 512 && a.K % 32 == 0 && a.K1 >= 32 && a.K1 % 32 == 0 && a.rows % 32 == 0 &&
+              a.B >= 1 && a.B <= a.rows, "k_headj was planned for a head it cannot run");
+  BHG_REQUIRE(a.ps && a.ps_bytes == sizeof(PstepArgs) && a.nu >= 0, "the update blocks' arguments do not match this build");
+  BHG_REQUIRE(a.J && a.Rh1 && a.Rh1p && a.W2p && a.rh_out && a.partT2 && a.addend && a.bias2 && a.mask2 && a.rd_prev && a.delta_top &&
+              a.mask_prev, "NULL argument");
+  HeadjArgs g{};
+  g.h = a.h; g.W = a.W; g.V = a.V; g.cb = a.cb; g.prob = a.prob; g.sd = a.sd; g.rd = a.rd;
+  g.K = a.K; g.C = a.C; g.B = a.B; g.rows = a.rows;
+  g.delta_top = a.delta_top; g.mask_prev = a.mask_prev; g.rd_prev = a.rd_prev; g.rd_prev_p = a.rd_prev_p;
+  g.fz = HeadFuse{nullptr, 0, a.rows * a.K, a.bias2, a.mask2, a.rh_out, a.addend};
+  g.partT1 = a.partT1; g.rz_out = a.rz_out; g.addend2 = a.addend2; g.gran = a.gran;
+  g.J = a.J; g.Rh1 = a.Rh1; g.K1 = a.K1; g.Rh1p = a.Rh1p; g.W2p = a.W2p; g.partT2 = a.partT2;
+  g.nt = headj_tiles(a.rows, a.K, a.tile_shape); g.nu = a.nu; g.t2n = a.t2n;
+  BHG_REQUIRE(a.t2n >= g.nt, "fewer T2h slots than tiles");
+  memcpy(&g.ps, a.ps, sizeof(PstepArgs));
+  const dim3 grid(a.rows + g.nt + g.nu);
+  const size_t lds = (size_t)a.K * sizeof(float);
+#ifdef BHG_AB
+  if (a.tile_shape == 0) hipLaunchKernelGGL((k_headj<4, 0>), grid, dim3(256), lds, st, g); else
+#endif
+  hipLaunchKernelGGL((k_headj<4, 1>), grid, dim3(256), lds, st, g);
+  return BHG_OK;
+}
+
+int launch_headj_pack(const float* W3, const float* mask2, float* Ap, int B, int C, int K, int RA, hipStream_t st) {
+  BHG_REQUIRE(W3 && mask2 && Ap && B >= 1 && C >= 1 && K % 16 == 0 && RA % 32 == 0 && RA >= B * C, "bad arguments");
+  const int64_t total = (int64_t)RA * K / 4;
+  hipLaunchKernelGGL(k_headj_pack, dim3((unsigned)((total + 255) / 256)), dim3(256), 0, st, W3, mask2, Ap, B, C, K, RA);
+  return BHG_OK;
+}
+
+}
diff --git a/betty_amd/csrc/bhg_mlp_headj.hpp b/betty_amd/csrc/bhg_mlp_headj.hpp
--- /dev/null
+++ b/betty_amd/csrc/bhg_mlp_headj.hpp
@@ -0,0 +1,30 @@
+#pragma once
+#include <stddef.h>
+
+#include "bhg_common.hpp"
+
+namespace bhg {
+
+struct HeadjLaunch {
+  const float* h; const float* W; const float* V; const float* cb; const float* prob; const float* sd; float* rd;
+  int K, C, B, rows;
+  const float* delta_top; const float* mask_prev; float* rd_prev; float* rd_prev_p;
+  double* partT1; float* rz_out;
+  const float* bias2; const float* mask2;
+  const float* addend; const float* addend2; const unsigned long long* gran;
+  const float* J;
+  const float* Rh1;
+  int K1;
+  const float* Rh1p; const float* W2p;
+  float* rh_out;
+  double* partT2; int t2n;
+  int tile_shape;
+  const void* ps; size_t ps_bytes; int nu;
+};
+constexpr int kHeadjTile = 1;
+int headj_tiles(int rows, int K, int shape);
+int launch_headj(const HeadjLaunch& a, hipStream_t st);
+
+int launch_headj_pack(const float* W3, const float* mask2, float* Ap, int B, int C, int K, int RA, hipStream_t st);
+
+}
diff --git a/betty_amd/csrc/mlp/chain_plan.inc b/betty_amd/csrc/mlp/chain_plan.inc
--- a/betty_amd/csrc/mlp/chain_plan.inc
+++ b/betty_amd/csrc/mlp/chain_plan.inc
@@ -29,6 +29,7 @@
   int nk;
   const void* const* rhs;
   int lin_head;
+  int head_j;
 };
 
 struct ChainPlan {
@@ -53,6 +54,7 @@
   bool rnew;
   bool vnew;
   bool lin, lin_head;
+  bool head_j;
 
   float* rh0_slot(int k) const { return (k & 1) ? hoist + hp->rh0alt_off : rh0; }
   float* gp1(int par) const { return hoist + (par ? hp->gp1alt_off : hp->g_off[hp->gf[1]]); }
@@ -67,6 +69,8 @@
   int lin_nu = 0, lin_U = 4;
   bool lin_update_pending = false;
   bool sd_in_chain = false;
+  bool head_j = false;
+  int head_j_nt = 0;
 };
 
 int plan_chain(const bhg_mlp* m, const ChainMode& cm, ChainPlan* p) {
@@ -111,6 +115,7 @@
   BHG_REQUIRE(!p->lin || (p->rnew && hp && hp->lin_ok && cm.beta && cm.beta->nt <= 16 && proj_step_merged() && L >= 4),
               "the linear first product was planned for a solve that cannot run it");
   p->lin_head = p->lin && cm.lin_head != 0;
+  p->head_j = p->lin_head && cm.head_j != 0;
   return BHG_OK;
 }
 
diff --git a/betty_amd/csrc/mlp/head_body.inc b/betty_amd/csrc/mlp/head_body.inc
--- a/betty_amd/csrc/mlp/head_body.inc
+++ b/betty_amd/csrc/mlp/head_body.inc
@@ -16,8 +16,10 @@
         *reinterpret_cast<float4*>(rd_prev + (int64_t)b * K + k) = make_float4(0.f, 0.f, 0.f, 0.f);
         if (rd_prev_p) *reinterpret_cast<float4*>(rd_prev_p + ((int64_t)(k >> 4) * BHG_HEAD_ROWS + b) * 16 + (k & 15)) = make_float4(0.f, 0.f, 0.f, 0.f);
       }
+#ifndef BHG_HEAD_J
     if (FUSED)
       for (int k = 4 * t; k < K; k += 1024) *reinterpret_cast<float4*>(fz.rh_out + (int64_t)b * K + k) = make_float4(0.f, 0.f, 0.f, 0.f);
+#endif
     return;
   }
   const float* hb = h + (int64_t)b * K;
@@ -51,12 +53,31 @@
     pf_sd = sd[b];
     pf_dt = delta_top[(int64_t)b * C + tc];
   }
+#ifdef BHG_HEAD_J
+  constexpr int HJT = 3;
+  const float* hj_rrow = hj_Rh1 + (int64_t)b * hj_K1;
+  const float* hj_jrow[JMAX];
+#pragma unroll
+  for (int j = 0; j < JMAX; ++j) hj_jrow[j] = hj_J + ((int64_t)b * C + min(wave + 4 * j, C - 1)) * hj_K1;
+  float4 hj_r[HJT], hj_j[HJT][JMAX];
+#pragma unroll
+  for (int tr = 0; tr < HJT; ++tr) {
+    const int k = 4 * lane + 256 * tr;
+    const int kc = k < hj_K1 ? k : 0;
+    hj_r[tr] = ld16(hj_rrow + kc);
+#pragma unroll
+    for (int j = 0; j < JMAX; ++j) hj_j[tr][j] = ld16(hj_jrow[j] + kc);
+  }
+#endif
   if (FUSED) {
     for (int k = 4 * t; k < K; k += 1024) {
+#ifndef BHG_HEAD_J
       const float* p0 = fz.part + (int64_t)b * K + k;
+#endif
       const float4 bv = ld16(fz.bias + k);
       const float4 mv = ld16(fz.mask + (int64_t)b * K + k);
       float4 v = make_float4(0.f, 0.f, 0.f, 0.f);
+#ifndef BHG_HEAD_J
       constexpr int NB = PF ? 16 : 8;
       for (int s0 = 0; s0 < fz.splits; s0 += NB) {
         float4 tt[NB];
@@ -66,6 +87,7 @@
         for (int u = 0; u < NB; ++u)
           if (s0 + u < fz.splits) { v.x += tt[u].x; v.y += tt[u].y; v.z += tt[u].z; v.w += tt[u].w; }
       }
+#endif
       if (fz.addend) {
         float4 ad = ld16(fz.addend + (int64_t)b * K + k);
 #if BHG_HEAD_LAZY
@@ -79,10 +101,39 @@
       }
       v.x = (v.x + bv.x) * mv.x; v.y = (v.y + bv.y) * mv.y; v.z = (v.z + bv.z) * mv.z; v.w = (v.w + bv.w) * mv.w;
       *reinterpret_cast<float4*>(srow + k) = v;
+#ifndef BHG_HEAD_J
       *reinterpret_cast<float4*>(fz.rh_out + (int64_t)b * K + k) = v;
-    }
-    __syncthreads();
-  }
+#endif
+    }
+    __syncthreads();
+  }
+#ifdef BHG_HEAD_J
+  for (int k0 = 0; k0 < hj_K1; k0 += 256 * HJT) {
+    if (k0 > 0) {
+#pragma unroll
+      for (int tr = 0; tr < HJT; ++tr) {
+        const int k = k0 + 4 * lane + 256 * tr;
+        const int kc = k < hj_K1 ? k : 0;
+        hj_r[tr] = ld16(hj_rrow + kc);
+#pragma unroll
+        for (int j = 0; j < JMAX; ++j) hj_j[tr][j] = ld16(hj_jrow[j] + kc);
+      }
+    }
+#pragma unroll
+    for (int tr = 0; tr < HJT; ++tr) {
+      if (k0 + 4 * lane + 256 * tr < hj_K1) {
+        const float4 rv = hj_r[tr];
+#pragma unroll
+        for (int j = 0; j < JMAX; ++j) {
+          float a = acc[j];
+          const float4 jv = hj_j[tr][j];
+          a = fmaf(rv.x, jv.x, a); a = fmaf(rv.y, jv.y, a); a = fmaf(rv.z, jv.z, a); a = fmaf(rv.w, jv.w, a);
+          acc[j] = a;
+        }
+      }
+    }
+  }
+#endif
   const float* rhb = HAS_RH ? (FUSED ? srow : Rh + (int64_t)b * K) : nullptr;
   float4 pf_mk, pf_W[12], pf_V[12];
   if (PF) {
diff --git a/include/bhg.h b/include/bhg.h
--- a/include/bhg.h
+++ b/include/bhg.h
@@ -188,6 +188,8 @@
 
 void* bhg_mlp_timeout_flag_dev(const bhg_mlp* m, void* fws);
 
+const float* bhg_mlp_head_j_dev(const bhg_mlp* m, void* fws, int* rows, int* cols);
+
 int bhg_mwn_max_hidden(void);
 int bhg_mwn_forward(const float* ce, int B, const float* w1, const float* b1, const float* w2, const float* b2, int H, float* s,
                     float* sd, void* stream);
```

After: 777.5 (median of 6 runs). 1.2% higher.
